# jkulhanek/tetra-nerf

Measured on AMD Instinct MI355X. Metric: ray_tet_intersections_per_s, higher is better.
Workload: dtype f32

## Files before the change

### include/tetranerf_hip.h

```cpp
#ifndef TETRANERF_HIP_H
#define TETRANERF_HIP_H

#include <stddef.h>
#include <stdint.h>

#ifdef __cplusplus
extern "C" {
#endif

typedef struct tn_tracer *tn_tracer_t;

const char *tn_last_error(void);

const char *tn_version(void);

#define TN_ABI_VERSION 6
int tn_abi_version(void);

int tn_tracer_create(int device, tn_tracer_t *out);

int tn_tracer_destroy(tn_tracer_t tracer);

int tn_load_tetrahedra(tn_tracer_t tracer, size_t num_vertices, size_t num_cells,
                       const float *xyz, const uint32_t *cells, void *stream);

int tn_update_vertices(tn_tracer_t tracer, size_t num_vertices, const float *xyz, void *stream);

size_t tn_refit_table_bytes(tn_tracer_t tracer);

#define TN_LIMIT_STEP_NO_VERIFY 1u
int tn_tet_quality(tn_tracer_t tracer, size_t num_vertices, const float *xyz, float *width, int8_t *orient, float *star_width,
                   void *stream);
int tn_limit_vertex_step(tn_tracer_t tracer, size_t num_vertices, const float *xyz_old, float *xyz_new, float fraction,
                         float *star_width, uint32_t *counters, uint32_t flags, void *stream);

int tn_delaunay_check(tn_tracer_t tracer, size_t num_vertices, const float *xyz, uint32_t *counters, int8_t *face_state,
                      uint8_t *tet_violations, void *stream);

int tn_remap_tet_values(size_t num_vertices, size_t num_old_cells, const uint32_t *old_cells, const float *old_values,
                        size_t num_new_cells, const uint32_t *new_cells, float *new_values, float *star_max, void *stream);

int tn_isosurface_count(size_t num_vertices, size_t num_cells, const uint32_t *cells, const float *values, float level,
                        const uint8_t *tet_mask, uint32_t *tri_offsets, uint32_t *ref_offsets, void *stream);
int tn_isosurface_emit(size_t num_vertices, size_t num_cells, const float *xyz, const uint32_t *cells, const float *values,
                       float level, const uint8_t *tet_mask, const uint32_t *tri_offsets, const uint32_t *ref_offsets,
                       size_t num_triangles, size_t num_refs, uint32_t *triangles, uint32_t *triangle_tets,
                       uint32_t *edge_vertices, float *edge_t, float *positions, uint32_t *num_out_vertices, void *stream);

int tn_isosurface_refine_begin(size_t num_vertices, size_t num_surface_vertices, const uint32_t *edge_vertices,
                               const float *values, float level, float *brackets, uint8_t *frozen, void *stream);
int tn_isosurface_refine_points(size_t num_vertices, size_t num_surface_vertices, uint32_t round, const uint32_t *edge_vertices,
                                const float *brackets, const uint8_t *frozen, uint32_t *vertex_indices, float *barycentric,
                                void *stream);
int tn_isosurface_refine_select(size_t num_surface_vertices, uint32_t round, float level, const float *densities,
                                float *brackets, uint8_t *frozen, void *stream);
int tn_isosurface_refine_vertices(size_t num_vertices, size_t num_surface_vertices, const float *xyz,
                                  const uint32_t *edge_vertices, const float *brackets, float level, float *edge_t,
                                  float *positions, void *stream);

int tn_split_count(size_t num_vertices, size_t num_cells, const float *xyz, const uint32_t *cells, const uint8_t *select,
                   uint32_t *offsets, uint32_t *counters, void *stream);
int tn_split_emit(size_t num_vertices, size_t num_cells, const float *xyz, const uint32_t *cells, const uint32_t *offsets,
                  size_t num_new, float *xyz_out, uint32_t *cells_out, uint32_t *cell_parent, uint32_t *vertex_parents,
                  void *stream);
int tn_split_vertex_rows(size_t rows, size_t num_vertices, size_t num_new, const float *values, const float *values_vm,
                         const uint32_t *vertex_parents, uint32_t new_mode, float *out, float *out_vm, void *stream);

int tn_prune_count(tn_tracer_t tracer, size_t num_vertices, const uint8_t *dead, const uint8_t *vertex_select, uint32_t *offsets,
                   uint32_t *counters, void *stream);
int tn_prune_count_tables(int device, size_t num_vertices, size_t num_cells, const uint32_t *cells, size_t num_faces,
                          const uint32_t *faces, const uint32_t *face_tets, const uint8_t *dead, const uint8_t *vertex_select,
                          uint32_t *offsets, uint32_t *counters, void *stream);
int tn_prune_emit(size_t num_vertices, const float *xyz, const uint32_t *offsets, size_t num_kept, uint32_t *new_id,
                  uint32_t *kept_ids, float *xyz_out, void *stream);
int tn_prune_vertex_rows(size_t rows, size_t num_vertices, size_t num_kept, const float *values, const float *values_vm,
                         const uint32_t *kept_ids, float *out, float *out_vm, void *stream);

int tn_edge_split_count_tables(int device, size_t num_vertices, size_t num_cells, const float *xyz, const uint32_t *cells,
                               const uint8_t *select, size_t num_faces, const uint32_t *faces, const uint32_t *face_tets,
                               uint32_t *tet_offsets, uint32_t *tet_edge, uint8_t *bisected, uint32_t *edge_vertices,
                               uint32_t *counters, void *stream);
int tn_edge_split_count(tn_tracer_t tracer, size_t num_vertices, const float *xyz, const uint8_t *select, uint32_t *tet_offsets,
                        uint32_t *tet_edge, uint8_t *bisected, uint32_t *edge_vertices, uint32_t *counters, void *stream);
int tn_edge_split_emit(size_t num_vertices, size_t num_cells, const float *xyz, const uint32_t *cells, const uint32_t *tet_offsets,
                       const uint32_t *tet_edge, const uint32_t *edge_vertices, size_t num_new, size_t num_rows, float *xyz_out,
                       uint32_t *cells_out, uint32_t *cell_parent, uint32_t *vertex_parents, void *stream);

size_t tn_num_faces(tn_tracer_t tracer);

int tn_get_faces(tn_tracer_t tracer, uint32_t *faces_host, uint32_t *face_tets_host);

int tn_get_build_table(tn_tracer_t tracer, int which, void *dst, size_t *bytes);

int tn_trace_rays(tn_tracer_t tracer, size_t num_rays, uint32_t max_ray_triangles,
                  const float *origins, const float *directions, uint32_t *num_visited,
                  uint32_t *visited, float *bary, float *dist, uint32_t *verts, void *stream);

#define TN_TRACE_COMPACT_ROWS 1u
#define TN_TRACE_BIN_RAYS 2u
int tn_trace_rays_ex(tn_tracer_t tracer, size_t num_rays, uint32_t max_ray_triangles,
                     const float *origins, const float *directions, uint32_t *num_visited,
                     uint32_t *visited, float *bary, float *dist, uint32_t *verts, uint32_t flags, void *stream);

int tn_trace_rays_triangles(tn_tracer_t tracer, size_t num_rays, uint32_t max_ray_triangles,
                            const float *origins, const float *directions, uint32_t *num_visited,
                            uint32_t *visited, float *bary, float *dist, uint32_t *verts, void *stream);

int tn_find_tetrahedra(tn_tracer_t tracer, size_t num_points, const float *positions, uint32_t *tetrahedra,
                       float *bary, uint32_t *verts, void *stream);

int tn_find_matched_cells(size_t num_rays, size_t num_samples, size_t max_visited_cells,
                          const uint32_t *num_visited, const uint32_t *visited,
                          const float *dist, const float *bary, const float *distances,
                          const uint32_t *verts, uint32_t *cells_out, uint32_t *verts_out,
                          uint8_t *mask_out, float *bary_out, void *stream);

int tn_find_matched_cells_indexed(size_t num_rays, size_t num_samples, size_t max_visited_cells,
                                  const uint32_t *ray_index, const uint32_t *num_visited, const uint32_t *visited,
                                  const float *dist, const float *bary, const float *distances,
                                  const uint32_t *verts, uint32_t *cells_out, uint32_t *verts_out,
                                  uint8_t *mask_out, float *bary_out, const uint32_t *count ,
                                  void *stream);

int tn_compact_hits(size_t num_rays, const uint32_t *num_visited, uint32_t *order, uint32_t *count, uint32_t *padded,
                    uint32_t *scratch, size_t scratch_len, void *stream);

int tn_interpolate_values(uint32_t interpolation_dim, uint32_t num_vertices,
                          uint32_t num_values, uint32_t field_dim,
                          const uint32_t *vertex_indices, const float *barycentric,
                          const float *field, float *result, void *stream);

int tn_interpolate_values_backward(uint32_t interpolation_dim, uint32_t num_vertices,
                                   uint32_t num_values, uint32_t field_dim,
                                   const uint32_t *vertex_indices, const float *barycentric,
                                   const float *grad_in, float *field_grad_out, void *stream);

int tn_interpolate_values_backward_rows(uint32_t interpolation_dim, uint32_t num_vertices,
                                        uint32_t num_values, uint32_t field_dim,
                                        const uint32_t *vertex_indices, const float *barycentric,
                                        const float *grad_rows, float *field_grad_out, void *stream);

int tn_transpose_f32(uint32_t rows, uint32_t cols, const float *in, float *out, void *stream);
int tn_interpolate_values_vm(uint32_t interpolation_dim, uint32_t num_values, uint32_t field_dim,
                             const uint32_t *vertex_indices, const float *barycentric, const float *field_vm,
                             float *result, void *stream);
int tn_interpolate_values_backward_vm(uint32_t interpolation_dim, uint32_t num_values, uint32_t field_dim,
                                      const uint32_t *vertex_indices, const float *barycentric,
                                      const float *grad_rows, float *field_grad_vm, void *stream);
int tn_interpolate_values_backward_vm_det(uint32_t interpolation_dim, uint32_t num_vertices, uint32_t num_values,
                                          uint32_t field_dim, const uint32_t *vertex_indices, const float *barycentric,
                                          const float *grad_rows, float *field_grad_vm, void *stream);

int tn_interpolate_values_backward_bary_vm(uint32_t interpolation_dim, uint32_t num_values, uint32_t field_dim,
                                           const uint32_t *vertex_indices, const float *grad_rows, const float *field_vm,
                                           float *grad_bary, void *stream);
int tn_sample_positions_backward(size_t num_rays, uint32_t samples_per_ray, uint32_t num_vertices,
                                 const uint32_t *vertex_indices, const float *barycentric, const float *grad_bary,
                                 const float *distances, const float *vertices,
                                 float *grad_points, float *grad_origins, float *grad_directions,
                                 float *grad_vertices, void *stream);

int tn_postprocess_hits(tn_tracer_t tracer, size_t num_rays, uint32_t max_ray_triangles,
                        const uint32_t *hit_count, const uint32_t *hit_ids, const float *hit_t,
                        const float *hit_uv, uint32_t *num_visited, uint32_t *visited,
                        float *bary, float *dist, uint32_t *verts, void *stream);

int tn_postprocess_hits_tables(int device, size_t num_rays, uint32_t max_ray_triangles, const uint32_t *faces,
                               const uint32_t *face_tets, const uint32_t *hit_count, const uint32_t *hit_ids,
                               const float *hit_t, const float *hit_uv, uint32_t *num_visited, uint32_t *visited,
                               float *bary, float *dist, uint32_t *verts, void *stream);

int tn_trace_stats(tn_tracer_t tracer, uint64_t stats[4]);

int tn_trace_flag_reasons(tn_tracer_t tracer, uint64_t reasons[16]);

int tn_trace_cross_check(tn_tracer_t tracer, uint64_t out[8]);

int tn_trace_timings(tn_tracer_t tracer, float ms[8]);

int tn_trace_ray_order(tn_tracer_t tracer, uint32_t *order_host, size_t *n);

int tn_fill_rows(size_t num_rays, uint32_t max_ray_triangles, uint32_t first_slot, uint32_t *visited, float *bary, float *dist,
                 uint32_t *verts, void *stream);

int tn_set_option(tn_tracer_t tracer, const char *name, int value);

int tn_gather_uint32(int elem_size, uint32_t num_values, uint32_t num_indices, const uint32_t *indices,
                     const void *values, void *result, void *stream);
int tn_scatter_ema_uint32(int elem_size, uint32_t num_result, uint32_t num_indices, const uint32_t *indices,
                          double decay, const void *values, void *result, void *stream);

typedef struct tn_mlp_weights {
    const float *w1, *b1;
    const float *w2, *b2;
    const float *w3, *b3;
    const float *wd, *bd;
    const float *wh, *bh;
    const float *wr, *br;
} tn_mlp_weights;

typedef struct tn_mlp *tn_mlp_t;
int tn_mlp_create(int device, tn_mlp_t *out);
int tn_mlp_destroy(tn_mlp_t mlp);
int tn_mlp_set_weights(tn_mlp_t mlp, const tn_mlp_weights *weights, void *stream);

int tn_mlp_forward(tn_mlp_t mlp, size_t n, uint32_t samples_per_ray, const float *feats, const float *dirs, int mode,
                   float *sigma, float *rgb, void *stream);

int tn_mlp_forward_gather(tn_mlp_t mlp, size_t n, uint32_t samples_per_ray, const uint32_t *vertex_indices,
                          const float *barycentric, const float *field_vm, const float *dirs, int mode, float *sigma,
                          float *rgb, const float *ray_head_bias, const uint32_t *count ,
                          void *stream);

int tn_occupancy_update(uint32_t num_cells, size_t n, const uint32_t *cells, const float *sigma, float decay, float *occupancy,
                        uint32_t samples_per_ray, const uint32_t *count, void *stream);

int tn_cull_samples(size_t n, uint32_t samples_per_ray, const uint32_t *cells, const float *occupancy, uint32_t num_cells,
                    float threshold, uint32_t *live, uint32_t *live_count, float *sigma, float *rgb, uint32_t *scratch,
                    size_t scratch_len, const uint32_t *count, void *stream);

int tn_mlp_forward_gather_indexed(tn_mlp_t mlp, size_t n_max, uint32_t samples_per_ray, const uint32_t *live,
                                  const uint32_t *live_count, const uint32_t *vertex_indices, const float *barycentric,
                                  const float *field_vm, const float *dirs, int mode, float *sigma, float *rgb,
                                  const float *ray_head_bias, const uint32_t *count, void *stream);

int tn_tet_stats_accumulate(uint32_t num_cells, size_t num_rows, uint32_t samples_per_ray, const uint32_t *cells, const float *sigma,
                            const float *edges, const float *ray_value, const uint32_t *ray_index, const uint32_t *count,
                            int64_t *stats, void *stream);

int tn_sample_live(size_t num_hit_rays, uint32_t num_samples, uint32_t max_ray_triangles, const uint32_t *ray_index,
                   const uint32_t *num_visited, const uint32_t *visited, const float *hit_distances, const float *occupancy,
                   uint32_t num_cells, float threshold, const float *linspace, const float *t_rand, float *s_edges,
                   float *near_far_live, const uint32_t *count, void *stream);
int tn_live_to_distance(size_t num_hit_rays, uint32_t num_values, uint32_t max_ray_triangles, const uint32_t *ray_index,
                        const uint32_t *num_visited, const uint32_t *visited, const float *hit_distances, const float *occupancy,
                        uint32_t num_cells, float threshold, const float *values, float *t, uint32_t *slot, const uint32_t *count,
                        void *stream);

typedef struct tn_rgb_background { float r, g, b; int clamp; } tn_rgb_background;
int tn_render_rays(tn_mlp_t mlp, uint32_t max_ray_triangles, const uint32_t *num_visited, const float *hit_distances,
                   const float *barycentric, const uint32_t *vertex_indices, const uint32_t *ray_index, const uint32_t *count,
                   size_t num_hit_rays_max, uint32_t num_samples, uint32_t num_fine, int biased, const float *linspace,
                   const float *u_table, float histogram_padding, float eps, const float *field_vm, const float *dirs,
                   const tn_rgb_background *background, float *out_rgb, float *out_acc, float *out_depth,
                   const float *ray_head_bias, void *stream);
int tn_render_rays_ex(tn_mlp_t mlp, uint32_t max_ray_triangles, const uint32_t *num_visited, const float *hit_distances,
                   const float *barycentric, const uint32_t *vertex_indices, const uint32_t *ray_index, const uint32_t *count,
                   size_t num_hit_rays_max, uint32_t num_samples, uint32_t num_fine, int biased, const float *linspace,
                   const float *u_table, float histogram_padding, float eps, const float *field_vm, const float *dirs,
                   const tn_rgb_background *background, float *out_rgb, float *out_acc, float *out_depth,
                   const float *ray_head_bias, int mode, void *stream);

int tn_sample_coarse(size_t num_hit_rays, uint32_t num_samples, uint32_t max_ray_triangles, const uint32_t *ray_index,
                     const uint32_t *num_visited, const float *hit_distances, const float *linspace, const float *t_rand,
                     int biased, float *edges, float *near_far, const uint32_t *count, void *stream);
int tn_sample_pdf(size_t num_hit_rays, uint32_t num_samples, uint32_t num_fine, const float *edges, const float *weights,
                  const float *near_far, const float *u_table, const float *u_rand, float histogram_padding, float eps,
                  float *edges_out, const uint32_t *count, void *stream);

int tn_composite(size_t num_rays, uint32_t num_samples, const float *sigma, const float *rgb, const float *edges,
                 const tn_rgb_background *background, float *out_rgb, float *out_acc, float *out_depth,
                 float *out_weights, const uint32_t *ray_index, const uint32_t *count, void *stream);

typedef struct tn_mlp_backward_buffers {
    float *x0, *h1, *h2, *h3, *h4;
    void *masks;
    float *d1, *d2, *d3, *d4, *dhead, *dx0;
} tn_mlp_backward_buffers;
int tn_mlp_forward_gather_train(tn_mlp_t mlp, size_t n, uint32_t samples_per_ray, const uint32_t *vertex_indices,
                                const float *barycentric, const float *field_vm, const float *dirs, float *sigma, float *rgb,
                                const tn_mlp_backward_buffers *buffers, const float *ray_head_bias, void *stream);
int tn_mlp_forward_gather_train_ex(tn_mlp_t mlp, size_t n, uint32_t samples_per_ray, const uint32_t *vertex_indices,
                                   const float *barycentric, const float *field_vm, const float *dirs, int mode, float *sigma,
                                   float *rgb, const tn_mlp_backward_buffers *buffers, const float *ray_head_bias, void *stream);
int tn_mlp_backward(tn_mlp_t mlp, size_t n, const float *sigma, const float *rgb, const float *d_sigma, const float *d_rgb,
                    const tn_mlp_backward_buffers *buffers, void *stream);
int tn_mlp_backward_ex(tn_mlp_t mlp, size_t n, const float *sigma, const float *rgb, const float *d_sigma, const float *d_rgb,
                       const tn_mlp_backward_buffers *buffers, int mode, void *stream);
int tn_mlp_ray_head_grad(size_t n, uint32_t samples_per_ray, const tn_mlp_backward_buffers *buffers, float *d_ray_head_bias,
                         void *stream);
typedef struct tn_mlp_grads {
    float *w1, *b1, *w2, *b2, *w3, *b3, *wd, *bd, *wh, *bh, *wr, *br;
} tn_mlp_grads;
int tn_mlp_param_grads(tn_mlp_t mlp, size_t n, uint32_t samples_per_ray, const float *dirs,
                       const tn_mlp_backward_buffers *buffers, const tn_mlp_grads *grads, void *stream);
int tn_mlp_param_grads_ex(tn_mlp_t mlp, size_t n, uint32_t samples_per_ray, const float *dirs,
                          const tn_mlp_backward_buffers *buffers, const tn_mlp_grads *grads, int mode, void *stream);

int tn_mlp_forward_gather_train_indexed(tn_mlp_t mlp, size_t n_live, size_t n_samples, uint32_t samples_per_ray, const uint32_t *live,
                                        const uint32_t *vertex_indices, const float *barycentric, const float *field_vm,
                                        const float *dirs, int mode, float *sigma, float *rgb, const tn_mlp_backward_buffers *buffers,
                                        const float *ray_head_bias, void *stream);
int tn_mlp_param_grads_indexed(tn_mlp_t mlp, size_t n_live, size_t n_samples, uint32_t samples_per_ray, const uint32_t *live,
                               const float *dirs, const tn_mlp_backward_buffers *buffers, const tn_mlp_grads *grads, int mode,
                               void *stream);
int tn_mlp_ray_head_grad_indexed(size_t n_live, size_t n_samples, uint32_t samples_per_ray, const uint32_t *live,
                                 const tn_mlp_backward_buffers *buffers, float *d_ray_head_bias, void *stream);
int tn_compact_rows(uint32_t words_per_row, size_t n_live, const uint32_t *live, const void *src, void *dst, void *stream);

int tn_composite_backward(size_t num_rays, uint32_t num_samples, const float *sigma, const float *rgb, const float *edges,
                          const tn_rgb_background *background, const float *d_out_rgb, const float *d_out_acc,
                          float *d_sigma, float *d_rgb, void *stream);

int tn_composite_aux(size_t num_rays, uint32_t num_samples, const float *sigma, const float *edges, float *out_depth_moment,
                     float *out_distortion, float *out_weights, void *stream);

int tn_composite_backward_aux(size_t num_rays, uint32_t num_samples, const float *sigma, const float *rgb, const float *edges,
                              const tn_rgb_background *background, const float *d_out_rgb, const float *d_out_acc,
                              const float *d_out_depth_moment, const float *d_out_distortion, float *d_sigma, float *d_rgb,
                              void *stream);

typedef struct tn_radam_hyper {
    float one_minus_beta1, beta2, one_minus_beta2, eps, decay;
    int decay_mode;
} tn_radam_hyper;
typedef struct tn_radam_tensor {
    float *param;
    const float *grad;
    float *exp_avg, *exp_avg_sq;
    size_t count;
    float step_size;
    int adaptive;
} tn_radam_tensor;
int tn_radam_step_field(uint32_t num_vertices, float *field, const float *grad, float *exp_avg, float *exp_avg_sq, float *shadow_vm,
                        float step_size, int adaptive, const tn_radam_hyper *hyper, void *stream);
int tn_radam_step(size_t num_tensors, const tn_radam_tensor *tensors, const tn_radam_hyper *hyper, void *stream);

#ifdef __cplusplus
}
#endif
#endif
```

### tetra-nerf_amd/_lib.py

```python
from __future__ import annotations

import ctypes as C
from pathlib import Path

import os

_HERE = Path(__file__).resolve().parent
LIB_PATH = Path(os.environ["TETRANERF_HIP_LIB"]).resolve() if os.environ.get("TETRANERF_HIP_LIB") else _HERE / "libtetranerf_hip.so"

SYMBOLS = (
    "tn_last_error", "tn_version", "tn_abi_version", "tn_tracer_create", "tn_tracer_destroy", "tn_load_tetrahedra",
    "tn_num_faces", "tn_get_faces", "tn_get_build_table", "tn_trace_rays", "tn_trace_rays_ex", "tn_trace_rays_triangles", "tn_find_tetrahedra",
    "tn_find_matched_cells", "tn_find_matched_cells_indexed",
    "tn_interpolate_values", "tn_interpolate_values_backward", "tn_interpolate_values_backward_rows",
    "tn_transpose_f32", "tn_interpolate_values_vm", "tn_interpolate_values_backward_vm", "tn_interpolate_values_backward_vm_det",
    "tn_postprocess_hits", "tn_postprocess_hits_tables",
    "tn_trace_stats", "tn_trace_flag_reasons", "tn_set_option", "tn_mlp_create", "tn_mlp_destroy", "tn_mlp_set_weights",
    "tn_mlp_forward", "tn_mlp_forward_gather", "tn_composite", "tn_gather_uint32", "tn_scatter_ema_uint32",
    "tn_mlp_forward_gather_train", "tn_mlp_forward_gather_train_ex", "tn_mlp_backward", "tn_mlp_backward_ex", "tn_mlp_ray_head_grad", "tn_mlp_param_grads", "tn_mlp_param_grads_ex", "tn_composite_backward", "tn_sample_coarse", "tn_sample_pdf",
    "tn_trace_timings", "tn_trace_cross_check", "tn_fill_rows", "tn_compact_hits", "tn_render_rays", "tn_render_rays_ex",
    "tn_trace_ray_order",
    "tn_interpolate_values_backward_bary_vm", "tn_sample_positions_backward",
    "tn_occupancy_update", "tn_cull_samples", "tn_mlp_forward_gather_indexed",
    "tn_mlp_forward_gather_train_indexed", "tn_mlp_param_grads_indexed", "tn_mlp_ray_head_grad_indexed", "tn_compact_rows",
    "tn_update_vertices", "tn_refit_table_bytes",
    "tn_sample_live", "tn_live_to_distance",
    "tn_composite_aux", "tn_composite_backward_aux",
    "tn_tet_quality", "tn_limit_vertex_step",
    "tn_delaunay_check", "tn_remap_tet_values",
    "tn_isosurface_count", "tn_isosurface_emit",
    "tn_isosurface_refine_begin", "tn_isosurface_refine_points", "tn_isosurface_refine_select", "tn_isosurface_refine_vertices",
    "tn_radam_step_field", "tn_radam_step",
    "tn_split_count", "tn_split_emit", "tn_split_vertex_rows",
    "tn_tet_stats_accumulate",
    "tn_prune_count", "tn_prune_count_tables", "tn_prune_emit", "tn_prune_vertex_rows",
    "tn_edge_split_count", "tn_edge_split_count_tables", "tn_edge_split_emit",
)

ABI_VERSION = 6

_lib = None


def load():
    global _lib
    if _lib is not None:
        return _lib
    if not LIB_PATH.exists():
        raise RuntimeError(
            f"ERROR: {LIB_PATH} is missing. Build it first: python __graft_entry__.py "
            "(or make -C tetra-nerf_amd/csrc). There is no CPU fallback.")
    lib = C.CDLL(str(LIB_PATH))
    vp, sz, u32, i32 = C.c_void_p, C.c_size_t, C.c_uint32, C.c_int
    lib.tn_last_error.restype = C.c_char_p
    lib.tn_last_error.argtypes = []
    lib.tn_version.restype = C.c_char_p
    lib.tn_version.argtypes = []
    if not hasattr(lib, "tn_abi_version") or lib.tn_abi_version() != ABI_VERSION:
        got = lib.tn_abi_version() if hasattr(lib, "tn_abi_version") else "none (a build older than ABI 6)"
        raise RuntimeError(f"ERROR: {LIB_PATH} exports ABI {got}, this binding needs ABI {ABI_VERSION} "
                           "(include/tetranerf_hip.h: TN_ABI_VERSION). Rebuild it: python __graft_entry__.py")
    lib.tn_abi_version.argtypes = []
    lib.tn_tracer_create.argtypes = [i32, C.POINTER(vp)]
    lib.tn_tracer_destroy.argtypes = [vp]
    lib.tn_load_tetrahedra.argtypes = [vp, sz, sz, vp, vp, vp]
    lib.tn_update_vertices.argtypes = [vp, sz, vp, vp]
    lib.tn_tet_quality.argtypes = [vp, sz, vp, vp, vp, vp, vp]
    lib.tn_limit_vertex_step.argtypes = [vp, sz, vp, vp, C.c_float, vp, vp, u32, vp]
    lib.tn_delaunay_check.argtypes = [vp, sz, vp, vp, vp, vp, vp]
    lib.tn_remap_tet_values.argtypes = [sz, sz, vp, vp, sz, vp, vp, vp, vp]
    lib.tn_isosurface_count.argtypes = [sz, sz, vp, vp, C.c_float, vp, vp, vp, vp]
    lib.tn_isosurface_emit.argtypes = [sz, sz, vp, vp, vp, C.c_float, vp, vp, vp, sz, sz, vp, vp, vp, vp, vp, vp, vp]
    lib.tn_isosurface_refine_begin.argtypes = [sz, sz, vp, vp, C.c_float, vp, vp, vp]
    lib.tn_isosurface_refine_points.argtypes = [sz, sz, u32, vp, vp, vp, vp, vp, vp]
    lib.tn_isosurface_refine_select.argtypes = [sz, u32, C.c_float, vp, vp, vp, vp]
    lib.tn_isosurface_refine_vertices.argtypes = [sz, sz, vp, vp, vp, C.c_float, vp, vp, vp]
    lib.tn_split_count.argtypes = [sz, sz, vp, vp, vp, vp, vp, vp]
    lib.tn_split_emit.argtypes = [sz, sz, vp, vp, vp, sz, vp, vp, vp, vp, vp]
    lib.tn_split_vertex_rows.argtypes = [sz, sz, sz, vp, vp, vp, u32, vp, vp, vp]
    lib.tn_prune_count.argtypes = [vp, sz, vp, vp, vp, vp, vp]
    lib.tn_prune_count_tables.argtypes = [i32, sz, sz, vp, sz, vp, vp, vp, vp, vp, vp, vp]
    lib.tn_prune_emit.argtypes = [sz, vp, vp, sz, vp, vp, vp, vp]
    lib.tn_prune_vertex_rows.argtypes = [sz, sz, sz, vp, vp, vp, vp, vp, vp]
    lib.tn_edge_split_count_tables.argtypes = [i32, sz, sz, vp, vp, vp, sz, vp, vp, vp, vp, vp, vp, vp, vp]
    lib.tn_edge_split_count.argtypes = [vp, sz, vp, vp, vp, vp, vp, vp, vp, vp]
    lib.tn_edge_split_emit.argtypes = [sz, sz, vp, vp, vp, vp, vp, sz, sz, vp, vp, vp, vp, vp]
    lib.tn_tet_stats_accumulate.argtypes = [u32, sz, u32, vp, vp, vp, vp, vp, vp, vp, vp]
    lib.tn_refit_table_bytes.restype = sz
    lib.tn_refit_table_bytes.argtypes = [vp]
    lib.tn_num_faces.restype = sz
    lib.tn_num_faces.argtypes = [vp]
    lib.tn_get_faces.argtypes = [vp, vp, vp]
    lib.tn_get_build_table.argtypes = [vp, i32, vp, C.POINTER(sz)]
    lib.tn_trace_rays.argtypes = [vp, sz, u32, vp, vp, vp, vp, vp, vp, vp, vp]
    lib.tn_trace_rays_ex.argtypes = [vp, sz, u32, vp, vp, vp, vp, vp, vp, vp, u32, vp]
    lib.tn_trace_rays_triangles.argtypes = [vp, sz, u32, vp, vp, vp, vp, vp, vp, vp, vp]
    lib.tn_find_tetrahedra.argtypes = [vp, sz, vp, vp, vp, vp, vp]
    lib.tn_find_matched_cells.argtypes = [sz, sz, sz] + [vp] * 11
    lib.tn_find_matched_cells_indexed.argtypes = [sz, sz, sz] + [vp] * 13
    lib.tn_interpolate_values.argtypes = [u32, u32, u32, u32, vp, vp, vp, vp, vp]
    lib.tn_interpolate_values_backward.argtypes = [u32, u32, u32, u32, vp, vp, vp, vp, vp]
    lib.tn_interpolate_values_backward_rows.argtypes = [u32, u32, u32, u32, vp, vp, vp, vp, vp]
    lib.tn_transpose_f32.argtypes = [u32, u32, vp, vp, vp]
    lib.tn_interpolate_values_vm.argtypes = [u32, u32, u32, vp, vp, vp, vp, vp]
    lib.tn_interpolate_values_backward_vm.argtypes = [u32, u32, u32, vp, vp, vp, vp, vp]
    lib.tn_interpolate_values_backward_vm_det.argtypes = [u32, u32, u32, u32, vp, vp, vp, vp, vp]
    lib.tn_interpolate_values_backward_bary_vm.argtypes = [u32, u32, u32, vp, vp, vp, vp, vp]
    lib.tn_sample_positions_backward.argtypes = [sz, u32, u32] + [vp] * 10
    lib.tn_postprocess_hits.argtypes = [vp, sz, u32] + [vp] * 10
    lib.tn_postprocess_hits_tables.argtypes = [i32, sz, u32] + [vp] * 12
    lib.tn_trace_stats.argtypes = [vp, C.POINTER(C.c_uint64 * 4)]
    lib.tn_trace_flag_reasons.argtypes = [vp, C.POINTER(C.c_uint64 * 16)]
    lib.tn_set_option.argtypes = [vp, C.c_char_p, i32]
    lib.tn_trace_timings.argtypes = [vp, C.POINTER(C.c_float * 8)]
    lib.tn_trace_cross_check.argtypes = [vp, C.POINTER(C.c_uint64 * 8)]
    lib.tn_trace_ray_order.argtypes = [vp, vp, C.POINTER(sz)]
    lib.tn_fill_rows.argtypes = [sz, u32, u32, vp, vp, vp, vp, vp]
    lib.tn_mlp_create.argtypes = [i32, C.POINTER(vp)]
    lib.tn_mlp_destroy.argtypes = [vp]
    lib.tn_mlp_set_weights.argtypes = [vp, vp, vp]
    lib.tn_mlp_forward.argtypes = [vp, sz, u32, vp, vp, i32, vp, vp, vp]
    lib.tn_mlp_forward_gather.argtypes = [vp, sz, u32, vp, vp, vp, vp, i32, vp, vp, vp, vp, vp]
    lib.tn_gather_uint32.argtypes = [i32, u32, u32, vp, vp, vp, vp]
    lib.tn_scatter_ema_uint32.argtypes = [i32, u32, u32, vp, C.c_double, vp, vp, vp]
    lib.tn_composite.argtypes = [sz, u32, vp, vp, vp, vp, vp, vp, vp, vp, vp, vp, vp]
    lib.tn_mlp_forward_gather_train.argtypes = [vp, sz, u32, vp, vp, vp, vp, vp, vp, vp, vp, vp]
    lib.tn_mlp_forward_gather_train_ex.argtypes = [vp, sz, u32, vp, vp, vp, vp, i32, vp, vp, vp, vp, vp]
    lib.tn_mlp_ray_head_grad.argtypes = [sz, u32, vp, vp, vp]
    lib.tn_mlp_backward.argtypes = [vp, sz, vp, vp, vp, vp, vp, vp]
    lib.tn_mlp_backward_ex.argtypes = [vp, sz, vp, vp, vp, vp, vp, i32, vp]
    lib.tn_mlp_param_grads.argtypes = [vp, sz, u32, vp, vp, vp, vp]
    lib.tn_mlp_param_grads_ex.argtypes = [vp, sz, u32, vp, vp, vp, i32, vp]
    lib.tn_composite_backward.argtypes = [sz, u32, vp, vp, vp, vp, vp, vp, vp, vp, vp]
    lib.tn_composite_aux.argtypes = [sz, u32, vp, vp, vp, vp, vp, vp]
    lib.tn_composite_backward_aux.argtypes = [sz, u32, vp, vp, vp, vp, vp, vp, vp, vp, vp, vp, vp]
    lib.tn_sample_coarse.argtypes = [sz, u32, u32, vp, vp, vp, vp, vp, i32, vp, vp, vp, vp]
    lib.tn_sample_pdf.argtypes = [sz, u32, u32, vp, vp, vp, vp, vp, C.c_float, C.c_float, vp, vp, vp]
    lib.tn_sample_live.argtypes = [sz, u32, u32, vp, vp, vp, vp, vp, u32, C.c_float, vp, vp, vp, vp, vp, vp]
    lib.tn_live_to_distance.argtypes = [sz, u32, u32, vp, vp, vp, vp, vp, u32, C.c_float, vp, vp, vp, vp, vp]
    lib.tn_compact_hits.argtypes = [sz, vp, vp, vp, vp, vp, sz, vp]
    lib.tn_render_rays.argtypes = [vp, u32, vp, vp, vp, vp, vp, vp, sz, u32, u32, i32, vp, vp, C.c_float, C.c_float, vp, vp, vp, vp, vp, vp, vp, vp]
    lib.tn_render_rays_ex.argtypes = [vp, u32, vp, vp, vp, vp, vp, vp, sz, u32, u32, i32, vp, vp, C.c_float, C.c_float, vp, vp, vp, vp, vp, vp, vp, i32, vp]
    lib.tn_occupancy_update.argtypes = [u32, sz, vp, vp, C.c_float, vp, u32, vp, vp]
    lib.tn_cull_samples.argtypes = [sz, u32, vp, vp, u32, C.c_float, vp, vp, vp, vp, vp, sz, vp, vp]
    lib.tn_mlp_forward_gather_indexed.argtypes = [vp, sz, u32, vp, vp, vp, vp, vp, vp, i32, vp, vp, vp, vp, vp]
    lib.tn_mlp_forward_gather_train_indexed.argtypes = [vp, sz, sz, u32, vp, vp, vp, vp, vp, i32, vp, vp, vp, vp, vp]
    lib.tn_mlp_param_grads_indexed.argtypes = [vp, sz, sz, u32, vp, vp, vp, vp, i32, vp]
    lib.tn_mlp_ray_head_grad_indexed.argtypes = [sz, sz, u32, vp, vp, vp, vp]
    lib.tn_compact_rows.argtypes = [u32, sz, vp, vp, vp, vp]
    lib.tn_radam_step_field.argtypes = [u32, vp, vp, vp, vp, vp, C.c_float, i32, vp, vp]
    lib.tn_radam_step.argtypes = [sz, vp, vp, vp]
    for name in SYMBOLS:
        fn = getattr(lib, name)
        if fn.restype is C.c_int and name not in ("tn_last_error", "tn_version", "tn_abi_version", "tn_num_faces", "tn_refit_table_bytes"):
            fn.restype = C.c_int
    _lib = lib
    return lib


def check(rc: int):
    if rc != 0:
        msg = load().tn_last_error().decode("utf-8", "replace")
        raise RuntimeError(msg or f"libtetranerf_hip call failed (rc={rc})")
```

### tetra-nerf_amd/csrc/tn_api_tracer.hip

```cpp
#include <algorithm>
#include <cmath>
#include <cstring>
#include <memory>
#include <mutex>

#include "tn_api_common.h"
#include "tn_build.h"
#include "tn_devbuf.h"
#include "tn_isosurface_core.h"
#include "tn_kernels.h"
#include "tn_split_core.h"
#include "tn_edge_split_core.h"

using tn::check_loaded;
using tn::check_pow2_M;
using tn::DeviceGuard;
using tn::guarded;

struct tn_tracer {
    int device = 0;
    std::mutex mu;

    struct Mesh {
        bool loaded = false;
        tn::DeviceMesh view;
        tn::HostMesh host;
        uint32_t bvh_max_stack = 1;
        tn::DevBuf<uint32_t> faces, face_tets;
        tn::DevWideBvh bvh;
        tn::DevBuf<tn::WalkVar> vars;
        tn::DevBuf<tn::WalkHot> hot;
        tn::DevBuf<tn::WalkCold> cold;
        tn::DevBuf<tn::WalkTet> tets;
        tn::DevBuf<tn::WalkFid> fidt;
        tn::DevBuf<float> hull_nodes, hull_tris;
        tn::RefitTables refit;
        bool device_built = false;
    } mesh;

    struct Options {
        bool gpu_build = true;
        unsigned leaf_width = 16;
        int writer_table = 0;
        bool refit_tables = false;
        int use_walk = 1;
        size_t walk_min_rays = 12288;
        bool walk_min_auto = true;
        bool dense_tails = true;
        bool literal = true;
        size_t log_cap_bytes = 0;
        int spec_fill = 0;
        unsigned spec_k0 = 0;
        tn::FillRange spec{true, 0, true, tn::FillKind::Spans, 512};
        unsigned walk_lds_kb = 26;
        tn::FillRange tail{false, 0, false, tn::FillKind::RowPerBlock, 0};
        unsigned writer_blocks = 0;
        bool hull_flat = true;
        bool small_lds = true;
        unsigned lds_cap = 0;
        unsigned verify_stride = 256;
        bool verify_risk = true;
        unsigned risk_band = 2;
        bool verify_inject = false;
        unsigned literal_sort_passes = 8;
        int cert_ends = 2;
        bool bin_rays = false;
        bool timing = false;
    } opt;

    struct Scratch {
        tn::DevBuf<uint32_t> fallback_list;
        tn::DevBuf<uint32_t> walk_n;
        tn::DevBuf<uint4> hull_entry;
        tn::DevBuf<uint2> literal_list;
        tn::DevBuf<uint4> hit_log;
        tn::DevBuf<uint32_t> verify_list;
        tn::DevBuf<uint32_t> risk_list;
        tn::DevBuf<uint32_t> ray_keys, ray_iota, ray_keys_sorted, order, walk_n_item;
        tn::DevBuf<char> sort_temp;
        static constexpr int N_CTR = 2;
        tn::DevBuf<unsigned long long> stats;
        uint32_t *fallback_count() { return reinterpret_cast<uint32_t *>(stats.p + tn::N_STATS); }
        uint32_t *literal_count() { return fallback_count() + 1; }
        uint32_t *verify_count() { return fallback_count() + 2; }
        uint32_t *risk_count() { return fallback_count() + 3; }
        static constexpr size_t stats_bytes() { return (tn::N_STATS + N_CTR) * sizeof(unsigned long long); }
        size_t last_num_rays = 0;
        bool last_walk = false;
        bool last_binned = false;
        hipStream_t last_stream = nullptr;

        template <typename T>
        static void grow(tn::DevBuf<T> &b, size_t n) { if (b.n < n) b.alloc(n); }
        void reserve(size_t R, size_t log_entries, bool verify, bool risk, size_t sort_temp_bytes = 0) {
            grow(fallback_list, R);
            if (!log_entries) return;
            grow(walk_n, R); grow(literal_list, R); grow(hull_entry, R); grow(hit_log, log_entries);
            if (verify) grow(verify_list, R);
            if (risk) grow(risk_list, R);
            if (sort_temp_bytes) {
                grow(ray_keys, R); grow(ray_iota, R); grow(ray_keys_sorted, R); grow(order, R); grow(walk_n_item, R);
                grow(sort_temp, sort_temp_bytes);
            }
        }
    } scratch;

    struct Schedule {
        hipStream_t side = nullptr;
        hipStream_t aux = nullptr;
        hipStream_t pre = nullptr;
        hipEvent_t ev_fork = nullptr, ev_join = nullptr, ev_start = nullptr, ev_pre = nullptr, ev_seg = nullptr, ev_aux = nullptr;
        static constexpr int N_TEV = 9;
        hipEvent_t tev[N_TEV] = {};
        bool tev_valid = false;
    } sched;
};

namespace {

tn_tracer *checked(tn_tracer_t t) {
    if (!t) throw tn::Error("tracer handle is null");
    return t;
}

void check_bvh_depth(uint32_t max_stack) {
    if (max_stack + (uint32_t)tn::WIDE > (uint32_t)tn::STACK_CAP)
        throw tn::Error("face BVH too deep for the traversal stack (" + std::to_string(max_stack) + " > " +
                        std::to_string(tn::STACK_CAP) + " entries)");
}

struct BuildCounts { size_t F = 0, n_hull = 0, n_hull_nodes = 0; };

BuildCounts build_on_host(tn_tracer::Mesh &m, unsigned leaf_width, size_t V, size_t T, const float *xyz, const uint32_t *cells,
                          hipStream_t stream) {
    std::vector<float> hxyz(3 * V);
    std::vector<uint32_t> hcells(4 * T);
    TN_HIP(hipStreamSynchronize(stream));
    if (V) TN_HIP(hipMemcpy(hxyz.data(), xyz, hxyz.size() * sizeof(float), hipMemcpyDeviceToHost));
    if (T) TN_HIP(hipMemcpy(hcells.data(), cells, hcells.size() * sizeof(uint32_t), hipMemcpyDeviceToHost));
    for (size_t i = 0; i < hcells.size(); ++i)
        if (hcells[i] >= V) throw tn::Error("cells contains a vertex index that is out of bounds");

    tn::build_face_table(T, hcells.data(), m.host);
    const size_t F = m.host.face_tets.size() / 2;
    float smax = 0.f;
    for (size_t i = 0; i < hcells.size(); ++i)
        for (int k = 0; k < 3; ++k) smax = std::max(smax, std::fabs(hxyz[3 * (size_t)hcells[i] + k]));
    m.host.scene_max = smax;

    std::vector<uint32_t> all(F), hull_ids;
    for (size_t f = 0; f < F; ++f) {
        all[f] = (uint32_t)f;
        if (m.host.face_tets[2 * f + 1] == TN_EMPTY) hull_ids.push_back((uint32_t)f);
    }
    tn::HostWideBvh hb;
    tn::build_wide_bvh(hxyz.data(), m.host.faces.data(), all, hb, leaf_width);
    check_bvh_depth(hb.max_stack);
    m.bvh_max_stack = hb.max_stack;
    std::vector<tn::TetRec> recs;
    std::vector<uint32_t> rec_of_tet;
    tn::build_tet_records(T, hcells.data(), hxyz.data(), m.host, recs, rec_of_tet);
    tn::HostHullBvh hth;
    tn::build_hull_threaded(hxyz.data(), m.host.faces.data(), m.host.face_tets.data(), hull_ids, recs, rec_of_tet, hth);

    m.faces.upload(m.host.faces);
    m.face_tets.upload(m.host.face_tets);
    m.bvh.upload(hb, smax);
    {
        std::vector<tn::WalkVar> vars;
        tn::build_walk_variants(recs, vars);
        m.vars.upload(vars);
    }
    m.hull_nodes.upload(hth.nodes_and_flat());
    m.hull_tris.upload(hth.tris);
    return BuildCounts{F, hull_ids.size(), hth.nodes.size() / 8};
}

tn::TraceParams mesh_params(const tn_tracer *t, size_t num_items, const tn::Rows &r, const float *o, const float *d) {
    tn::TraceParams p{};
    p.origins = o; p.dirs = d;
    p.faces = t->mesh.view.faces; p.face_tets = t->mesh.view.face_tets;
    p.bvh = t->mesh.view.bvh;
    p.out_num = r.num; p.out_cells = r.cells; p.out_bary = r.bary; p.out_dist = r.dist; p.out_verts = r.verts;
    p.M = r.M; p.num_items = num_items; p.ray_list = nullptr;
    return p;
}

struct TraceCall {
    tn_tracer *t;
    size_t R;
    const float *origins, *dirs;
    tn::Rows rows;
    bool dense_tails;
    hipStream_t stream;
    bool binned = false;

    const tn_tracer::Options &o() const { return t->opt; }
    tn_tracer::Scratch &s() const { return t->scratch; }
    const tn::DeviceMesh &mesh() const { return t->mesh.view; }
    bool verify_risk() const { return o().verify_risk && o().verify_stride; }

    size_t walk_min_rays() const {
        if (!o().walk_min_auto) return o().walk_min_rays;
        return mesh().T >= 4000000u ? (size_t)6144 : mesh().T >= 2000000u ? (size_t)8192 : o().walk_min_rays;
    }
    bool use_walk() const {
        return o().use_walk && (R >= walk_min_rays() || o().use_walk == 2) && rows.M >= 4 && mesh().n_hull > 0 &&
               mesh().n_hull < (1u << 24);
    }
    size_t log_chunk() const {
        size_t cap_bytes = o().log_cap_bytes;
        if (!cap_bytes) {
            size_t free_b = 0, total_b = 0;
            TN_HIP(hipMemGetInfo(&free_b, &total_b));
            cap_bytes = std::min<size_t>((free_b + s().hit_log.n * sizeof(uint4)) / 4, (size_t)24 << 30);
        }
        const size_t chunk = std::max<size_t>(cap_bytes / ((size_t)rows.M * sizeof(uint4)) / 4096 * 4096, 4096);
        return std::min(chunk, R);
    }

    tn::TraceParams trace_params(size_t base, size_t n) const {
        tn::TraceParams q = mesh_params(t, n, rows.at(base), origins + 3 * base, dirs + 3 * base);
        q.stats = s().stats.p;
        q.compact_rows = dense_tails ? 0u : 1u;
        q.sort_passes = o().literal_sort_passes;
        return q;
    }
    tn::WalkParams walk_params(size_t base, size_t n) const {
        const tn::DeviceMesh &m = mesh();
        tn::WalkParams w{};
        w.t = trace_params(base, n);
        w.vars = m.hot;
        w.scene_max = m.bvh.scene_max;
        w.hull_nodes = m.hull_nodes; w.hull_tris = m.hull_tris; w.n_hull_nodes = m.n_hull_nodes; w.n_hull = m.n_hull;
        w.hull_flat = m.hull_nodes + 2 * (size_t)m.n_hull_nodes;
        w.n_hull_leaves = o().hull_flat ? tn::hull_flat_leaves(m.n_hull) : 0u;
        w.n_hull_groups = o().hull_flat ? tn::hull_flat_groups(m.n_hull) : 0u;
        w.ray_base = base;
        w.hull_entry = s().hull_entry.p + base; w.walk_n = s().walk_n.p + base; w.hit_log = s().hit_log.p;
        w.fallback_list = s().fallback_list.p; w.fallback_count = s().fallback_count();
        w.literal_list = o().literal ? s().literal_list.p : nullptr; w.literal_count = s().literal_count();
        w.risk_list = verify_risk() ? s().risk_list.p : nullptr; w.risk_count = s().risk_count();
        w.risk_band = (float)o().risk_band;
        if (binned) { w.order = s().order.p; w.walk_n_item = s().walk_n_item.p; }
        w.cert_ends = o().cert_ends == 2 ? (m.T >= tn::WALK_TET_MIN_TETS ? 1u : 3u) : (uint32_t)o().cert_ends;
        return w;
    }
    tn::WriteParams write_params(size_t base, size_t n) const {
        const tn::Rows r = rows.at(base);
        tn::WriteParams q{};
        q.num_rays = n; q.M = r.M; q.dense_tails = dense_tails ? 1u : 0u;
        q.walk_n = s().walk_n.p + base;
        q.hit_log = s().hit_log.p;
        q.cold = mesh().cold; q.tets = mesh().tets;
        q.out_cells = r.cells; q.out_bary = r.bary; q.out_dist = r.dist; q.out_verts = r.verts;
        if (binned) { q.walk_n = s().walk_n_item.p; q.order = s().order.p; }
        return q;
    }

    void fill_tails(size_t base, size_t n, uint32_t k_hi) const {
        if (!dense_tails) return;
        tn::FillRange f = o().tail;
        f.k_split = k_hi;
        tn::launch_fill(rows.at(base), n, s().walk_n.p + base, f, stream);
    }
    void pair_literal(size_t base, size_t n, hipStream_t st) const {
        if (!o().literal) return;
        tn::launch_postprocess_log(trace_params(base, n), mesh().fidt, s().hit_log.p, s().literal_list.p, s().literal_count(), n, st,
                                   binned ? s().order.p : nullptr);
    }
    void trace_listed(const uint32_t *list, const uint32_t *count, size_t max_items, hipStream_t st) const {
        tn::TraceParams q = trace_params(0, max_items);
        q.ray_list = list; q.item_count = count;
        tn::launch_trace_general(q, st);
    }

    uint32_t spec_fill_first_slot() const {
        if (!o().spec_fill || !dense_tails) return 0;
        const uint32_t M = rows.M;
        uint32_t K0 = (((uint32_t)(3.6 * std::cbrt((double)std::max<uint32_t>(mesh().T, 1u))) + 31u) & ~31u) + 32u;
        const uint32_t quarter = (3u * M / 4u) & ~31u, half = (M / 2u) & ~31u;
        if (mesh().T >= tn::WALK_TET_MIN_TETS) K0 = K0 > quarter + 32u ? 0u : quarter;
        else K0 = K0 > quarter ? 0u : (K0 + 32u > half ? half : quarter);
        if (o().spec_k0) K0 = o().spec_k0 & ~31u;
        return K0 + 32u > M ? 0u : K0;
    }

    void run_overlapped() const {
        tn_tracer::Schedule &c = t->sched;
        const bool timing = o().timing;
        const hipStream_t s_pre = timing ? stream : c.pre, s_aux = timing ? stream : c.aux, s_side = timing ? stream : c.side;
        if (timing && !c.tev[0])
            for (hipEvent_t &e : c.tev) TN_HIP(hipEventCreate(&e));
        int mark_i = 0;
        auto mark = [&] { if (timing) TN_HIP(hipEventRecord(c.tev[mark_i++], stream)); };
        const uint32_t K0 = spec_fill_first_slot();
        mark();
        if (K0) {
            TN_HIP(hipEventRecord(c.ev_start, stream));
            TN_HIP(hipStreamWaitEvent(s_pre, c.ev_start, 0));
            tn::FillRange f = o().spec;
            f.k_split = K0;
            tn::launch_fill(rows, R, s().walk_n.p, f, s_pre);
            TN_HIP(hipEventRecord(c.ev_pre, s_pre));
        }
        mark();
        if (binned)
            tn::launch_ray_order(R, origins, dirs, tn::ray_key_box(mesh().box_lo, mesh().box_hi), s().ray_keys.p, s().ray_iota.p,
                                 s().ray_keys_sorted.p, s().order.p, s().sort_temp.p, s().sort_temp.n, stream);
        tn::launch_trace_walk(walk_params(0, R), stream, K0 && !timing ? (size_t)o().walk_lds_kb * 1024 : 0);
        mark();
        TN_HIP(hipEventRecord(c.ev_fork, stream));
        TN_HIP(hipStreamWaitEvent(s_aux, c.ev_fork, 0));
        if (K0) {
            TN_HIP(hipStreamWaitEvent(s_aux, c.ev_pre, 0));
            TN_HIP(hipStreamWaitEvent(stream, c.ev_pre, 0));
        }
        trace_listed(s().fallback_list.p, s().fallback_count(), R, s_aux);
        mark();
        if (o().verify_stride) {
            tn::launch_verify_counts(trace_params(0, R), o().verify_stride, s().walk_n.p, s().verify_list.p, s().verify_count(), 0,
                                     s_aux, true, o().verify_inject);
            if (verify_risk())
                tn::launch_verify_counts(trace_params(0, R), o().verify_stride, s().walk_n.p, s().verify_list.p, s().verify_count(), 0,
                                         s_aux, true, false, s().risk_list.p, s().risk_count(), R);
        }
        mark();
        TN_HIP(hipEventRecord(c.ev_aux, s_aux));
        tn::launch_write_segments(write_params(0, R), stream, o().writer_blocks);
        mark();
        TN_HIP(hipEventRecord(c.ev_seg, stream));
        TN_HIP(hipStreamWaitEvent(s_side, c.ev_seg, 0));
        pair_literal(0, R, s_side);
        mark();
        fill_tails(0, R, K0 ? K0 : rows.M);
        mark();
        TN_HIP(hipEventRecord(c.ev_join, s_side));
        TN_HIP(hipStreamWaitEvent(stream, c.ev_join, 0));
        TN_HIP(hipStreamWaitEvent(stream, c.ev_aux, 0));
        if (o().verify_stride) trace_listed(s().verify_list.p, s().verify_count(), 64, stream);
        mark();
        c.tev_valid = timing;
    }

    void run_chunked(size_t chunk) const {
        for (size_t base = 0; base < R; base += chunk) {
            const size_t n = std::min(R - base, chunk);
            TN_HIP(hipMemsetAsync(s().literal_count(), 0, sizeof(uint32_t), stream));
            TN_HIP(hipMemsetAsync(s().risk_count(), 0, sizeof(uint32_t), stream));
            const tn::WalkParams w = walk_params(base, n);
            tn::launch_trace_walk(w, stream, 0);
            if (o().verify_stride) {
                tn::launch_verify_counts(w.t, o().verify_stride, w.walk_n, w.fallback_list, w.fallback_count, base, stream, false,
                                         o().verify_inject);
                if (verify_risk())
                    tn::launch_verify_counts(w.t, o().verify_stride, w.walk_n, w.fallback_list, w.fallback_count, base, stream, false,
                                             false, s().risk_list.p, s().risk_count(), n);
            }
            tn::launch_write_segments(write_params(base, n), stream, o().writer_blocks);
            fill_tails(base, n, rows.M);
            pair_literal(base, n, stream);
        }
        trace_listed(s().fallback_list.p, s().fallback_count(), R, stream);
    }

    void run_small_batch() const {
        uint32_t C = 64;
        const double expect = 3.6 * std::cbrt((double)std::max<uint32_t>(mesh().T, 1u));
        while (C < expect && C < rows.M) C <<= 1;
        if (o().lds_cap) C = o().lds_cap;
        tn::TraceParams p = trace_params(0, R);
        if (o().small_lds && C < rows.M) {
            s().reserve(R, 0, false, false);
            tn::TraceParams p1 = p;
            p1.lds_cap = C; p1.overflow_list = s().fallback_list.p; p1.overflow_count = s().fallback_count();
            tn::launch_trace_general(p1, stream);
            p.ray_list = s().fallback_list.p;
            p.item_count = s().fallback_count();
        }
        tn::launch_trace_general(p, stream);
    }
};

}

extern "C" {

int tn_tracer_create(int device, tn_tracer_t *out) {
    return guarded([&] {
        if (!out) throw tn::Error("out is null");
        int count = 0;
        TN_HIP(hipGetDeviceCount(&count));
        if (device < 0 || device >= count) throw tn::Error("The device argument must be a CUDA device.");
        DeviceGuard g(device);
        auto t = std::make_unique<tn_tracer>();
        t->device = device;
        t->opt.use_walk = tn::env_flag("TETRANERF_HIP_WALK", true) ? 1 : 0;
        t->opt.gpu_build = tn::env_flag("TETRANERF_HIP_GPU_BUILD", true);
        t->opt.bin_rays = tn::env_flag("TETRANERF_HIP_BIN_RAYS", false);
        t->scratch.stats.alloc(tn::N_STATS + tn_tracer::Scratch::N_CTR);
        TN_HIP(hipMemset(t->scratch.stats.p, 0, tn_tracer::Scratch::stats_bytes()));
        tn_tracer::Schedule &c = t->sched;
        int least = 0, greatest = 0;
        TN_HIP(hipDeviceGetStreamPriorityRange(&least, &greatest));
        TN_HIP(hipStreamCreateWithPriority(&c.side, hipStreamNonBlocking, least));
        TN_HIP(hipStreamCreateWithPriority(&c.aux, hipStreamNonBlocking, least));
        TN_HIP(hipStreamCreateWithFlags(&c.pre, hipStreamNonBlocking));
        for (hipEvent_t *e : {&c.ev_fork, &c.ev_join, &c.ev_start, &c.ev_pre, &c.ev_seg, &c.ev_aux})
            TN_HIP(hipEventCreateWithFlags(e, hipEventDisableTiming));
        *out = t.release();
    });
}

int tn_tracer_destroy(tn_tracer_t tracer) {
    return guarded([&] {
        if (!tracer) return;
        DeviceGuard g(tracer->device);
        (void)hipDeviceSynchronize();
        const tn_tracer::Schedule &c = tracer->sched;
        for (hipStream_t st : {c.side, c.aux, c.pre})
            if (st) (void)hipStreamDestroy(st);
        for (hipEvent_t e : {c.ev_fork, c.ev_join, c.ev_start, c.ev_pre, c.ev_seg, c.ev_aux})
            if (e) (void)hipEventDestroy(e);
        for (hipEvent_t e : c.tev)
            if (e) (void)hipEventDestroy(e);
        delete tracer;
    });
}

int tn_load_tetrahedra(tn_tracer_t tracer, size_t V, size_t T, const float *xyz, const uint32_t *cells,
                       void *stream_) {
    return guarded([&] {
        tn_tracer *t = checked(tracer);
        std::lock_guard<std::mutex> lock(t->mu);
        DeviceGuard g(t->device);
        hipStream_t stream = (hipStream_t)stream_;
        if ((V && !xyz) || (T && !cells)) throw tn::Error("xyz / cells must not be null");
        if (V >= 0xFFFFFFFFull || T >= 0x0FFFFFFFull) throw tn::Error("mesh too large (uint32 ids)");
        if (T == 0) throw tn::Error("load_tetrahedra needs at least one tetrahedron");
        tn_tracer::Mesh &b = t->mesh;
        b.loaded = false;
        b.host.faces.clear(); b.host.face_tets.clear();
        b.refit.release();
        b.device_built = t->opt.gpu_build;
        BuildCounts n;
        if (b.device_built) {
            tn::BuildInfo bi;
            tn::device_build(V, T, xyz, cells, stream,
                             tn::BuildTargets{b.faces, b.face_tets, b.vars, b.hull_nodes, b.hull_tris, b.bvh}, bi, t->opt.leaf_width,
                             t->opt.refit_tables ? &b.refit : nullptr);
            check_bvh_depth(bi.max_stack);
            b.host.scene_max = bi.scene_max;
            b.bvh_max_stack = bi.max_stack;
            n = BuildCounts{bi.F, bi.n_hull, bi.n_hull_nodes};
        } else {
            n = build_on_host(b, t->opt.leaf_width, V, T, xyz, cells, stream);
        }

        tn::DeviceMesh &m = b.view;
        m.xyz = xyz; m.cells = cells;
        m.V = (uint32_t)V; m.T = (uint32_t)T; m.F = (uint32_t)n.F;
        m.faces = b.faces.p; m.face_tets = b.face_tets.p;
        m.bvh = b.bvh.view;
        {
            const size_t n4 = b.vars.n;
            const bool per_tet = t->opt.writer_table ? t->opt.writer_table == 2 : n4 / 4 >= tn::WALK_TET_MIN_TETS;
            b.hot.alloc(n4); b.fidt.alloc(n4);
            b.cold.release(); b.tets.release();
            if (per_tet) b.tets.alloc(n4 / 4); else b.cold.alloc(n4);
            tn::launch_split_walk_records(n4, b.vars.p, b.hot.p, per_tet ? nullptr : b.cold.p, per_tet ? b.tets.p : nullptr,
                                          b.fidt.p, stream);
            TN_HIP(hipStreamSynchronize(stream));
            b.vars.release();
        }
        m.hot = b.hot.p; m.cold = b.cold.n ? b.cold.p : nullptr; m.tets = b.tets.n ? b.tets.p : nullptr; m.fidt = b.fidt.p;
        m.n_hull = (uint32_t)n.n_hull;
        m.hull_nodes = reinterpret_cast<const float4 *>(b.hull_nodes.p);
        m.hull_tris = reinterpret_cast<const float4 *>(b.hull_tris.p);
        m.n_hull_nodes = (uint32_t)n.n_hull_nodes;
        tn::mesh_box(V, T, xyz, cells, m.box_lo, m.box_hi, stream);
        b.loaded = true;
    });
}

int tn_update_vertices(tn_tracer_t tracer, size_t V, const float *xyz, void *stream_) {
    return guarded([&] {
        tn_tracer *t = checked(tracer);
        std::lock_guard<std::mutex> lock(t->mu);
        tn_tracer::Mesh &b = t->mesh;
        if (!b.loaded) throw tn::Error("tn_update_vertices: no mesh is loaded; call load_tetrahedra first");
        if (!b.device_built)
            throw tn::Error("tn_update_vertices: the mesh was built on the host (option \"gpu_build\" = 0); the refit is part of the "
                            "device build: set \"gpu_build\" = 1 and load again, or reload after every move");
        if (!b.refit.valid)
            throw tn::Error("tn_update_vertices: the mesh was loaded without the refit tables; set option \"refit_tables\" = 1 "
                            "(Python: load_tetrahedra(..., refittable=True)) and load again");
        if (V != b.view.V)
            throw tn::Error("tn_update_vertices: " + std::to_string(V) + " vertices given, the loaded mesh has " +
                            std::to_string(b.view.V) + "; a mesh with other vertices or cells needs load_tetrahedra");
        if (!xyz) throw tn::Error("tn_update_vertices: xyz must not be null");
        DeviceGuard g(t->device);
        hipStream_t stream = (hipStream_t)stream_;
        tn::DeviceMesh &m = b.view;
        float smax = 0.f;
        tn::device_refit(V, m.T, xyz, m.cells, stream, tn::RefitTargets{b.hot.p, b.faces.p, b.hull_nodes, b.hull_tris, b.bvh}, b.refit,
                         smax, m.box_lo, m.box_hi);
        b.host.scene_max = smax;
        m.bvh = b.bvh.view;
        m.xyz = xyz;
    });
}

size_t tn_refit_table_bytes(tn_tracer_t tracer) {
    return tracer && tracer->mesh.loaded && tracer->mesh.refit.valid ? tracer->mesh.refit.bytes() : 0;
}

namespace {
void check_guard_mesh(tn_tracer *t, const char *who, size_t V) {
    tn_tracer::Mesh &b = t->mesh;
    if (!b.loaded) throw tn::Error(std::string(who) + ": no mesh is loaded; call load_tetrahedra first");
    if (V != b.view.V)
        throw tn::Error(std::string(who) + ": " + std::to_string(V) + " vertices given, the loaded mesh has " + std::to_string(b.view.V));
}
}

int tn_tet_quality(tn_tracer_t tracer, size_t V, const float *xyz, float *width, int8_t *orient, float *star_width, void *stream_) {
    return guarded([&] {
        tn_tracer *t = checked(tracer);
        std::lock_guard<std::mutex> lock(t->mu);
        check_guard_mesh(t, "tn_tet_quality", V);
        const tn::DeviceMesh &m = t->mesh.view;
        if (!xyz) throw tn::Error("tn_tet_quality: xyz must not be null");
        DeviceGuard g(t->device);
        tn::launch_tet_quality(V, m.T, m.cells, xyz, width, orient, star_width, (hipStream_t)stream_);
    });
}

int tn_limit_vertex_step(tn_tracer_t tracer, size_t V, const float *xyz_old, float *xyz_new, float fraction, float *star_width,
                         uint32_t *counters, uint32_t flags, void *stream_) {
    return guarded([&] {
        tn_tracer *t = checked(tracer);
        std::lock_guard<std::mutex> lock(t->mu);
        check_guard_mesh(t, "tn_limit_vertex_step", V);
        const tn::DeviceMesh &m = t->mesh.view;
        if (!xyz_old || !xyz_new || !star_width || !counters)
            throw tn::Error("tn_limit_vertex_step: xyz_old, xyz_new, star_width and counters must not be null");
        if (!(fraction > 0.f && fraction <= 0.45f))
            throw tn::Error("tn_limit_vertex_step: fraction must be in (0, 0.45]: the bound is proved for moves below half a width, "
                            "and 0.45 leaves room for the rounding of the new coordinates");
        if (flags & ~(uint32_t)TN_LIMIT_STEP_NO_VERIFY) throw tn::Error("tn_limit_vertex_step: unknown flags");
        DeviceGuard g(t->device);
        tn::launch_limit_vertex_step(V, m.T, m.cells, xyz_old, xyz_new, fraction, star_width, counters,
                                     !(flags & TN_LIMIT_STEP_NO_VERIFY), (hipStream_t)stream_);
    });
}

int tn_delaunay_check(tn_tracer_t tracer, size_t V, const float *xyz, uint32_t *counters, int8_t *face_state, uint8_t *tet_violations,
                      void *stream_) {
    return guarded([&] {
        tn_tracer *t = checked(tracer);
        std::lock_guard<std::mutex> lock(t->mu);
        check_guard_mesh(t, "tn_delaunay_check", V);
        const tn::DeviceMesh &m = t->mesh.view;
        if (!xyz || !counters) throw tn::Error("tn_delaunay_check: xyz and counters must not be null");
        if ((uintptr_t)tet_violations & 3u)
            throw tn::Error("tn_delaunay_check: tet_violations must be 4-byte aligned (its bytes are counted through 32-bit atomics)");
        DeviceGuard g(t->device);
        tn::launch_delaunay_check(m.T, m.F, m.cells, m.face_tets, xyz, counters, face_state, tet_violations, (hipStream_t)stream_);
    });
}

int tn_remap_tet_values(size_t V, size_t num_old_cells, const uint32_t *old_cells, const float *old_values, size_t num_new_cells,
// ... 215 lines not shown
        if (num_kept && (!kept_ids || !out || (!values && !values_vm)))
            throw tn::Error("tn_prune_vertex_rows: a null pointer beside a non-zero count");
        tn::launch_prune_vertex_rows(rows, V, num_kept, values, values_vm, kept_ids, out, out_vm, (hipStream_t)stream_);
    });
}

namespace {
void check_edge_split_count(const char *who, size_t V, size_t T, size_t F, const void *xyz, const void *cells, const void *select,
                            const void *faces, const void *face_tets, const void *tet_offsets, const void *tet_edge,
                            const void *bisected, const void *edge_vertices, const void *counters) {
    const std::string w(who);
    if (V >= 0xFFFFFFFFull) throw tn::Error(w + ": too many vertices (uint32 ids)");
    if (T >= tn::esplit::MAX_CELLS) throw tn::Error(w + ": num_cells must be below 2^30");
    if (F >= 0xFFFFFFFFull) throw tn::Error(w + ": too many faces");
    if (!tet_offsets || !counters || (T && (!cells || !select || !tet_edge || !bisected || !edge_vertices)) || (T && V && !xyz) ||
        (F && (!faces || !face_tets)))
        throw tn::Error(w + ": a null pointer beside a non-zero count");
}
}

int tn_edge_split_count_tables(int device, size_t V, size_t T, const float *xyz, const uint32_t *cells, const uint8_t *select,
                               size_t F, const uint32_t *faces, const uint32_t *face_tets, uint32_t *tet_offsets, uint32_t *tet_edge,
                               uint8_t *bisected, uint32_t *edge_vertices, uint32_t *counters, void *stream_) {
    return guarded([&] {
        check_edge_split_count("tn_edge_split_count_tables", V, T, F, xyz, cells, select, faces, face_tets, tet_offsets, tet_edge,
                               bisected, edge_vertices, counters);
        DeviceGuard g(device);
        tn::launch_edge_split_count(V, T, xyz, cells, select, F, faces, face_tets, tet_offsets, tet_edge, bisected, edge_vertices,
                                    counters, (hipStream_t)stream_);
    });
}

int tn_edge_split_count(tn_tracer_t tracer, size_t V, const float *xyz, const uint8_t *select, uint32_t *tet_offsets,
                        uint32_t *tet_edge, uint8_t *bisected, uint32_t *edge_vertices, uint32_t *counters, void *stream_) {
    return guarded([&] {
        tn_tracer *t = checked(tracer);
        std::lock_guard<std::mutex> lock(t->mu);
        check_guard_mesh(t, "tn_edge_split_count", V);
        const tn::DeviceMesh &m = t->mesh.view;
        check_edge_split_count("tn_edge_split_count", V, m.T, m.F, xyz, m.cells, select, m.faces, m.face_tets, tet_offsets, tet_edge,
                               bisected, edge_vertices, counters);
        DeviceGuard g(t->device);
        tn::launch_edge_split_count(V, m.T, xyz, m.cells, select, m.F, m.faces, m.face_tets, tet_offsets, tet_edge, bisected,
                                    edge_vertices, counters, (hipStream_t)stream_);
    });
}

int tn_edge_split_emit(size_t V, size_t T, const float *xyz, const uint32_t *cells, const uint32_t *tet_offsets,
                       const uint32_t *tet_edge, const uint32_t *edge_vertices, size_t num_new, size_t num_rows, float *xyz_out,
                       uint32_t *cells_out, uint32_t *cell_parent, uint32_t *vertex_parents, void *stream_) {
    return guarded([&] {
        const std::string w("tn_edge_split_emit");
        if (num_new > T || num_rows > T) throw tn::Error(w + ": num_new or num_rows exceeds num_cells (a tetrahedron is bisected at most once)");
        if (V >= 0xFFFFFFFFull || V + num_new >= 0xFFFFFFFFull) throw tn::Error(w + ": too many vertices (uint32 ids)");
        if (T >= tn::esplit::MAX_CELLS || T + num_rows >= tn::esplit::MAX_CELLS) throw tn::Error(w + ": num_cells + num_rows must be below 2^30");
        if ((T && (!cells || !tet_offsets || !tet_edge || !cells_out || !cell_parent)) || (V && (!xyz || !xyz_out)) ||
            (num_new && (!edge_vertices || !xyz_out || !vertex_parents)) || (num_rows && !edge_vertices))
            throw tn::Error(w + ": a null pointer beside a non-zero count");
        tn::launch_edge_split_emit(V, T, xyz, cells, tet_offsets, tet_edge, edge_vertices, num_new, num_rows, xyz_out, cells_out,
                                   cell_parent, vertex_parents, (hipStream_t)stream_);
    });
}

size_t tn_num_faces(tn_tracer_t tracer) { return tracer && tracer->mesh.loaded ? tracer->mesh.view.F : 0; }

int tn_get_faces(tn_tracer_t tracer, uint32_t *faces_host, uint32_t *face_tets_host) {
    return guarded([&] {
        tn_tracer *t = checked(tracer);
        check_loaded(t->mesh.loaded);
        tn_tracer::Mesh &b = t->mesh;
        const size_t F = b.view.F;
        if (b.host.face_tets.size() != 2 * F) {
            DeviceGuard g(t->device);
            b.host.faces.resize(3 * F);
            b.host.face_tets.resize(2 * F);
            if (F) {
                TN_HIP(hipMemcpy(b.host.faces.data(), b.faces.p, b.host.faces.size() * sizeof(uint32_t), hipMemcpyDeviceToHost));
                TN_HIP(hipMemcpy(b.host.face_tets.data(), b.face_tets.p, b.host.face_tets.size() * sizeof(uint32_t), hipMemcpyDeviceToHost));
            }
        }
        if (faces_host) std::memcpy(faces_host, b.host.faces.data(), b.host.faces.size() * sizeof(uint32_t));
        if (face_tets_host) std::memcpy(face_tets_host, b.host.face_tets.data(), b.host.face_tets.size() * sizeof(uint32_t));
    });
}

int tn_get_build_table(tn_tracer_t tracer, int which, void *dst, size_t *bytes) {
    return guarded([&] {
        tn_tracer *t = checked(tracer);
        check_loaded(t->mesh.loaded);
        DeviceGuard g(t->device);
        const tn_tracer::Mesh &b = t->mesh;
        const void *src = nullptr;
        size_t n = 0;
        switch (which) {
            case 0: src = b.faces.p; n = b.faces.n * 4; break;
            case 1: src = b.face_tets.p; n = b.face_tets.n * 4; break;
            case 2: {
                const size_t n4 = b.hot.n;
                n = n4 * sizeof(tn::WalkVar);
                if (bytes) *bytes = n;
                if (dst && n4) {
                    std::vector<tn::WalkHot> h(n4); std::vector<tn::WalkTet> c(b.tets.n); std::vector<tn::WalkCold> cc(b.cold.n);
                    std::vector<tn::WalkFid> f(n4);
                    TN_HIP(hipMemcpy(h.data(), b.hot.p, n4 * sizeof(tn::WalkHot), hipMemcpyDeviceToHost));
                    if (!c.empty()) TN_HIP(hipMemcpy(c.data(), b.tets.p, c.size() * sizeof(tn::WalkTet), hipMemcpyDeviceToHost));
                    if (!cc.empty()) TN_HIP(hipMemcpy(cc.data(), b.cold.p, cc.size() * sizeof(tn::WalkCold), hipMemcpyDeviceToHost));
                    TN_HIP(hipMemcpy(f.data(), b.fidt.p, n4 * sizeof(tn::WalkFid), hipMemcpyDeviceToHost));
                    tn::WalkVar *o = static_cast<tn::WalkVar *>(dst);
                    for (size_t i = 0; i < n4; ++i) {
                        tn::WalkVar v{};
                        for (int k = 0; k < 3; ++k) v.pn[k] = h[i].pn[k];
                        v.nb[0] = h[i].nb0; v.nb[1] = h[i].nb1; v.nb[2] = h[i].nb2; v.code_lo = h[i].code_lo; v.code_hi = h[i].code_hi;
                        if (!c.empty()) { v.orig = c[i >> 2].orig; for (uint32_t k = 0; k < 4; ++k) v.vid[k] = c[i >> 2].vid((uint32_t)(i & 3), k); }
                        else { v.orig = cc[i].orig; for (int k = 0; k < 4; ++k) v.vid[k] = cc[i].vid[k]; }
                        v.fid0 = f[i].fid[0]; v.fid1 = f[i].fid[1]; v.fid2 = f[i].fid[2];
                        o[i] = v;
                    }
                }
                return;
            }
            case 3: src = b.hull_nodes.p; n = b.hull_nodes.n * 4; break;
            case 4: src = b.hull_tris.p; n = b.hull_tris.n * 4; break;
            case 5: src = b.bvh.child.p; n = b.bvh.child.n * 4; break;
            case 6: src = b.bvh.boxes.p; n = b.bvh.boxes.n * 4; break;
            case 7: src = b.bvh.leaf_id.p; n = b.bvh.leaf_id.n * 4; break;
            case 8: src = b.bvh.leaf_tri.p; n = b.bvh.leaf_tri.n * 4; break;
            default: throw tn::Error("unknown table");
        }
        if (bytes) *bytes = n;
        if (dst && n) TN_HIP(hipMemcpy(dst, src, n, hipMemcpyDeviceToHost));
    });
}

int tn_trace_rays_ex(tn_tracer_t tracer, size_t R, uint32_t M, const float *origins, const float *directions,
                     uint32_t *num_visited, uint32_t *visited, float *bary, float *dist, uint32_t *verts,
                     uint32_t flags, void *stream_) {
    return guarded([&] {
        tn_tracer *t = checked(tracer);
        std::lock_guard<std::mutex> lock(t->mu);
        if (flags & ~(uint32_t)(TN_TRACE_COMPACT_ROWS | TN_TRACE_BIN_RAYS)) throw tn::Error("unknown trace flag");
        check_pow2_M(M);
        check_loaded(t->mesh.loaded);
        if (M > 4096) throw tn::Error("max_ray_triangles larger than 4096 is not supported");
        if (R >= 0xFFFFFFFFull) throw tn::Error("too many rays for one call");
        if (R == 0) return;
        if (!origins || !directions || !num_visited || !visited || !bary || !dist)
            throw tn::Error("null ray / output pointer");
        DeviceGuard g(t->device);
        TraceCall call{t, R, origins, directions, tn::Rows{num_visited, visited, bary, dist, verts, M},
                             t->opt.dense_tails && !(flags & TN_TRACE_COMPACT_ROWS), (hipStream_t)stream_};
        tn_tracer::Scratch &s = t->scratch;
        TN_HIP(hipMemsetAsync(s.stats.p, 0, tn_tracer::Scratch::stats_bytes(), call.stream));
        s.last_stream = call.stream;
        s.last_num_rays = R;
        s.last_walk = call.use_walk();
        s.last_binned = false;
        if (s.last_walk) {
            const size_t chunk = call.log_chunk();
            call.binned = s.last_binned = ((flags & TN_TRACE_BIN_RAYS) || t->opt.bin_rays) && chunk >= R;
            s.reserve(R, (chunk + 255) / 256 * 256 * (size_t)M, t->opt.verify_stride != 0, call.verify_risk(),
                      call.binned ? tn::ray_order_temp_bytes(R) : 0);
            if (chunk >= R) call.run_overlapped();
            else call.run_chunked(chunk);
        } else {
            call.run_small_batch();
        }
        TN_HIP(hipGetLastError());
    });
}

int tn_trace_rays(tn_tracer_t tracer, size_t R, uint32_t M, const float *origins, const float *directions,
                  uint32_t *num_visited, uint32_t *visited, float *bary, float *dist, uint32_t *verts,
                  void *stream_) {
    return tn_trace_rays_ex(tracer, R, M, origins, directions, num_visited, visited, bary, dist, verts, 0u, stream_);
}

int tn_postprocess_hits(tn_tracer_t tracer, size_t R, uint32_t M, const uint32_t *hit_count,
                        const uint32_t *hit_ids, const float *hit_t, const float *hit_uv,
                        uint32_t *num_visited, uint32_t *visited, float *bary, float *dist, uint32_t *verts,
                        void *stream_) {
    return guarded([&] {
        tn_tracer *t = checked(tracer);
        check_pow2_M(M);
        check_loaded(t->mesh.loaded);
        if (R == 0) return;
        DeviceGuard g(t->device);
        const tn::TraceParams p = mesh_params(t, R, tn::Rows{num_visited, visited, bary, dist, verts, M}, nullptr, nullptr);
        tn::launch_postprocess_hits(p, hit_count, hit_ids, hit_t, hit_uv, (hipStream_t)stream_);
        TN_HIP(hipGetLastError());
    });
}

int tn_postprocess_hits_tables(int device, size_t R, uint32_t M, const uint32_t *faces, const uint32_t *face_tets,
                               const uint32_t *hit_count, const uint32_t *hit_ids, const float *hit_t,
                               const float *hit_uv, uint32_t *num_visited, uint32_t *visited, float *bary, float *dist,
                               uint32_t *verts, void *stream_) {
    return guarded([&] {
        check_pow2_M(M);
        if (!faces || !face_tets) throw tn::Error("null face table");
        if (R == 0) return;
        DeviceGuard g(device);
        tn::TraceParams p{};
        p.M = M; p.num_items = R;
        p.faces = faces; p.face_tets = face_tets;
        p.out_num = num_visited; p.out_cells = visited; p.out_bary = bary; p.out_dist = dist; p.out_verts = verts;
        tn::launch_postprocess_hits(p, hit_count, hit_ids, hit_t, hit_uv, (hipStream_t)stream_);
        TN_HIP(hipGetLastError());
    });
}

int tn_trace_rays_triangles(tn_tracer_t tracer, size_t R, uint32_t M, const float *origins, const float *directions,
                            uint32_t *num_visited, uint32_t *visited, float *bary, float *dist, uint32_t *verts,
                            void *stream_) {
    return guarded([&] {
        tn_tracer *t = checked(tracer);
        check_pow2_M(M);
        check_loaded(t->mesh.loaded);
        if (M > 4096) throw tn::Error("max_ray_triangles larger than 4096 is not supported");
        if (R == 0) return;
        DeviceGuard g(t->device);
        const tn::TraceParams p = mesh_params(t, R, tn::Rows{num_visited, nullptr, nullptr, nullptr, nullptr, M}, origins, directions);
        tn::launch_trace_triangles(p, visited, dist, bary, verts, (hipStream_t)stream_);
        TN_HIP(hipGetLastError());
    });
}

int tn_find_tetrahedra(tn_tracer_t tracer, size_t N, const float *positions, uint32_t *tetrahedra, float *bary,
                       uint32_t *verts, void *stream_) {
    return guarded([&] {
        tn_tracer *t = checked(tracer);
        check_loaded(t->mesh.loaded);
        if (N == 0) return;
        DeviceGuard g(t->device);
        const tn::TraceParams p = mesh_params(t, N, tn::Rows{nullptr, nullptr, nullptr, nullptr, nullptr, 512}, nullptr, nullptr);
        tn::launch_find_tetrahedra(p, positions, tetrahedra, bary, verts, (hipStream_t)stream_);
        TN_HIP(hipGetLastError());
    });
}

int tn_trace_stats(tn_tracer_t tracer, uint64_t stats[4]) {
    return guarded([&] {
        tn_tracer *t = checked(tracer);
        std::lock_guard<std::mutex> lock(t->mu);
        DeviceGuard g(t->device);
        TN_HIP(hipStreamSynchronize(t->scratch.last_stream));
        unsigned long long h[tn::N_STATS];
        TN_HIP(hipMemcpy(h, t->scratch.stats.p, sizeof h, hipMemcpyDeviceToHost));
        const size_t R = t->scratch.last_num_rays;
        size_t other = R;
        if (t->scratch.last_walk) {
            uint32_t fb = 0;
            TN_HIP(hipMemcpy(&fb, t->scratch.fallback_count(), sizeof fb, hipMemcpyDeviceToHost));
            other = (uint32_t)(fb + (uint32_t)h[tn::STAT_REASON + tn::REASON_LITERAL_PAIRED]);
        }
        stats[tn::STAT_WALK] = R - other;
        stats[tn::STAT_OTHER] = other;
        stats[tn::STAT_LITERAL_BRANCH] = h[tn::STAT_LITERAL_BRANCH];
        stats[tn::STAT_OVERFLOW] = h[tn::STAT_OVERFLOW];
    });
}

int tn_trace_flag_reasons(tn_tracer_t tracer, uint64_t reasons[16]) {
    return guarded([&] {
        tn_tracer *t = checked(tracer);
        std::lock_guard<std::mutex> lock(t->mu);
        DeviceGuard g(t->device);
        TN_HIP(hipStreamSynchronize(t->scratch.last_stream));
        unsigned long long h[tn::N_STATS];
        TN_HIP(hipMemcpy(h, t->scratch.stats.p, sizeof h, hipMemcpyDeviceToHost));
        for (int i = 0; i < tn::N_REASONS; ++i) reasons[i] = h[tn::STAT_REASON + i];
    });
}

int tn_trace_cross_check(tn_tracer_t tracer, uint64_t out[8]) {
    return guarded([&] {
        tn_tracer *t = checked(tracer);
        std::lock_guard<std::mutex> lock(t->mu);
        if (!out) throw tn::Error("out is null");
        DeviceGuard g(t->device);
        TN_HIP(hipStreamSynchronize(t->scratch.last_stream));
        unsigned long long h[tn::N_STATS];
        TN_HIP(hipMemcpy(h, t->scratch.stats.p, sizeof h, hipMemcpyDeviceToHost));
        out[0] = t->opt.verify_stride;
        out[1] = h[tn::STAT_REASON + tn::REASON_VERIFY_CHECKED]; out[2] = h[tn::STAT_REASON + tn::REASON_VERIFY_BAD];
        out[3] = h[tn::STAT_RISK_HULL]; out[4] = h[tn::STAT_RISK_THIN];
        out[5] = h[tn::STAT_RISK_CHECKED]; out[6] = h[tn::STAT_RISK_BAD]; out[7] = 0;
    });
}

int tn_trace_ray_order(tn_tracer_t tracer, uint32_t *order_host, size_t *n) {
    return guarded([&] {
        tn_tracer *t = checked(tracer);
        std::lock_guard<std::mutex> lock(t->mu);
        if (!n) throw tn::Error("n is null");
        const tn_tracer::Scratch &s = t->scratch;
        *n = s.last_binned ? s.last_num_rays : 0;
        if (!order_host || !*n) return;
        DeviceGuard g(t->device);
        TN_HIP(hipStreamSynchronize(s.last_stream));
        TN_HIP(hipMemcpy(order_host, s.order.p, *n * sizeof(uint32_t), hipMemcpyDeviceToHost));
    });
}

int tn_trace_timings(tn_tracer_t tracer, float ms[8]) {
    return guarded([&] {
        tn_tracer *t = checked(tracer);
        std::lock_guard<std::mutex> lock(t->mu);
        if (!ms) throw tn::Error("ms is null");
        const tn_tracer::Schedule &c = t->sched;
        if (!c.tev_valid) throw tn::Error("no timed call: set option \"timing\" = 1 and trace a one-chunk walk call first");
        DeviceGuard g(t->device);
        TN_HIP(hipEventSynchronize(c.tev[c.N_TEV - 1]));
        for (int i = 0; i + 1 < c.N_TEV; ++i) TN_HIP(hipEventElapsedTime(&ms[i], c.tev[i], c.tev[i + 1]));
    });
}

int tn_fill_rows(size_t R, uint32_t M, uint32_t first_slot, uint32_t *visited, float *bary, float *dist, uint32_t *verts,
                 void *stream_) {
    return guarded([&] {
        if (R == 0) return;
        if (!visited || !bary || !dist) throw tn::Error("null output pointer");
        if (M < 4 || (M & (M - 1)) != 0) throw tn::Error("max_ray_triangles must be a power of 2.");
        if (first_slot >= M) return;
        if (first_slot & 31u) throw tn::Error("tn_fill_rows: first_slot must be a multiple of 32");
        tn::launch_fill(tn::Rows{nullptr, visited, bary, dist, verts, M}, R, nullptr,
                        tn::FillRange{true, first_slot, false, tn::FillKind::Linear, 0}, (hipStream_t)stream_);
        TN_HIP(hipGetLastError());
    });
}

int tn_set_option(tn_tracer_t tracer, const char *name, int value) {
    return guarded([&] {
        tn_tracer *t = checked(tracer);
        std::lock_guard<std::mutex> lock(t->mu);
        tn_tracer::Options &o = t->opt;
        auto set_grid = [](tn::FillRange &f, int v) {
            f.kind = v == -2 ? tn::FillKind::Linear : v < 0 ? tn::FillKind::RowPerBlock : tn::FillKind::Spans;
            f.blocks = v > 0 ? (unsigned)v : 0u;
        };
        const std::string k = name ? name : "";
        if (k == "gpu_build") o.gpu_build = value != 0;
        else if (k == "bin_rays") o.bin_rays = value != 0;
        else if (k == "timing") { o.timing = value != 0; t->sched.tev_valid = false; }
        else if (k == "leaf_width") {
            if (value != 16 && value != 32 && value != 64) throw tn::Error("leaf_width must be 16, 32 or 64");
            o.leaf_width = (unsigned)value;
        }
        else if (k == "walk") o.use_walk = value < 0 ? 0 : (value > 2 ? 2 : value);
        else if (k == "walk_min_rays") { o.walk_min_rays = value < 0 ? 0 : (size_t)value; o.walk_min_auto = false; }
        else if (k == "dense_tails") o.dense_tails = value != 0;
        else if (k == "literal") o.literal = value != 0;
        else if (k == "spec_fill") o.spec_fill = value != 0;
        else if (k == "spec_k0") o.spec_k0 = (unsigned)value;
        else if (k == "spec_blocks") set_grid(o.spec, value);
        else if (k == "hull_flat") o.hull_flat = value != 0;
        else if (k == "writer_blocks") o.writer_blocks = (unsigned)value;
        else if (k == "fill_blocks") set_grid(o.tail, value);
        else if (k == "walk_lds_kb") o.walk_lds_kb = (unsigned)value;
        else if (k == "small_lds") o.small_lds = value != 0;
        else if (k == "lds_cap") {
            if (value < 0 || (value & (value - 1)) != 0 || (value && value < 8)) throw tn::Error("lds_cap must be 0 or a power of two >= 8");
            o.lds_cap = (unsigned)value;
        }
        else if (k == "writer_table") o.writer_table = value;
        else if (k == "refit_tables") o.refit_tables = value != 0;
        else if (k == "cert_ends") { if (value < 0 || value > 3) throw tn::Error("cert_ends must be 0 .. 3"); o.cert_ends = value; }
        else if (k == "verify_inject") o.verify_inject = value != 0;
        else if (k == "literal_sort_passes") o.literal_sort_passes = value < 0 ? 0u : (unsigned)value;
        else if (k == "verify_stride") o.verify_stride = value < 0 ? 0u : (unsigned)value;
        else if (k == "verify_risk") o.verify_risk = value != 0;
        else if (k == "risk_band") o.risk_band = value < 1 ? 1u : (unsigned)value;
        else if (k == "log_cap_mb") o.log_cap_bytes = value <= 0 ? 0 : (size_t)value << 20;
        else throw tn::Error("unknown option " + (name ? k : std::string("(null)")));
    });
}

}
```

### tetra-nerf_amd/csrc/tn_kernels.h

```cpp
#pragma once
#include "tn_common.h"
#include "tn_ray_key.h"

namespace tn {

struct Rows {
    uint32_t *num;
    uint32_t *cells;
    float *bary;
    float *dist;
    uint32_t *verts;
    uint32_t M;
    Rows at(size_t base) const {
        return Rows{num ? num + base : nullptr, cells + base * M, bary + base * M * 6, dist + base * M * 2,
                    verts ? verts + base * M * 4 : nullptr, M};
    }
};

struct TraceParams {
    const float *origins;
    const float *dirs;
    const uint32_t *faces;
    const uint32_t *face_tets;
    WideBvh bvh;
    uint32_t *out_num;
    uint32_t *out_cells;
    float *out_bary;
    float *out_dist;
    uint32_t *out_verts;
    uint32_t M;
    size_t num_items;
    const uint32_t *ray_list;
    const uint32_t *item_count;
    uint32_t lds_cap;
    uint32_t *overflow_list;
    uint32_t *overflow_count;
    unsigned long long *stats;
    uint32_t compact_rows;
    uint32_t sort_passes;
};

void launch_trace_general(const TraceParams &p, hipStream_t stream);
void launch_postprocess_hits(const TraceParams &p, const uint32_t *hit_count, const uint32_t *hit_ids,
                             const float *hit_t, const float *hit_uv, hipStream_t stream);
size_t trace_general_smem_bytes(uint32_t M);
void launch_trace_triangles(const TraceParams &p, uint32_t *out_ids, float *out_t, float *out_uv, uint32_t *out_v3,
                            hipStream_t stream);
void launch_find_tetrahedra(const TraceParams &p, const float *points, uint32_t *out_tet, float *out_bary,
                            uint32_t *out_verts, hipStream_t stream);

void launch_split_walk_records(size_t n4, const WalkVar *vars, WalkHot *hot, WalkCold *cold, WalkTet *tets, WalkFid *fidt, hipStream_t stream);

struct WalkParams {
    TraceParams t;
    const WalkHot *vars;
    float scene_max;
    const float4 *hull_nodes;
    const float4 *hull_tris;
    uint32_t n_hull_nodes;
    const float4 *hull_flat;
    uint32_t n_hull_groups, n_hull_leaves;
    uint32_t n_hull;
    uint4 *hull_entry;
    uint32_t *fallback_list;
    uint32_t *fallback_count;
    uint2 *literal_list;
    uint32_t *literal_count;
    uint32_t *walk_n;
    uint4 *hit_log;
    size_t ray_base;
    uint32_t *risk_list;
    uint32_t *risk_count;
    float risk_band;
    uint32_t cert_ends;
    const uint32_t *order;
    uint32_t *walk_n_item;
};
void launch_trace_walk(const WalkParams &p, hipStream_t stream, size_t lds_reserve = 0);
void launch_postprocess_log(const TraceParams &p, const WalkFid *fidt, const uint4 *hit_log, const uint2 *literal_list,
                            const uint32_t *literal_count, size_t max_items, hipStream_t stream, const uint32_t *order = nullptr);

void launch_verify_counts(const TraceParams &p, uint32_t stride, uint32_t *walk_n, uint32_t *fallback_list, uint32_t *fallback_count,
                          size_t ray_base, hipStream_t stream, bool late = false, bool inject = false, const uint32_t *ray_list = nullptr,
                          const uint32_t *list_count = nullptr, size_t max_list = 0);

struct WriteParams {
    size_t num_rays;
    uint32_t M;
    uint32_t dense_tails;
    const uint32_t *walk_n;
    const uint4 *hit_log;
    const WalkCold *cold;
    const WalkTet *tets;
    uint32_t *out_cells;
    float *out_bary;
    float *out_dist;
    uint32_t *out_verts;
    const uint32_t *order;
};
void launch_write_segments(const WriteParams &q, hipStream_t stream, unsigned max_blocks = 0);
enum class FillKind {
    Spans,
    RowPerBlock,
    Linear,
};
struct FillRange { bool all_rows; uint32_t k_split; bool nontemporal; FillKind kind; unsigned blocks; };
void launch_fill(const Rows &rows, size_t num_rays, const uint32_t *walk_n, const FillRange &f, hipStream_t stream);

void mesh_box(size_t V, size_t T, const float *xyz, const uint32_t *cells, float lo[3], float hi[3], hipStream_t stream);
size_t ray_order_temp_bytes(size_t R);
void launch_ray_order(size_t R, const float *origins, const float *dirs, const RayKeyBox &box, uint32_t *keys, uint32_t *iota,
                      uint32_t *keys_sorted, uint32_t *order, void *temp, size_t temp_bytes, hipStream_t stream);

void launch_find_matched_cells(size_t R, size_t S, size_t M, const uint32_t *num_visited,
                               const uint32_t *visited, const float *dist, const float *bary,
                               const float *distances, const uint32_t *verts, uint32_t *cells_out,
                               uint32_t *verts_out, uint8_t *mask_out, float *bary_out, hipStream_t stream,
                               const uint32_t *ray_index = nullptr, const uint32_t *count = nullptr);

void launch_interpolate_values(uint32_t D, uint32_t V, uint32_t n, uint32_t Fd, const uint32_t *vi,
                               const float *bc, const float *field, float *result, hipStream_t stream);
void launch_interpolate_values_backward(uint32_t D, uint32_t V, uint32_t n, uint32_t Fd, const uint32_t *vi,
                                        const float *bc, const float *grad_in, bool rows_major, float *field_grad,
                                        hipStream_t stream);

void launch_interpolate_values_vm(uint32_t D, uint32_t n, uint32_t Fd, const uint32_t *vi, const float *bc,
                                  const float *fieldT, float *result, hipStream_t stream);
void launch_interpolate_values_backward_vm_det(uint32_t D, uint32_t V, uint32_t n, uint32_t Fd, const uint32_t *vi, const float *bc,
                                               const float *grad_rows, float *gradT, hipStream_t stream);
void launch_interpolate_values_backward_vm(uint32_t D, uint32_t n, uint32_t Fd, const uint32_t *vi, const float *bc,
                                           const float *grad_rows, float *gradT, hipStream_t stream);

void launch_interpolate_values_backward_bary_vm(uint32_t D, uint32_t n, uint32_t Fd, const uint32_t *vi, const float *grad_rows,
                                                const float *fieldT, float *grad_bary, hipStream_t stream);
void launch_sample_positions_backward(size_t R, uint32_t S, uint32_t V, const uint32_t *vi, const float *bc, const float *grad_bary,
                                      const float *dist, const float *verts, float *grad_points, float *grad_o, float *grad_d,
                                      float *grad_v, hipStream_t stream);

struct MlpWeights {
    const float *w1, *b1;
    const float *w2, *b2;
    const float *w3, *b3;
    const float *wd, *bd;
    const float *wh, *bh;
    const float *wr, *br;
};
struct MlpPacks {
    const float *pk_plain;
    const float *pk_gather;
    const float *pt;
    const uint4 *blob;
    const float *wenc;
    float *hterm;
    float *enc;
    const float *ray_bias;
    float *grad_scratch;
    const uint4 *blob_bf16;
    const uint4 *blob_t;
};
size_t mlp_pack_floats();
size_t mlp_backward_pack_floats();
size_t mlp_x3_blob_u4();
size_t mlp_x3_t_blob_u4();
size_t mlp_enc_floats_per_ray();
void launch_mlp_pack(const MlpWeights &w, float *pk, bool gather_l1, hipStream_t stream);
void launch_pack_wenc(const MlpWeights &w, float *wenc, hipStream_t stream);
void launch_mlp_pack_t(const MlpWeights &w, float *pt, hipStream_t stream);
void launch_mlp_pack_x3(const MlpWeights &w, uint4 *blob, hipStream_t stream);
void launch_mlp_pack_x3_t(const MlpWeights &w, uint4 *blob_t, hipStream_t stream);
void launch_mlp_forward(size_t n, uint32_t samples_per_ray, size_t num_rays, const float *feats, const uint32_t *vi,
                        const float *bc, const float *fieldT, const float *dirs, const MlpPacks &w, float *sigma, float *rgb,
                        hipStream_t stream, const uint32_t *count = nullptr);
void launch_mlp_forward_x3(size_t n, uint32_t samples_per_ray, size_t num_rays, const float *feats, const uint32_t *vi,
                           const float *bc, const float *fieldT, const float *dirs, const MlpPacks &w, float *sigma, float *rgb,
                           hipStream_t stream, const uint32_t *count = nullptr);
size_t mlp_bf16_blob_u4();
void launch_mlp_pack_bf16(const uint4 *x3blob, uint4 *blob, hipStream_t stream);
void launch_mlp_forward_bf16(size_t n, uint32_t samples_per_ray, size_t num_rays, const float *feats, const uint32_t *vi,
                             const float *bc, const float *fieldT, const float *dirs, const MlpPacks &w, float *sigma, float *rgb,
                             hipStream_t stream, const uint32_t *count = nullptr);
struct MlpFwdSave {
    float *x0;
    float *h1, *h2, *h3, *h4;
    unsigned long long *masks;
};
struct MlpBackwardBuffers : MlpFwdSave {
    float *d1, *d2, *d3, *d4;
    float *dhead;
    float *dx0;
};
void launch_mlp_forward_train(size_t n, uint32_t samples_per_ray, size_t num_rays, const uint32_t *vi, const float *bc,
                              const float *fieldT, const float *dirs, const MlpPacks &w, float *sigma, float *rgb,
                              const MlpBackwardBuffers &save, hipStream_t stream);
void launch_mlp_forward_x3_train(size_t n, uint32_t samples_per_ray, size_t num_rays, const uint32_t *vi, const float *bc,
                                 const float *fieldT, const float *dirs, const MlpPacks &w, float *sigma, float *rgb,
                                 const MlpBackwardBuffers &save, hipStream_t stream);
void launch_mlp_backward(size_t n, const float *sigma, const float *rgb, const MlpPacks &w, const float *d_sigma, const float *d_rgb,
                         const MlpBackwardBuffers &b, hipStream_t stream);
void launch_mlp_backward_x3(size_t n, const float *sigma, const float *rgb, const MlpPacks &w, const float *d_sigma, const float *d_rgb,
                            const MlpBackwardBuffers &b, hipStream_t stream);
void launch_ray_head_grad(size_t n, uint32_t samples_per_ray, const float *d4, float *out, hipStream_t stream);
struct MlpParamGrads { float *w1, *b1, *w2, *b2, *w3, *b3, *wd, *bd, *wh, *bh, *wr, *br; };
size_t mlp_param_grad_scratch_floats();
void launch_mlp_param_grads(size_t n, uint32_t samples_per_ray, const float *dirs, const MlpPacks &w, const MlpBackwardBuffers &b,
                            const MlpParamGrads &g, hipStream_t stream);
void launch_mlp_param_grads_x3(size_t n, uint32_t samples_per_ray, const float *dirs, const MlpPacks &w, const MlpBackwardBuffers &b,
                               const MlpParamGrads &g, hipStream_t stream);
struct DwGemmArgs {
    const float *A;
    const float *B;
    const float *enc;
    const float *dh;
    uint32_t spr;
    float *part;
};
void launch_dw_gemm_x3(int nbm, bool extra, unsigned grid, const DwGemmArgs &g, size_t n, uint32_t slice, hipStream_t stream);
struct Background { float r, g, b; int clamp; };
__host__ __device__ __forceinline__ float nan_to_num(float x) {
    return x != x ? 0.f : (x > 3.4028234663852886e38f ? 3.4028234663852886e38f : (x < -3.4028234663852886e38f ? -3.4028234663852886e38f : x));
}
void launch_composite_backward(size_t R, uint32_t S, const float *sigma, const float *rgb, const float *edges, Background background,
                               const float *d_out_rgb, const float *d_out_acc, float *d_sigma, float *d_rgb, hipStream_t stream);
void launch_composite_aux(size_t R, uint32_t S, const float *sigma, const float *edges, float *out_moment, float *out_dist,
                          float *out_weights, hipStream_t stream);
void launch_composite_backward_aux(size_t R, uint32_t S, const float *sigma, const float *rgb, const float *edges, Background background,
                                   const float *d_out_rgb, const float *d_out_acc, const float *d_out_moment, const float *d_out_dist,
                                   float *d_sigma, float *d_rgb, hipStream_t stream);
void launch_transpose(const float *in, float *out, uint32_t rows, uint32_t cols, hipStream_t stream);
struct RadamHyper { float one_minus_beta1, beta2, one_minus_beta2, eps, decay; int decay_mode; };
struct RadamTensor { float *p; const float *g; float *m; float *v; uint64_t n; float a; int adaptive; uint32_t first_block; };
constexpr uint32_t RADAM_TABLE = 32;
struct RadamTable { RadamTensor t[RADAM_TABLE]; uint32_t count; };
void launch_radam_field(uint32_t V, float *p, const float *g, float *m, float *v, float *shadow, const RadamHyper &h, float a,
                        bool adaptive, hipStream_t stream);
void launch_radam_flat(size_t count, const RadamTensor *tensors, const RadamHyper &h, hipStream_t stream);
struct RenderRaysLayout { uint32_t T; size_t per_block, o_edges_f, o_hterm, o_vi, o_bc, o_sigma, o_rgb, o_enc; };
size_t render_rays_scratch_floats(size_t r_max, uint32_t S, uint32_t S_fine, bool has_bias, unsigned grid, RenderRaysLayout &L);
void launch_render_rays(const uint32_t *num_visited, const float *dist, const float *bary, const uint32_t *verts, uint32_t M,
                        const uint32_t *ray_index, const uint32_t *count, size_t r_max, uint32_t S, uint32_t S_fine, bool biased,
                        const float *lin, const float *u_table, float hist_pad, float eps, const float *fieldT, const float *dirs,
                        const float *ray_bias, const MlpPacks &w, Background background, float *out_rgb, float *out_acc, float *out_depth,
                        float *scratch, const RenderRaysLayout &L, unsigned grid, hipStream_t stream,
                        unsigned long long *prof = nullptr ,
                        int mode = 0 );
void launch_sample_coarse(size_t r, uint32_t S, uint32_t M, const uint32_t *ray_index, const uint32_t *num_visited, const float *hit_dist,
                          const float *lin, const float *t_rand, bool biased, float *edges, float *near_far, hipStream_t stream,
                          const uint32_t *count = nullptr);
void launch_sample_pdf(size_t r, uint32_t S, uint32_t num_fine, const float *edges, const float *weights, const float *near_far,
                       const float *u_table, const float *u_rand, float histogram_padding, float eps, float *out, hipStream_t stream,
                       const uint32_t *count = nullptr);
void launch_sample_live(size_t r, uint32_t S, uint32_t M, const uint32_t *ray_index, const uint32_t *num_visited, const uint32_t *visited,
                        const float *hit_dist, const float *occupancy, uint32_t T, float threshold, const float *lin, const float *t_rand,
                        float *edges, float *near_far, hipStream_t stream, const uint32_t *count = nullptr);
void launch_live_to_distance(size_t r, uint32_t n, uint32_t M, const uint32_t *ray_index, const uint32_t *num_visited,
                             const uint32_t *visited, const float *hit_dist, const float *occupancy, uint32_t T, float threshold,
                             const float *values, float *t, uint32_t *slot, hipStream_t stream, const uint32_t *count = nullptr);
void launch_composite(size_t R, uint32_t S, const float *sigma, const float *rgb, const float *edges, Background background,
                      float *out_rgb, float *out_acc, float *out_depth, float *out_weights, hipStream_t stream,
                      const uint32_t *ray_index = nullptr, const uint32_t *count = nullptr);
size_t compact_scratch_u32(size_t R);
void launch_compact_hits(size_t R, const uint32_t *num_visited, uint32_t *order, uint32_t *count, uint32_t *padded, uint32_t *scratch,
                         hipStream_t stream);

void launch_head_ray_term(size_t num_rays, const float *dirs, const MlpPacks &w, hipStream_t stream);

void launch_occupancy_update(uint32_t T, size_t n, const uint32_t *cells, const float *sigma, float decay, float *occupancy,
                             uint32_t samples_per_ray, const uint32_t *count, hipStream_t stream);
size_t cull_scratch_u32(size_t n);
void launch_cull_samples(size_t n, uint32_t samples_per_ray, const uint32_t *cells, const float *occupancy, uint32_t T, float threshold,
                         uint32_t *live, uint32_t *live_count, float *sigma, float *rgb, uint32_t *scratch, const uint32_t *count,
                         hipStream_t stream);
void launch_mlp_forward_indexed(size_t n_max, uint32_t samples_per_ray, size_t num_rays, const uint32_t *live, const uint32_t *live_count,
                                const uint32_t *vi, const float *bc, const float *fieldT, const float *dirs, const MlpPacks &w, int mode,
                                float *sigma, float *rgb, hipStream_t stream, const uint32_t *count);
void launch_mlp_forward_train_indexed(size_t n_live, size_t n_samples, uint32_t samples_per_ray, const uint32_t *live, const uint32_t *vi,
                                      const float *bc, const float *fieldT, const float *dirs, const MlpPacks &w, int mode, float *sigma,
                                      float *rgb, const MlpBackwardBuffers &save, hipStream_t stream);
void launch_mlp_param_grads_indexed(size_t n_live, size_t n_samples, uint32_t samples_per_ray, const uint32_t *live, const float *dirs,
                                    const MlpPacks &w, const MlpBackwardBuffers &b, const MlpParamGrads &g, int mode, hipStream_t stream);
void launch_dw_gemm_head_indexed(bool x3, unsigned grid, const DwGemmArgs &g, size_t n, uint32_t slice, const uint32_t *live,
                                 uint32_t num_rays, hipStream_t stream);
void launch_ray_head_grad_indexed(size_t n_live, size_t n_samples, uint32_t samples_per_ray, const uint32_t *live, const float *d4,
                                  float *out, hipStream_t stream);
void launch_compact_rows(int words_per_row, size_t n_live, const uint32_t *live, const void *src, void *dst, hipStream_t stream);

void launch_gather_uint32(int elem_size, uint32_t num_values, uint32_t num_indices, const uint32_t *indices,
                          const void *values, void *result, hipStream_t stream);
void launch_scatter_ema_uint32(int elem_size, uint32_t num_result, uint32_t num_indices, const uint32_t *indices,
                               double decay, const void *values, void *result, hipStream_t stream);

}
```

### tetra-nerf_amd/csrc/tn_trace_general.hip

```cpp
#include "tn_device.h"
#include "tn_kernels.h"

namespace tn {

namespace {

struct WaveSmem {
    uint64_t *key;
    float *hu;
    float *hv;
    uint2 *hft;
    uint32_t *stack;
    uint8_t *mark;
    uint8_t *emitf;
};

__device__ __forceinline__ WaveSmem carve(char *smem, uint32_t M) {
    WaveSmem s;
    s.key = reinterpret_cast<uint64_t *>(smem);
    s.hft = reinterpret_cast<uint2 *>(s.key + M);
    s.hu = reinterpret_cast<float *>(s.hft + (M < 32 ? 32 : M));
    s.hv = s.hu + M;
    s.stack = reinterpret_cast<uint32_t *>(s.hv + M);
    s.mark = reinterpret_cast<uint8_t *>(s.stack + STACK_CAP);
    s.emitf = s.mark + M;
    return s;
}

__device__ __forceinline__ void wave_sync() { __syncthreads(); }

__device__ void insert_overflow(WaveSmem &s, uint32_t cap, uint64_t k, float u, float v, int lane) {
    uint64_t best = 0;
    uint32_t bidx = 0;
    for (uint32_t i = lane; i < cap; i += 64) {
        const uint64_t x = s.key[i];
        if (x >= best) { best = x; bidx = i; }
    }
#pragma unroll
    for (int off = 32; off > 0; off >>= 1) {
        const uint64_t ob = __shfl_xor(best, off);
        const uint32_t oi = __shfl_xor(bidx, off);
        if (ob > best || (ob == best && oi > bidx)) { best = ob; bidx = oi; }
    }
    if (k < best && lane == 0) { s.key[bidx] = k; s.hu[bidx] = u; s.hv[bidx] = v; }
    wave_sync();
}

__device__ void postprocess_and_write(const WaveSmem &s, uint32_t nh, uint32_t M, const uint32_t *__restrict__ faces,
                                      const uint32_t *__restrict__ face_tets, uint32_t *__restrict__ out_num,
                                      uint32_t *__restrict__ out_cells, float *__restrict__ out_bary,
                                      float *__restrict__ out_dist, uint32_t *__restrict__ out_verts,
                                      unsigned long long *stats, int lane, bool compact = false) {
    for (uint32_t base = 0; base < nh; base += 512) {
        uint2 ft[8];
#pragma unroll
        for (int q = 0; q < 8; ++q) {
            const uint32_t j = base + 64 * q + lane;
            if (j < nh) ft[q] = *reinterpret_cast<const uint2 *>(face_tets + 2 * (size_t)(uint32_t)s.key[j]);
        }
#pragma unroll
        for (int q = 0; q < 8; ++q) {
            const uint32_t j = base + 64 * q + lane;
            if (j < nh) { s.hft[j] = ft[q]; s.mark[j] = 0; }
        }
    }
    wave_sync();

    bool bad = false;
    for (uint32_t j = lane; j + 1 < nh; j += 64) {
        uint32_t c;
        const float t0 = __uint_as_float((uint32_t)(s.key[j] >> 32));
        const float t1 = __uint_as_float((uint32_t)(s.key[j + 1] >> 32));
        if (!common_tet(s.hft[j], s.hft[j + 1], c)) bad = true;
        if (j + 2 < nh) {
            const float t2 = __uint_as_float((uint32_t)(s.key[j + 2] >> 32));
            if (fabsf(t1 - t0) < TN_EPS && fabsf(t2 - t1) < TN_EPS) bad = true;
        }
    }
    const bool clean = (__ballot(bad) == 0ull);

    if (clean) {
        for (uint32_t j = lane; j < nh; j += 64) {
            bool em = false;
            if (j + 1 < nh) {
                const float t0 = __uint_as_float((uint32_t)(s.key[j] >> 32));
                const float t1 = __uint_as_float((uint32_t)(s.key[j + 1] >> 32));
                em = fabsf(t0 - t1) >= TN_EPS;
            }
            s.emitf[j] = em ? 1 : 0;
        }
    } else {
        if (stats && lane == 0) atomicAdd(&stats[STAT_LITERAL_BRANCH], 1ull);
        auto Tk = [](uint64_t k) { return __uint_as_float((uint32_t)(k >> 32)); };
        auto T = [&](uint32_t j) { return Tk(s.key[j]); };
        auto ID = [&](uint32_t j) { return (uint32_t)s.key[j]; };
        uint32_t nruns = 0;
        for (uint32_t base = 0; base < nh; base += 64) {
            const uint32_t j = base + lane;
            bool start = false;
            if (j + 1 < nh) {
                const bool sj = fabsf(T(j + 1) - T(j)) < TN_EPS;
                const bool sp = j > 0 && fabsf(T(j) - T(j - 1)) < TN_EPS;
                start = sj && !sp;
            }
            const uint64_t m = __ballot(start);
            if (start) {
                const uint32_t slot = nruns + __popcll(m & lanemask_lt());
                if (slot < (uint32_t)STACK_CAP) s.stack[slot] = j;
            }
            nruns += __popcll(m);
        }
        wave_sync();
        const bool runs_fit = nruns <= (uint32_t)STACK_CAP;
        auto phase1_at = [&](uint32_t j) {
            if (ID(j) == TN_EMPTY) return;
            const float dn = T(j);
            bool clear_self = false;
            for (uint32_t off = 1; j + off < nh && (ID(j + off) == TN_EMPTY || fabsf(T(j + off) - dn) < TN_EPS); ++off) {
                uint32_t c;
                if (ID(j + off) != TN_EMPTY && common_tet(s.hft[j], s.hft[j + off], c)) {
                    if (ID(j) != ID(j + off)) clear_self = true;
                    if (s.mark[j + off]) s.key[j + off] = (s.key[j + off] & 0xFFFFFFFF00000000ull) | TN_EMPTY;
                    else s.mark[j + off] = 1;
                }
            }
            if (clear_self && s.mark[j]) s.key[j] = (s.key[j] & 0xFFFFFFFF00000000ull) | TN_EMPTY;
            s.mark[j] = 0;
        };
        if (runs_fit) {
            for (uint32_t ci = lane; ci < nruns; ci += 64) {
                for (uint32_t j = s.stack[ci];; ++j) {
                    phase1_at(j);
                    if (!(j + 1 < nh && fabsf(T(j + 1) - T(j)) < TN_EPS)) break;
                }
            }
        } else if (lane == 0) {
            for (uint32_t j = 0; j + 1 < nh; ++j) phase1_at(j);
        }
        wave_sync();
        unsigned long long *amask = reinterpret_cast<unsigned long long *>(s.stack);
        for (uint32_t base = 0; base < nh; base += 64) {
            const uint32_t j = base + lane;
            bool anomalous = false;
            uint8_t em = 0;
            if (j + 1 < nh && ID(j) != TN_EMPTY) {
                uint32_t c;
                const bool plain = ID(j + 1) != TN_EMPTY && common_tet(s.hft[j], s.hft[j + 1], c);
                anomalous = !plain;
                em = (plain && fabsf(T(j) - T(j + 1)) >= TN_EPS) ? 1 : 0;
            }
            if (j < nh) s.emitf[j] = em;
            const uint64_t m = __ballot(anomalous);
            if (lane == 0) amask[base >> 6] = m;
        }
        wave_sync();
        if (lane == 0) {
            const uint32_t nwords = (nh + 63) >> 6;
            auto next_anomaly = [&](uint32_t from) -> uint32_t {
                for (uint32_t w = from >> 6; w < nwords; ++w) {
                    unsigned long long m = amask[w];
                    if (w == (from >> 6)) m &= ~0ull << (from & 63);
                    if (m) return (w << 6) + (uint32_t)__ffsll(m) - 1;
                }
                return nh;
            };
            uint32_t touched = 0;
            uint32_t j = next_anomaly(0);
            while (j < nh) {
                s.emitf[j] = 0;
                if (ID(j) != TN_EMPTY) {
                    uint32_t cell;
                    if (j + 1 < nh && ID(j + 1) != TN_EMPTY && common_tet(s.hft[j], s.hft[j + 1], cell)) {
                        if (fabsf(T(j) - T(j + 1)) >= TN_EPS) s.emitf[j] = 1;
                    } else {
                        const uint2 orig = s.hft[j];
                        float dn = T(j);
                        uint32_t real_off = 1;
                        for (uint32_t off = 1; j + off < nh && (real_off < 3 || ID(j + off) == TN_EMPTY || fabsf(T(j + off) - dn) < TN_EPS); ++off) {
                            if (ID(j + off) == TN_EMPTY) continue;
                            if (common_tet(orig, s.hft[j + off], cell)) {
                                if (fabsf(T(j) - T(j + off)) >= TN_EPS) s.emitf[j] = 1;
                                if (off > 1) {
                                    const uint64_t k0 = s.key[j + off]; s.key[j + off] = s.key[j + 1]; s.key[j + 1] = k0;
                                    const float u0 = s.hu[j + off]; s.hu[j + off] = s.hu[j + 1]; s.hu[j + 1] = u0;
                                    const float v0 = s.hv[j + off]; s.hv[j + off] = s.hv[j + 1]; s.hv[j + 1] = v0;
                                    const uint2 f0 = s.hft[j + off]; s.hft[j + off] = s.hft[j + 1]; s.hft[j + 1] = f0;
                                    const uint8_t m0 = s.mark[j + off]; s.mark[j + off] = s.mark[j + 1]; s.mark[j + 1] = m0;
                                    touched = j + off > touched ? j + off : touched;
                                }
                                break;
                            }
                            dn = T(j + off);
                            real_off++;
                        }
                    }
                }
                ++j;
                if (j > touched) j = next_anomaly(j);
            }
        }
    }
    wave_sync();

    uint32_t nseg = 0;
    struct FaceIds { uint32_t a[3], b[3]; bool emit; };
    auto face_ids = [&](uint32_t base) {
        FaceIds r;
        const uint32_t j = base + lane;
        r.emit = j + 1 < nh && s.emitf[j] != 0;
#pragma unroll
        for (int k = 0; k < 3; ++k) r.a[k] = r.b[k] = 0u;
        if (r.emit) {
            const uint32_t f0 = (uint32_t)s.key[j], f1 = (uint32_t)s.key[j + 1];
#pragma unroll
            for (int k = 0; k < 3; ++k) { r.a[k] = faces[3 * (size_t)f0 + k]; r.b[k] = faces[3 * (size_t)f1 + k]; }
        }
        return r;
    };
    FaceIds nxt = face_ids(0);
    for (uint32_t base = 0; base + 1 < nh; base += 64) {
        const uint32_t j = base + lane;
        const FaceIds cur = nxt;
        if (base + 65 < nh) nxt = face_ids(base + 64);
        const bool emit = cur.emit;
        const uint64_t m = __ballot(emit);
        if (emit) {
            const uint32_t slot = nseg + __popcll(m & lanemask_lt());
            const float t0 = __uint_as_float((uint32_t)(s.key[j] >> 32));
            const float t1 = __uint_as_float((uint32_t)(s.key[j + 1] >> 32));
            uint32_t cell = TN_EMPTY;
            common_tet(s.hft[j], s.hft[j + 1], cell);
            const uint32_t id1[3] = {cur.a[0], cur.a[1], cur.a[2]};
            const uint32_t id2[3] = {cur.b[0], cur.b[1], cur.b[2]};
            uint32_t vi[4];
            float b1[3], b2[3];
            combine_indices(id1, id2, s.hu[j], s.hv[j], s.hu[j + 1], s.hv[j + 1], vi, b1, b2);
            out_cells[slot] = cell;
            *reinterpret_cast<float2 *>(out_dist + 2 * (size_t)slot) = make_float2(t0, t1);
            float2 *bp = reinterpret_cast<float2 *>(out_bary + 6 * (size_t)slot);
            bp[0] = make_float2(b1[0], b1[1]);
            bp[1] = make_float2(b1[2], b2[0]);
            bp[2] = make_float2(b2[1], b2[2]);
            if (out_verts) *reinterpret_cast<uint4 *>(out_verts + 4 * (size_t)slot) = make_uint4(vi[0], vi[1], vi[2], vi[3]);
        }
        nseg += __popcll(m);
    }

    for (uint32_t j = nseg + lane; j < (compact ? nseg : M); j += 64) {
        out_cells[j] = TN_EMPTY;
        *reinterpret_cast<float2 *>(out_dist + 2 * (size_t)j) = make_float2(0.f, 0.f);
        float2 *bp = reinterpret_cast<float2 *>(out_bary + 6 * (size_t)j);
        bp[0] = make_float2(0.f, 0.f); bp[1] = make_float2(0.f, 0.f); bp[2] = make_float2(0.f, 0.f);
        if (out_verts) *reinterpret_cast<uint4 *>(out_verts + 4 * (size_t)j) = make_uint4(TN_EMPTY, TN_EMPTY, TN_EMPTY, TN_EMPTY);
    }
    if (lane == 0) *out_num = nseg;
}

__device__ void sort_hits(const WaveSmem &s, uint32_t nh, int lane) {
    uint32_t Np = 1;
    while (Np < nh) Np <<= 1;
    for (uint32_t i = nh + lane; i < Np; i += 64) s.key[i] = ~0ull;
    wave_sync();
    for (uint32_t k = 2; k <= Np; k <<= 1) {
        for (uint32_t j = k >> 1; j > 0; j >>= 1) {
            for (uint32_t tix = lane; tix < (Np >> 1); tix += 64) {
                const uint32_t i = ((tix & ~(j - 1)) << 1) | (tix & (j - 1));
                const uint32_t ij = i | j;
                const uint64_t a = s.key[i], b = s.key[ij];
                const bool up = (i & k) == 0;
                if ((a > b) == up && a != b) {
                    s.key[i] = b; s.key[ij] = a;
                    const float ua = s.hu[i], ub = s.hu[ij]; s.hu[i] = ub; s.hu[ij] = ua;
                    const float va = s.hv[i], vb = s.hv[ij]; s.hv[i] = vb; s.hv[ij] = va;
                }
            }
            wave_sync();
        }
    }
}

__device__ void sort_logged_hits(const WaveSmem &s, uint32_t nh, int lane, uint32_t max_passes) {
    for (uint32_t pass = 0; pass < max_passes; ++pass) {
        bool swapped = false;
#pragma unroll
        for (uint32_t par = 0; par < 2; ++par) {
            for (uint32_t i = 2 * (uint32_t)lane + par; i + 1 < nh; i += 128) {
                const uint64_t a = s.key[i], b = s.key[i + 1];
                if (a > b) {
                    s.key[i] = b; s.key[i + 1] = a;
                    const float ua = s.hu[i], ub = s.hu[i + 1]; s.hu[i] = ub; s.hu[i + 1] = ua;
                    const float va = s.hv[i], vb = s.hv[i + 1]; s.hv[i] = vb; s.hv[i + 1] = va;
                    swapped = true;
                }
            }
            wave_sync();
        }
        if (__ballot(swapped) == 0ull) return;
    }
    sort_hits(s, nh, lane);
}

}

__device__ uint32_t collect_hits(const WideBvh &bvh, WaveSmem &s, uint32_t M, uint32_t cap, float ox, float oy, float oz,
                                 float dx, float dy, float dz, unsigned long long *stats, int lane, bool &overflow,
                                 bool defer = false) {
    const RayPre rp = ray_pre(ox, oy, oz, dx, dy, dz);
    const float ix = safe_inv(dx), iy = safe_inv(dy), iz = safe_inv(dz);
    const float pad = 16.0f * 1.1920929e-7f * (fmaxf(fabsf(ox), fmaxf(fabsf(oy), fabsf(oz))) + bvh.scene_max);
        uint32_t nh = 0;
        overflow = false;
        bool aborted = false;

        auto test_leaf = [&](float a0, float a1, float a2, float b0, float b1, float b2, float c0, float c1, float c2,
                             uint32_t fid) {
            const SV A = shear(rp, a0, a1, a2), B = shear(rp, b0, b1, b2), C = shear(rp, c0, c1, c2);
            float t = 0.f, u = 0.f, v = 0.f;
            const bool hit = (fid != TN_EMPTY) && tri_hit_sv(A, B, C, t, u, v);
            const uint64_t m = __ballot(hit);
            const uint32_t c = __popcll(m);
            if (c) {
                const uint64_t k = ((uint64_t)__float_as_uint(t) << 32) | fid;
                if (nh + c <= cap) {
                    if (hit) {
                        const uint32_t slot = nh + __popcll(m & lanemask_lt());
                        s.key[slot] = k; s.hu[slot] = u; s.hv[slot] = v;
                    }
                    nh += c;
                } else if (defer) {
                    overflow = true;
                    aborted = true;
                } else {
                    overflow = true;
                    wave_sync();
                    uint64_t mm = m;
                    while (mm) {
                        const int src = __ffsll((unsigned long long)mm) - 1;
                        mm &= mm - 1;
                        const uint64_t ks = __shfl(k, src);
                        const float us = __shfl(u, src), vs = __shfl(v, src);
                        if (nh < cap) {
                            if (lane == 0) { s.key[nh] = ks; s.hu[nh] = us; s.hv[nh] = vs; }
                            nh++;
                            wave_sync();
                        } else {
                            insert_overflow(s, cap, ks, us, vs, lane);
                        }
                    }
                }
            }
        };
        uint32_t *leaf_list = reinterpret_cast<uint32_t *>(s.hft);
        const uint32_t leaf_cap = 2 * (M < 32 ? 32 : M);
        uint32_t nleaf = 0;
        auto run_leaves = [&]() {
            wave_sync();
            if (nleaf == 0) return;
            if (lane == 0 && stats) atomicAdd(&stats[STAT_DIAG_LEAVES], (unsigned long long)nleaf);
            const uint32_t LW = bvh.leaf_w, LS = bvh.leaf_shift, G = 64u >> LS;
            const uint32_t sub = (uint32_t)lane >> LS, in = (uint32_t)lane & (LW - 1);
            const uint32_t ngroups = (nleaf + G - 1) / G;
            auto fetch = [&](uint32_t gi, float (&d)[9], uint32_t &fid) {
                const uint32_t e = gi * G + sub;
                fid = TN_EMPTY;
#pragma unroll
                for (int k = 0; k < 9; ++k) d[k] = 0.f;
                if (e < nleaf) {
                    const size_t li = leaf_list[e];
                    const float *tr = bvh.leaf_tri + li * (9 * (size_t)LW) + in;
#pragma unroll
                    for (int k = 0; k < 9; ++k) d[k] = tr[k * LW];
                    fid = bvh.leaf_id[li * LW + in];
                }
            };
            float cur[9], nx1[9], nx2[9];
            uint32_t cfid, f1 = TN_EMPTY, f2 = TN_EMPTY;
            fetch(0, cur, cfid);
            if (ngroups > 1) fetch(1, nx1, f1);
            for (uint32_t i = 0; i < ngroups && !aborted; ++i) {
                if (i + 2 < ngroups) fetch(i + 2, nx2, f2);
                test_leaf(cur[0], cur[1], cur[2], cur[3], cur[4], cur[5], cur[6], cur[7], cur[8], cfid);
#pragma unroll
                for (int k = 0; k < 9; ++k) { cur[k] = nx1[k]; nx1[k] = nx2[k]; }
                cfid = f1; f1 = f2;
            }
            nleaf = 0;
            wave_sync();
        };

        auto load_node = [&](uint32_t idx, float (&bx)[6], uint32_t &ch) {
            const float *b = bvh.boxes + (size_t)idx * (6 * WIDE) + lane;
#pragma unroll
            for (int k = 0; k < 6; ++k) bx[k] = b[k * WIDE];
            ch = bvh.child[(size_t)idx * WIDE + lane];
        };
        uint32_t sp = 0;
        float cbx[6], nbx[6];
        uint32_t cch, nch = TN_EMPTY;
        load_node(0u, cbx, cch);
        bool have_cur = true;
        while (have_cur && !aborted) {
            bool have_nxt = sp > 0;
            if (have_nxt) {
                const uint32_t nidx = s.stack[sp - 1];
                sp--;
                wave_sync();
                load_node(nidx, nbx, nch);
            }
            if (lane == 0 && stats) atomicAdd(&stats[STAT_DIAG_NODES], 1ull);
            const bool hit = cch != TN_EMPTY && line_box(ox, oy, oz, ix, iy, iz, cbx[0], cbx[1], cbx[2], cbx[3], cbx[4], cbx[5], pad);
            const bool to_leaf = hit && (cch >> 31) != 0, to_node = hit && (cch >> 31) == 0;
            const uint64_t ml = __ballot(to_leaf), mn = __ballot(to_node);
            if (nleaf + __popcll(ml) > leaf_cap) run_leaves();
            if (to_leaf) leaf_list[nleaf + __popcll(ml & lanemask_lt())] = cch & 0x7FFFFFFFu;
            nleaf += __popcll(ml);
            if (to_node) s.stack[sp + __popcll(mn & lanemask_lt())] = cch;
            sp += __popcll(mn);
            wave_sync();
            if (!have_nxt && sp > 0) {
                const uint32_t nidx = s.stack[sp - 1];
                sp--;
                wave_sync();
                load_node(nidx, nbx, nch);
                have_nxt = true;
            }
#pragma unroll
            for (int k = 0; k < 6; ++k) cbx[k] = nbx[k];
            cch = nch;
            have_cur = have_nxt;
        }
        if (!aborted) run_leaves();
        wave_sync();
        return nh;
}

#if TN_WALK_DIAG
__device__ unsigned long long g_gen_time[8];
extern "C" int tn_debug_general_time(unsigned long long out[8], int reset) {
    if (hipMemcpyFromSymbol(out, HIP_SYMBOL(g_gen_time), sizeof(unsigned long long) * 8) != hipSuccess) return 1;
    if (reset) { unsigned long long z[8] = {}; if (hipMemcpyToSymbol(HIP_SYMBOL(g_gen_time), z, sizeof z) != hipSuccess) return 1; }
    return 0;
}
#endif
__global__ __launch_bounds__(64) void k_trace_general(TraceParams p) {
    extern __shared__ __attribute__((aligned(16))) char smem[];
    const int lane = threadIdx.x;
    const uint32_t M = p.M;
    const uint32_t C = p.lds_cap && p.lds_cap < M ? p.lds_cap : M;
    const bool defer = C < M;
    WaveSmem s = carve(smem, C);
    const uint32_t cap = C - 1;

    const size_t n_items = p.item_count ? (size_t)*p.item_count : p.num_items;
    for (size_t it = blockIdx.x; it < n_items; it += gridDim.x) {
        const size_t ray = p.ray_list ? (size_t)p.ray_list[it] : it;
        bool overflow = false;
#if TN_WALK_DIAG
        const unsigned long long tk0 = wall_clock64();
#endif
        uint32_t nh = collect_hits(p.bvh, s, C, cap, p.origins[3 * ray], p.origins[3 * ray + 1], p.origins[3 * ray + 2],
                                   p.dirs[3 * ray], p.dirs[3 * ray + 1], p.dirs[3 * ray + 2],
                                   nullptr,
                                   lane, overflow, defer);
#if TN_WALK_DIAG
        const unsigned long long tk1 = wall_clock64();
#endif
        if (overflow && defer) {
            if (lane == 0) p.overflow_list[atomicAdd(p.overflow_count, 1u)] = (uint32_t)ray;
            continue;
        }
        if (overflow && lane == 0 && p.stats) atomicAdd(&p.stats[STAT_OVERFLOW], 1ull);

        sort_hits(s, nh, lane);
#if TN_WALK_DIAG
        const unsigned long long tk2 = wall_clock64();
#endif
        postprocess_and_write(s, nh, M, p.faces, p.face_tets, p.out_num + ray, p.out_cells + ray * M,
                              p.out_bary + ray * M * 6, p.out_dist + ray * M * 2,
                              p.out_verts ? p.out_verts + ray * M * 4 : nullptr, p.stats, lane, p.compact_rows != 0);
        wave_sync();
#if TN_WALK_DIAG
        if (lane == 0) {
            const unsigned long long tk3 = wall_clock64();
            atomicAdd(&g_gen_time[0], 1ull); atomicAdd(&g_gen_time[1], tk1 - tk0); atomicAdd(&g_gen_time[2], tk2 - tk1);
            atomicAdd(&g_gen_time[3], tk3 - tk2); atomicAdd(&g_gen_time[6], (unsigned long long)nh);
        }
#endif
    }
}

__global__ __launch_bounds__(64) void k_postprocess_hits(TraceParams p, const uint32_t *hit_count,
                                                         const uint32_t *hit_ids, const float *hit_t,
                                                         const float *hit_uv) {
    extern __shared__ __attribute__((aligned(16))) char smem[];
    WaveSmem s = carve(smem, p.M);
    const int lane = threadIdx.x;
    const uint32_t M = p.M;
    for (size_t ray = blockIdx.x; ray < p.num_items; ray += gridDim.x) {
        const uint32_t nh = hit_count[ray] < M ? hit_count[ray] : M;
        for (uint32_t j = lane; j < nh; j += 64) {
            s.key[j] = ((uint64_t)__float_as_uint(hit_t[ray * M + j]) << 32) | hit_ids[ray * M + j];
            s.hu[j] = hit_uv[2 * (ray * M + j)];
            s.hv[j] = hit_uv[2 * (ray * M + j) + 1];
        }
        wave_sync();
        postprocess_and_write(s, nh, M, p.faces, p.face_tets, p.out_num + ray, p.out_cells + ray * M,
                              p.out_bary + ray * M * 6, p.out_dist + ray * M * 2,
                              p.out_verts ? p.out_verts + ray * M * 4 : nullptr, p.stats, lane);
        wave_sync();
    }
}

template <bool BINNED>
__global__ __launch_bounds__(64) void k_postprocess_log(TraceParams p, const WalkFid *__restrict__ fidt,
                                                        const uint4 *__restrict__ hit_log,
                                                        const uint2 *__restrict__ literal_list,
                                                        const uint32_t *__restrict__ literal_count,
                                                        const uint32_t *__restrict__ order) {
    extern __shared__ __attribute__((aligned(16))) char smem[];
    WaveSmem s = carve(smem, p.M);
    const int lane = threadIdx.x;
    const uint32_t M = p.M;
    const size_t n_items = *literal_count;
    for (size_t it = blockIdx.x; it < n_items; it += gridDim.x) {
        const uint2 ent = literal_list[it];
        const size_t item = ent.x;
        const size_t ray = BINNED ? (size_t)order[item] : item;
        const uint32_t nh = ent.y < M ? ent.y : M - 1;
        const uint4 *lg = hit_log + (item >> 6) * (size_t)M * 64 + (item & 63);
        for (uint32_t base = 0; base < nh; base += 512) {
            uint4 e[8];
            uint32_t fid[8];
#pragma unroll
            for (int q = 0; q < 8; ++q) {
                const uint32_t j = base + 64 * q + lane;
                if (j < nh) e[q] = lg[(size_t)j * 64];
            }
#pragma unroll
            for (int q = 0; q < 8; ++q) {
                const uint32_t j = base + 64 * q + lane;
                if (j < nh) {
                    const uint32_t x = e[q].w >> 30, lo = e[q].w & 0x3FFFFFFFu;
                    fid[q] = x == 3u ? lo : fidt[lo].fid[x];
                }
            }
#pragma unroll
            for (int q = 0; q < 8; ++q) {
                const uint32_t j = base + 64 * q + lane;
                if (j < nh) {
                    s.key[j] = ((uint64_t)e[q].x << 32) | fid[q];
                    s.hu[j] = __uint_as_float(e[q].y);
                    s.hv[j] = __uint_as_float(e[q].z);
                }
            }
        }
        wave_sync();
        sort_logged_hits(s, nh, lane, p.sort_passes);
        postprocess_and_write(s, nh, M, p.faces, p.face_tets, p.out_num + ray, p.out_cells + ray * M,
                              p.out_bary + ray * M * 6, p.out_dist + ray * M * 2,
                              p.out_verts ? p.out_verts + ray * M * 4 : nullptr, p.stats, lane, p.compact_rows != 0);
        if (lane == 0 && p.stats) atomicAdd(&p.stats[STAT_REASON + REASON_LITERAL_PAIRED], 1ull);
        wave_sync();
    }
}

__global__ __launch_bounds__(64) void k_verify_counts(TraceParams p, uint32_t stride, uint32_t *__restrict__ walk_n,
                                                      uint32_t *__restrict__ fallback_list, uint32_t *__restrict__ fallback_count,
                                                      size_t ray_base, uint32_t late, uint32_t inject,
                                                      const uint32_t *__restrict__ ray_list, const uint32_t *__restrict__ list_count) {
    extern __shared__ __attribute__((aligned(16))) char smem[];
    WaveSmem s = carve(smem, p.M);
    const int lane = threadIdx.x;
    const size_t n_checks = ray_list ? (size_t)*list_count : (p.num_items + stride - 1) / stride;
    const int c_checked = ray_list ? STAT_RISK_CHECKED : STAT_REASON + REASON_VERIFY_CHECKED,
              c_bad = ray_list ? STAT_RISK_BAD : STAT_REASON + REASON_VERIFY_BAD;
    for (size_t it = blockIdx.x; it < n_checks; it += gridDim.x) {
        const size_t ray = ray_list ? (size_t)ray_list[it] : it * stride;
        if (ray_list && stride && ray % stride == 0) continue;
        const uint32_t wn_raw = walk_n[ray];
        if (wn_raw == TN_EMPTY) continue;
        const uint32_t wn = wn_raw & 0x3FFFFFFFu;
        bool overflow = false;
        const uint32_t nh = collect_hits(p.bvh, s, p.M, p.M - 1, p.origins[3 * ray], p.origins[3 * ray + 1], p.origins[3 * ray + 2],
                                         p.dirs[3 * ray], p.dirs[3 * ray + 1], p.dirs[3 * ray + 2], nullptr, lane, overflow);
        if (lane == 0) {
            if (p.stats) atomicAdd(&p.stats[c_checked], 1ull);
            if (nh != wn || overflow || inject) {
                if (!late) walk_n[ray] = TN_EMPTY;
                fallback_list[atomicAdd(fallback_count, 1u)] = (uint32_t)(ray_base + ray);
                if (p.stats) atomicAdd(&p.stats[c_bad], 1ull);
            }
        }
        wave_sync();
    }
}

size_t trace_general_smem_bytes(uint32_t M) {
    return (size_t)M * (8 + 4 + 4) + (size_t)(M < 32 ? 32 : M) * 8 + STACK_CAP * 4 + 2 * (size_t)M;
}

template <typename K>
static size_t wave_smem(K kernel, uint32_t M) {
    const size_t bytes = trace_general_smem_bytes(M);
    if (bytes > 64 * 1024) allow_dynamic_lds(reinterpret_cast<const void *>(kernel), bytes);
    return bytes;
}


__global__ __launch_bounds__(64) void k_trace_triangles(TraceParams p, uint32_t *out_ids, float *out_t, float *out_uv,
                                                        uint32_t *out_v3) {
    extern __shared__ __attribute__((aligned(16))) char smem[];
    WaveSmem s = carve(smem, p.M);
    const int lane = threadIdx.x;
    const uint32_t M = p.M;
    for (size_t ray = blockIdx.x; ray < p.num_items; ray += gridDim.x) {
        bool overflow = false;
        const uint32_t nh = collect_hits(p.bvh, s, M, M - 1, p.origins[3 * ray], p.origins[3 * ray + 1], p.origins[3 * ray + 2],
                                         p.dirs[3 * ray], p.dirs[3 * ray + 1], p.dirs[3 * ray + 2], nullptr, lane, overflow);
        sort_hits(s, nh, lane);
        for (uint32_t j = lane; j < M; j += 64) {
            const bool ok = j < nh;
            const uint32_t id = ok ? (uint32_t)s.key[j] : 0u;
            const size_t q = ray * M + j;
            out_ids[q] = id;
            out_t[q] = ok ? __uint_as_float((uint32_t)(s.key[j] >> 32)) : 0.f;
            out_uv[2 * q] = ok ? s.hu[j] : 0.f;
            out_uv[2 * q + 1] = ok ? s.hv[j] : 0.f;
            for (int k = 0; k < 3; ++k) out_v3[3 * q + k] = ok ? p.faces[3 * (size_t)id + k] : 0u;
        }
        if (lane == 0) p.out_num[ray] = nh;
        wave_sync();
    }
}

__global__ __launch_bounds__(64) void k_find_tetrahedra(TraceParams p, const float *__restrict__ points, uint32_t *out_tet,
                                                        float *out_bary, uint32_t *out_verts) {
    extern __shared__ __attribute__((aligned(16))) char smem[];
    WaveSmem s = carve(smem, p.M);
    const int lane = threadIdx.x;
    const uint32_t M = p.M;
    for (size_t pt = blockIdx.x; pt < p.num_items; pt += gridDim.x) {
        const float ox = points[3 * pt], oy = points[3 * pt + 1], oz = points[3 * pt + 2];
        uint32_t fid[2] = {TN_EMPTY, TN_EMPTY};
        float ht[2] = {0.f, 0.f}, hu[2] = {0.f, 0.f}, hv[2] = {0.f, 0.f};
        for (int side = 0; side < 2; ++side) {
            bool overflow = false;
            const uint32_t nh = collect_hits(p.bvh, s, M, M - 1, ox, oy, oz, side == 0 ? 1.0f : -1.0f, 0.0f, 0.0f, nullptr, lane, overflow);
            wave_sync();
            uint64_t best = ~0ull;
            uint32_t bidx = 0;
            for (uint32_t j = lane; j < nh; j += 64) if (s.key[j] < best) { best = s.key[j]; bidx = j; }
#pragma unroll
            for (int off = 32; off > 0; off >>= 1) {
                const uint64_t ob = __shfl_xor(best, off);
                const uint32_t oi = __shfl_xor(bidx, off);
                if (ob < best) { best = ob; bidx = oi; }
            }
            if (nh) {
                fid[side] = (uint32_t)best; ht[side] = __uint_as_float((uint32_t)(best >> 32));
                hu[side] = s.hu[bidx]; hv[side] = s.hv[bidx];
            }
            wave_sync();
        }
        if (lane == 0) {
            uint32_t cell = TN_EMPTY;
            uint32_t vi[4] = {0, 0, 0, 0};
            float c[3] = {0.f, 0.f, 0.f};
            if (fid[0] != TN_EMPTY && fid[1] != TN_EMPTY) {
                const uint2 t0 = *reinterpret_cast<const uint2 *>(p.face_tets + 2 * (size_t)fid[0]);
                const uint2 t1 = *reinterpret_cast<const uint2 *>(p.face_tets + 2 * (size_t)fid[1]);
                if (common_tet(t0, t1, cell)) {
                    const uint32_t id1[3] = {p.faces[3 * (size_t)fid[0]], p.faces[3 * (size_t)fid[0] + 1], p.faces[3 * (size_t)fid[0] + 2]};
                    const uint32_t id2[3] = {p.faces[3 * (size_t)fid[1]], p.faces[3 * (size_t)fid[1] + 1], p.faces[3 * (size_t)fid[1] + 2]};
                    float c0[3], c1[3];
                    combine_indices(id1, id2, hu[0], hv[0], hu[1], hv[1], vi, c0, c1);
                    const float m = ht[1] / (ht[0] + ht[1]);
                    for (int k = 0; k < 3; ++k) c[k] = c0[k] * m + c1[k] * (1 - m);
                } else {
                    cell = TN_EMPTY;
                }
            }
            out_tet[pt] = cell;
            for (int k = 0; k < 3; ++k) out_bary[3 * pt + k] = c[k];
            for (int k = 0; k < 4; ++k) out_verts[4 * pt + k] = vi[k];
        }
        wave_sync();
    }
}

void launch_trace_triangles(const TraceParams &p, uint32_t *out_ids, float *out_t, float *out_uv, uint32_t *out_v3,
                            hipStream_t stream) {
    if (p.num_items == 0) return;
    const size_t max_blocks = 256 * 16;
    const unsigned grid = (unsigned)(p.num_items < max_blocks ? p.num_items : max_blocks);
    hipLaunchKernelGGL(k_trace_triangles, dim3(grid), dim3(64), wave_smem(k_trace_triangles, p.M), stream, p, out_ids, out_t, out_uv, out_v3);
}

void launch_find_tetrahedra(const TraceParams &p, const float *points, uint32_t *out_tet, float *out_bary,
                            uint32_t *out_verts, hipStream_t stream) {
    if (p.num_items == 0) return;
    const size_t max_blocks = 256 * 16;
    const unsigned grid = (unsigned)(p.num_items < max_blocks ? p.num_items : max_blocks);
    hipLaunchKernelGGL(k_find_tetrahedra, dim3(grid), dim3(64), wave_smem(k_find_tetrahedra, p.M), stream, p, points, out_tet, out_bary, out_verts);
}

void launch_trace_general(const TraceParams &p, hipStream_t stream) {
    if (p.num_items == 0) return;
    const size_t smem = wave_smem(k_trace_general, p.lds_cap && p.lds_cap < p.M ? p.lds_cap : p.M);
    const size_t max_blocks = 256 * 16;
    const unsigned grid = (unsigned)(p.num_items < max_blocks ? p.num_items : max_blocks);
    hipLaunchKernelGGL(k_trace_general, dim3(grid), dim3(64), smem, stream, p);
}

void launch_verify_counts(const TraceParams &p, uint32_t stride, uint32_t *walk_n, uint32_t *fallback_list, uint32_t *fallback_count,
                          size_t ray_base, hipStream_t stream, bool late, bool inject, const uint32_t *ray_list,
                          const uint32_t *list_count, size_t max_list) {
    if (p.num_items == 0 || (stride == 0 && !ray_list)) return;
    const size_t smem = wave_smem(k_verify_counts, p.M);
    const size_t n_checks = ray_list ? std::min<size_t>(max_list, 256 * 16) : (p.num_items + stride - 1) / stride, max_blocks = 256 * 16;
    if (n_checks == 0) return;
    hipLaunchKernelGGL(k_verify_counts, dim3((unsigned)(n_checks < max_blocks ? n_checks : max_blocks)), dim3(64), smem, stream, p, stride,
                       walk_n, fallback_list, fallback_count, ray_base, late ? 1u : 0u, inject ? 1u : 0u, ray_list, list_count);
}

void launch_postprocess_log(const TraceParams &p, const WalkFid *fidt, const uint4 *hit_log, const uint2 *literal_list,
                            const uint32_t *literal_count, size_t max_items, hipStream_t stream, const uint32_t *order) {
    if (max_items == 0) return;
    const size_t max_blocks = 256 * 16;
    const unsigned grid = (unsigned)(max_items < max_blocks ? max_items : max_blocks);
    if (order)
        hipLaunchKernelGGL(k_postprocess_log<true>, dim3(grid), dim3(64), wave_smem(k_postprocess_log<true>, p.M), stream, p, fidt,
                           hit_log, literal_list, literal_count, order);
    else
        hipLaunchKernelGGL(k_postprocess_log<false>, dim3(grid), dim3(64), wave_smem(k_postprocess_log<false>, p.M), stream, p, fidt,
                           hit_log, literal_list, literal_count, order);
}

void launch_postprocess_hits(const TraceParams &p, const uint32_t *hit_count, const uint32_t *hit_ids,
                             const float *hit_t, const float *hit_uv, hipStream_t stream) {
    if (p.num_items == 0) return;
    const size_t smem = wave_smem(k_postprocess_hits, p.M);
    const size_t max_blocks = 256 * 16;
    const unsigned grid = (unsigned)(p.num_items < max_blocks ? p.num_items : max_blocks);
    hipLaunchKernelGGL(k_postprocess_hits, dim3(grid), dim3(64), smem, stream, p, hit_count, hit_ids, hit_t, hit_uv);
}

}
```

### tetra-nerf_amd/tetranerf_cpp_extension.py

```python
from __future__ import annotations

import ctypes as C
import math
import os

import torch

from . import _lib


_POISON = os.environ.get("TETRANERF_HIP_POISON", "") not in ("", "0")


def _empty(*shape, dtype=torch.float32, device=None):
    t = torch.empty(*shape, dtype=dtype, device=device)
    if _POISON and t.numel():
        if t.dtype.is_floating_point:
            t.fill_(float("nan"))
        elif t.dtype == torch.bool:
            t.fill_(True)
        else:
            t.fill_(0x7F7F7F7F if t.dtype in (torch.int32, torch.int64) else 0x7F)
    return t

# ... 140 lines not shown
        return tet_values

    def _check_rays(self, ray_origins, ray_directions, max_ray_triangles):
        M = int(max_ray_triangles)
        if M <= 0 or (M & (M - 1)) != 0:
            raise RuntimeError("max_ray_triangles must be a power of 2.")
        self._check_float_dim3(ray_origins, "ray_origins")
        self._check_float_dim3(ray_directions, "ray_directions")
        R = ray_origins.numel() // 3
        _check(ray_directions.numel() // 3 == R, "ray_origins and ray_directions must have the same number of rays")
        return R, M

    def tet_quality(self, xyz=None):
        with torch.no_grad():
            xyz = self._xyz_or_loaded(xyz)
            V, T, dev = xyz.size(0), self.tetrahedra_cells.numel() // 4, self._device
            width = _empty((T,), dtype=torch.float32, device=dev)
            orient = _empty((T,), dtype=torch.int8, device=dev)
            star = _empty((V,), dtype=torch.float32, device=dev)
            with _on(dev):
                _lib.check(self._lib.tn_tet_quality(self._h, V, _ptr(xyz), _ptr(width), _ptr(orient), _ptr(star), _stream(dev)))
            return {"width": width, "orient": orient, "star_width": star}

    def limit_vertex_step(self, xyz_old, xyz_new, fraction: float = 0.25, verify: bool = True):
        with torch.no_grad():
            self._check_loaded_vertices(xyz_old, "xyz_old")
            self._check_loaded_vertices(xyz_new, "xyz_new")
            V, dev = xyz_old.size(0), self._device
            star = _empty((V,), dtype=torch.float32, device=dev)
            counters = _empty((4,), dtype=torch.int32, device=dev)
            with _on(dev):
                _lib.check(self._lib.tn_limit_vertex_step(self._h, V, _ptr(xyz_old), _ptr(xyz_new), float(fraction), _ptr(star),
                                                          _ptr(counters), 0 if verify else 1, _stream(dev)))
            return counters, star

    supports_delaunay_check = True
    DELAUNAY_GRID_LANES = 1024 * 256

    def delaunay_check(self, xyz=None, face_state: bool = False, tet_violations: bool = False):
        with torch.no_grad():
            xyz = self._xyz_or_loaded(xyz)
            V, T, dev = xyz.size(0), self.tetrahedra_cells.numel() // 4, self._device
            counters = _empty((4,), dtype=torch.int32, device=dev)
            state = _empty((int(self._lib.tn_num_faces(self._h)),), dtype=torch.int8, device=dev) if face_state else None
            per_tet = _empty((4 * ((T + 3) // 4),), dtype=torch.uint8, device=dev) if tet_violations else None
            with _on(dev):
                _lib.check(self._lib.tn_delaunay_check(self._h, V, _ptr(xyz), _ptr(counters), _ptr(state), _ptr(per_tet), _stream(dev)))
            return {"counters": counters, "face_state": state, "tet_violations": None if per_tet is None else per_tet[:T]}

    def retriangulate(self, xyz, tet_values=()):
        with torch.no_grad():
            self._check_loaded_vertices(xyz, "xyz")
            old_cells, V = self.tetrahedra_cells, xyz.size(0)
            tet_values = self._check_tet_values(tet_values, flat=True)
            cells = triangulate(xyz).to(torch.int32).contiguous()
            carried = [remap_tet_values(old_cells, cells, t, V) for t in tet_values]
            self.load_tetrahedra(xyz, cells, refittable=self._refittable)
            return {"cells": cells, "tet_values": carried, "num_tetrahedra": cells.size(0)}

    supports_isosurface = True
    ISOSURFACE_GRID_LANES = 1024 * 256

    def isosurface(self, values, level, tet_mask=None, xyz=None, refine=None):
        xyz = self._xyz_or_loaded(xyz)
        surface = isosurface(xyz.detach(), self.tetrahedra_cells.reshape(-1, 4), values, level, tet_mask)
        if refine is None:
            return surface
        _check(isinstance(refine, dict) and "rounds" in refine and (("density_fn" in refine) != ("field" in refine and "weights" in refine)),
               'refine must be a dict with "rounds" and either "density_fn" or "field" and "weights"')
        if "density_fn" in refine:
            return isosurface_refine_with(surface, xyz.detach(), values, level, refine["density_fn"], refine["rounds"])
        return isosurface_refine(surface, xyz.detach(), values, level, refine["field"], refine["weights"], refine["rounds"],
                                 mode=refine.get("mode", "fp32"))

    supports_split = True
    SPLIT_GRID_LANES = 1024 * 256

    def split_tetrahedra(self, select, vertex_rows=(), tet_values=()):
        with torch.no_grad():
            xyz, cells = self.tetrahedra_vertices, self.tetrahedra_cells
            _check(xyz is not None, "no mesh is loaded; call load_tetrahedra first")
            xyz, cells = xyz.detach().reshape(-1, 3), cells.reshape(-1, 4)
            V, T = xyz.size(0), cells.size(0)
            vertex_rows = tuple(vertex_rows)
            for v in vertex_rows:
                _check_input(v, "vertex_rows")
                _check(v.dtype == torch.float32 and v.dim() == 2 and v.size(1) == V and v.device == self._device,
                       "vertex_rows must be float32 [rows, V] arrays over the loaded vertices, on the tracer's device")
            tet_values = self._check_tet_values(tet_values, flat=False)
            out = split_tetrahedra(xyz, cells, select)
            if out["num_new"] == 0:
                out.update(vertices=self.tetrahedra_vertices, cells=self.tetrahedra_cells, vertex_rows=list(vertex_rows),
                           tet_values=list(tet_values))
                return out
            out["vertex_rows"] = [split_vertex_rows(v.detach(), out["vertex_parents"]) for v in vertex_rows]
            parent = out["cell_parent"].long()
            out["tet_values"] = [t.detach()[parent] for t in tet_values]
            self.load_tetrahedra(out["vertices"], out["cells"], refittable=self._refittable)
            return out

    supports_edge_split = True
    EDGE_SPLIT_GRID_LANES = 1024 * 256

    def edge_split_count(self, select, xyz=None):
        with torch.no_grad():
            xyz = self._xyz_or_loaded(xyz)
            V, T, dev = xyz.size(0), self.tetrahedra_cells.numel() // 4, self._device
            _check_input(select, "select")
            _check(select.dtype in (torch.uint8, torch.bool) and select.numel() == T and select.device == dev,
                   "select must be uint8 or bool [num_cells] on the tracer's device")
            with _on(dev):
                out = _edge_split_buffers(T, dev)
                _lib.check(self._lib.tn_edge_split_count(self._h, V, _ptr(xyz), _ptr(select), _ptr(out["tet_offsets"]), _ptr(out["tet_edge"]),
                                                         _ptr(out["bisected"]), _ptr(out["edge_vertices"]), _ptr(out["counters"]),
                                                         _stream(dev)))
            return out

    def split_edges(self, select, vertex_rows=(), tet_values=()):
        with torch.no_grad():
            xyz, cells = self.tetrahedra_vertices, self.tetrahedra_cells
            _check(xyz is not None, "no mesh is loaded; call load_tetrahedra first")
            xyz, cells = xyz.detach().reshape(-1, 3), cells.reshape(-1, 4)
            V = xyz.size(0)
            vertex_rows = tuple(vertex_rows)
            for v in vertex_rows:
                _check_input(v, "vertex_rows")
                _check(v.dtype == torch.float32 and v.dim() == 2 and v.size(1) == V and v.device == self._device,
                       "vertex_rows must be float32 [rows, V] arrays over the loaded vertices, on the tracer's device")
            tet_values = self._check_tet_values(tet_values, flat=False)
            with _on(self._device):
                out = _edge_split_emit(xyz, cells, self.edge_split_count(select, xyz))
            if out["num_new"] == 0:
                out.update(vertices=self.tetrahedra_vertices, cells=self.tetrahedra_cells, vertex_rows=list(vertex_rows),
                           tet_values=list(tet_values))
                return out
            out["vertex_rows"] = [split_vertex_rows(v.detach(), out["vertex_parents"]) for v in vertex_rows]
            parent = out["cell_parent"].long()
            out["tet_values"] = [t.detach()[parent] for t in tet_values]
            self.load_tetrahedra(out["vertices"], out["cells"], refittable=self._refittable)
            return out

    supports_prune = True
    PRUNE_GRID_LANES = 1024 * 256

    def prune_count(self, dead, vertex_select=None):
        with torch.no_grad():
            xyz = self.tetrahedra_vertices
            _check(xyz is not None, "no mesh is loaded; call load_tetrahedra first")
            V, T, dev = xyz.numel() // 3, self.tetrahedra_cells.numel() // 4, self._device
            _check_prune_masks(dead, vertex_select, T, V, dev)
            with _on(dev):
                offsets = _empty((V + 1,), dtype=torch.int32, device=dev)
                counters = _empty((5,), dtype=torch.int32, device=dev)
                _lib.check(self._lib.tn_prune_count(self._h, V, _ptr(dead), _ptr(vertex_select), _ptr(offsets), _ptr(counters),
                                                    _stream(dev)))
            return offsets, counters

    def remove_vertices(self, dead, vertex_select=None, vertex_rows=(), tet_values=()):
        with torch.no_grad():
            xyz, cells = self.tetrahedra_vertices, self.tetrahedra_cells
            _check(xyz is not None, "no mesh is loaded; call load_tetrahedra first")
            xyz, old_cells = xyz.detach().reshape(-1, 3), cells.reshape(-1, 4)
            V, T, dev = xyz.size(0), old_cells.size(0), self._device
            vertex_rows = tuple(vertex_rows)
            for v in vertex_rows:
                _check_input(v, "vertex_rows")
                _check(v.dtype == torch.float32 and v.dim() == 2 and v.size(1) == V and v.device == dev,
                       "vertex_rows must be float32 [rows, V] arrays over the loaded vertices, on the tracer's device")
            tet_values = self._check_tet_values(tet_values, flat=True)
            offsets, counters = self.prune_count(dead, vertex_select)
            with _on(dev):
                out = _prune_emit(xyz, offsets, counters)
            if out["num_removed"] == 0:
                out.update(vertices=self.tetrahedra_vertices, cells=self.tetrahedra_cells, vertex_rows=list(vertex_rows),
                           tet_values=list(tet_values), num_tetrahedra=T)
                return out
            new_cells = triangulate(out["vertices"]).to(torch.int32).contiguous()
            in_old_ids = out["kept_ids"][new_cells.long()].contiguous()
            out["vertex_rows"] = [prune_vertex_rows(v.detach(), out["kept_ids"]) for v in vertex_rows]
            out["tet_values"] = [remap_tet_values(old_cells, in_old_ids, t.detach(), V) for t in tet_values]
            self.load_tetrahedra(out["vertices"], new_cells, refittable=self._refittable)
            out.update(cells=new_cells, num_tetrahedra=new_cells.size(0))
            return out

    supports_compact_rows = True
    supports_bin_rays = True

    def trace_rays(self, ray_origins, ray_directions, max_ray_triangles, compact_rows: bool = False, bin_rays: bool = False):
        with torch.no_grad():
            R, M = self._check_rays(ray_origins, ray_directions, max_ray_triangles)
            out = _trace_rows(R, M, self._device)
            _lib.check(self._lib.tn_trace_rays_ex(
                self._h, R, M, _ptr(ray_origins), _ptr(ray_directions), *map(_ptr, out.values()),
                (1 if compact_rows else 0) | (2 if bin_rays else 0), _stream(self._device)))
        return out

    def trace_rays_triangles(self, ray_origins, ray_directions, max_ray_triangles):
        with torch.no_grad():
            R, M = self._check_rays(ray_origins, ray_directions, max_ray_triangles)
            dev = self._device
            num = _empty((R,), dtype=torch.int32, device=dev)
            vis = _empty((R, M), dtype=torch.int32, device=dev)
            bary = _empty((R, M, 2), dtype=torch.float32, device=dev)
            dist = _empty((R, M), dtype=torch.float32, device=dev)
            verts = _empty((R, M, 3), dtype=torch.int32, device=dev)
            _lib.check(self._lib.tn_trace_rays_triangles(self._h, R, M, _ptr(ray_origins), _ptr(ray_directions), _ptr(num),
                                                         _ptr(vis), _ptr(bary), _ptr(dist), _ptr(verts), _stream(dev)))
        return {"num_visited_triangles": num, "visited_triangles": vis, "barycentric_coordinates": bary,
                "vertex_indices": verts, "hit_distances": dist}

    def find_tetrahedra(self, positions):
        with torch.no_grad():
            self._check_float_dim3(positions, "positions")
            shape = tuple(positions.shape[:-1])
            N = positions.numel() // 3
            dev = self._device
            bary = _empty(shape + (3,), dtype=torch.float32, device=dev)
            verts = _empty(shape + (4,), dtype=torch.int32, device=dev)
            tets = _empty(shape, dtype=torch.int32, device=dev)
            _lib.check(self._lib.tn_find_tetrahedra(self._h, N, _ptr(positions), _ptr(tets), _ptr(bary), _ptr(verts),
                                                    _stream(dev)))
        return {"tetrahedra": tets, "barycentric_coordinates": bary, "vertex_indices": verts, "valid_mask": tets != -1}

    def find_visited_cells(self, num_visited_cells, visited_cells, barycentric_coordinates,
                           hit_distances, vertex_indices, distances, ray_index=None, count=None):
        sdev = self._device
        for x, name in ((num_visited_cells, "num_visited_cells"), (visited_cells, "visited_cells"),
                        (barycentric_coordinates, "barycentric_coordinates"),
                        (hit_distances, "hit_distances"), (distances, "distances"),
                        (vertex_indices, "vertex_indices")):
            if not (isinstance(x, torch.Tensor) and x.is_cuda and x.is_contiguous() and x.device == sdev):
                _check_input(x, name)
                _check(x.device == sdev, f"{name} must be on the same device")
        _check(distances.dtype == torch.float32, "distances must have float32 type")
        R = num_visited_cells.size(0)
        _check(count is None or ray_index is not None, "find_visited_cells: `count` needs `ray_index` (it counts rows of that list)")
        if ray_index is not None:
            _check_input(ray_index, "ray_index")
            _check(ray_index.dtype == torch.int32 and ray_index.dim() == 1, "ray_index must be int32 [r]")
            _check(ray_index.device == self._device, "ray_index must be on the same device")
            R = ray_index.size(0)
        _check(distances.dim() == 2 and distances.size(0) == R,
               "distances must be of [num_rays, num_samples_per_ray] shape")
        _check(vertex_indices.size(-1) == 4, "vertex_indices must have last dimension with size 4")
        _check(self.tetrahedra_vertices is not None, "load_tetrahedra must be called first")
        _check(num_visited_cells.dtype == torch.int32 and visited_cells.dtype == torch.int32
               and vertex_indices.dtype == torch.int32, "index tensors must have int32 type")
        _check(hit_distances.dtype == torch.float32 and barycentric_coordinates.dtype == torch.float32,
               "hit_distances / barycentric_coordinates must have float32 type")
        S = distances.size(-1)
        M = visited_cells.size(1)
        dev = self._device
        mask = _empty((R, S), dtype=torch.bool, device=dev)
        matched_cells = _empty((R, S), dtype=torch.int32, device=dev)
        barycentric_coordinates_out = _empty((R, S, 3), dtype=torch.float32, device=dev)
        vertex_indices_out = _empty((R, S, 4), dtype=torch.int32, device=dev)
        with _on(dev):
            if ray_index is None:
                _lib.check(self._lib.tn_find_matched_cells(
                    R, S, M, _ptr(num_visited_cells), _ptr(visited_cells), _ptr(hit_distances),
                    _ptr(barycentric_coordinates), _ptr(distances), _ptr(vertex_indices), _ptr(matched_cells),
                    _ptr(vertex_indices_out), _ptr(mask), _ptr(barycentric_coordinates_out), _stream(dev)))
            else:
                _lib.check(self._lib.tn_find_matched_cells_indexed(
                    R, S, M, _ptr(ray_index), _ptr(num_visited_cells), _ptr(visited_cells), _ptr(hit_distances),
                    _ptr(barycentric_coordinates), _ptr(distances), _ptr(vertex_indices), _ptr(matched_cells),
                    _ptr(vertex_indices_out), _ptr(mask), _ptr(barycentric_coordinates_out), _ptr(count), _stream(dev)))
        return {
            "cell_indices": matched_cells,
            "vertex_indices": vertex_indices_out,
            "mask": mask,
            "barycentric_coordinates": barycentric_coordinates_out,
        }

    def trace_stats(self):
        arr = (C.c_uint64 * 4)()
        _lib.check(self._lib.tn_trace_stats(self._h, C.byref(arr)))
        return {"walk": arr[0], "general": arr[1], "serial": arr[2], "overflow": arr[3]}

    def flag_reasons(self):
        arr = (C.c_uint64 * 16)()
        _lib.check(self._lib.tn_trace_flag_reasons(self._h, C.byref(arr)))
        return {k: int(arr[k]) for k in range(1, 16) if arr[k]}

    def set_option(self, name: str, value: int):
        _lib.check(self._lib.tn_set_option(self._h, name.encode(), int(value)))

    def cross_check(self):
        arr = (C.c_uint64 * 8)()
        _lib.check(self._lib.tn_trace_cross_check(self._h, C.byref(arr)))
        return {"stride": int(arr[0]), "checked": int(arr[1]), "mismatches": int(arr[2]),
                "risk": {"hull_near_miss_rays": int(arr[3]), "thin_neighbourhood_rays": int(arr[4]), "checked": int(arr[5]),
                         "mismatches": int(arr[6])}}

    def ray_order(self):
        import numpy as np

        n = C.c_size_t(0)
        _lib.check(self._lib.tn_trace_ray_order(self._h, None, C.byref(n)))
        out = np.empty(n.value, np.uint32)
        if n.value:
            _lib.check(self._lib.tn_trace_ray_order(self._h, out.ctypes.data_as(C.c_void_p), C.byref(n)))
        return out.astype(np.int64)

    TIMING_KEYS = ("speculative_fill", "walk", "bvh_fallback", "cross_check", "segment_writer", "literal_pairing", "tail_fill",
                   "cross_check_retrace")

    def trace_timings(self):
        arr = (C.c_float * 8)()
        _lib.check(self._lib.tn_trace_timings(self._h, C.byref(arr)))
        return {k: float(arr[i]) for i, k in enumerate(self.TIMING_KEYS)}

    def face_tables(self):
        F = self._lib.tn_num_faces(self._h)
        faces = _empty((F, 3), dtype=torch.int32)
        ft = _empty((F, 2), dtype=torch.int32)
        _lib.check(self._lib.tn_get_faces(self._h, _ptr(faces), _ptr(ft)))
        return faces, ft

    def build_table(self, which: int):
        n = C.c_size_t(0)
        _lib.check(self._lib.tn_get_build_table(self._h, int(which), None, C.byref(n)))
        out = _empty((n.value,), dtype=torch.uint8)
        if n.value:
            _lib.check(self._lib.tn_get_build_table(self._h, int(which), _ptr(out), C.byref(n)))
        return out

    def postprocess_hits(self, hit_count, hit_ids, hit_t, hit_uv, faces=None, face_tets=None):
        R, M = hit_ids.shape
        dev = self._device
        out = _trace_rows(R, M, dev)
        hits = (_ptr(hit_count), _ptr(hit_ids), _ptr(hit_t), _ptr(hit_uv))
        if faces is not None:
            _check(face_tets is not None and faces.dtype == torch.int32 and face_tets.dtype == torch.int32
                   and faces.is_contiguous() and face_tets.is_contiguous(), "faces / face_tets must be contiguous int32")
            _lib.check(self._lib.tn_postprocess_hits_tables(dev.index or 0, R, M, _ptr(faces), _ptr(face_tets), *hits,
                                                            *map(_ptr, out.values()), _stream(dev)))
            return out
        _lib.check(self._lib.tn_postprocess_hits(self._h, R, M, *hits, *map(_ptr, out.values()), _stream(dev)))
        return out


def fill_rows(visited_cells, barycentric_coordinates, hit_distances, vertex_indices=None, first_slot=0):
    for x, name in ((visited_cells, "visited_cells"), (barycentric_coordinates, "barycentric_coordinates"),
                    (hit_distances, "hit_distances")) + (() if vertex_indices is None else ((vertex_indices, "vertex_indices"),)):
        _check_input(x, name)
    R, M = visited_cells.shape
    dev = visited_cells.device
    with _on(dev):
        _lib.check(_lib.load().tn_fill_rows(R, M, int(first_slot), _ptr(visited_cells), _ptr(barycentric_coordinates),
                                            _ptr(hit_distances), _ptr(vertex_indices), _stream(dev)))


_FIELD_VM = {}
_CHECK_CACHES = os.environ.get("TETRANERF_HIP_CHECK_CACHES", "0") == "1"


def register_field(field):
    import weakref

    hit = _FIELD_VM.get(id(field))
    if hit is None or hit[0]() is not field:
        key = id(field)

        def _drop(ref, key=key):
            cur = _FIELD_VM.get(key)
            if cur is not None and cur[0] is ref:
                del _FIELD_VM[key]

        _FIELD_VM[key] = (weakref.ref(field, _drop), None, None, None, None)
    return field


def field_is_registered(field) -> bool:
    hit = _FIELD_VM.get(id(field))
    return hit is not None and hit[0]() is field


def install_field_shadow(field, shadow, event=None):
    hit = _FIELD_VM.get(id(field))
    _check(hit is not None and hit[0]() is field, "install_field_shadow: the field is not registered (cpp.register_field)")
    _check(shadow.dtype == torch.float32 and shadow.is_contiguous() and shadow.device == field.device
           and tuple(shadow.shape) == (field.shape[1], field.shape[0]), "install_field_shadow: shadow must be f32 [V, F] on the field's device")
    ev = torch.cuda.Event() if event is None else event
    ev.record(torch.cuda.current_stream(field.device))
    _FIELD_VM[id(field)] = (hit[0], field._version, field.data_ptr(), shadow, ev)
    return ev


def unregister_field(field):
    _FIELD_VM.pop(id(field), None)


def invalidate_field_cache(field=None):
    for k, v in list(_FIELD_VM.items()):
        if v[0]() is None:
            del _FIELD_VM[k]
        elif field is None or v[0]() is field:
            _FIELD_VM[k] = (v[0], None, None, None, None)


def _transpose_field(field):
    Fd, V = field.shape
    ft = _empty((V, Fd), dtype=torch.float32, device=field.device)
    with _on(field.device):
        _lib.check(_lib.load().tn_transpose_f32(Fd, V, _ptr(field), _ptr(ft), _stream(field.device)))
    return ft


def field_vertex_major(field):
    hit = _FIELD_VM.get(id(field))
    if hit is None or hit[0]() is not field:
        hit = next((v for v in _FIELD_VM.values() if v[0]() is not None and v[2] == field.data_ptr()
                    and v[0]().shape == field.shape and v[0]()._version == field._version), None)
        if hit is None:
            return _transpose_field(field)
        field = hit[0]()
    if hit[1] == field._version and hit[2] == field.data_ptr() and hit[3] is not None:
        cur = torch.cuda.current_stream(field.device)
        cur.wait_event(hit[4])
        if _CHECK_CACHES and not torch.equal(hit[3], field.detach().t()):
            raise RuntimeError("the cached vertex-major shadow of a registered field is STALE: the field was written through "
                               ".data or a raw pointer without cpp.invalidate_field_cache(field)")
        return hit[3]
    ft = _transpose_field(field)
    ev = torch.cuda.Event()
    ev.record(torch.cuda.current_stream(field.device))
    _FIELD_VM[id(field)] = (hit[0], field._version, field.data_ptr(), ft, ev)
    return ft


def interpolate_values(vertex_indices, barycentric_coordinates, field):
    for x, name in ((vertex_indices, "vertex_indices"), (barycentric_coordinates, "barycentric_coordinates"),
                    (field, "field")):
        _check_input(x, name)
    _check(vertex_indices.dtype == torch.int32, "vertex_indices must be a tensor of type int32")
    _check(barycentric_coordinates.dtype == torch.float32, "barycentric_coordinates must be a tensor of type float32")
    _check(barycentric_coordinates.size(-1) + 1 == vertex_indices.size(-1),
           "barycentric_coordinates must have the same last dimension as vertex_indices - 1")
    _check(field.dtype == torch.float32, "field must be a tensor of type float32")
    D = vertex_indices.size(-1)
    _check(D in (2, 3, 4, 6), f"Unsupported interpolation dimension with value {D}")
    n = vertex_indices.numel() // D
    Fd = field.size(0)
    result = _empty((Fd,) + tuple(vertex_indices.shape[:-1]), dtype=field.dtype, device=field.device)
    ft = field_vertex_major(field)
    with _on(field.device):
        _lib.check(_lib.load().tn_interpolate_values_vm(
            D, n, Fd, _ptr(vertex_indices), _ptr(barycentric_coordinates), _ptr(ft), _ptr(result), _stream(field.device)))
    return result.moveaxis(0, -1)


def deterministic_gradients() -> bool:
    return bool(DETERMINISTIC_FIELD_GRADIENT) or torch.are_deterministic_algorithms_enabled()


DETERMINISTIC_FIELD_GRADIENT = False


def _gather_adjoint_vm(lib, D, V, n, Fd, vi, bc, rows, grad_vm, stream):
    if deterministic_gradients():
        _lib.check(lib.tn_interpolate_values_backward_vm_det(D, V, n, Fd, _ptr(vi), _ptr(bc), _ptr(rows), _ptr(grad_vm), stream))
    else:
        _lib.check(lib.tn_interpolate_values_backward_vm(D, n, Fd, _ptr(vi), _ptr(bc), _ptr(rows), _ptr(grad_vm), stream))


def interpolate_values_backward(vertex_indices, barycentric_coordinates, field, grad_in):
    for x, name in ((vertex_indices, "vertex_indices"), (barycentric_coordinates, "barycentric_coordinates"),
                    (field, "field"), (grad_in, "grad_in")):
        _check_input(x, name)
    _check(vertex_indices.dtype == torch.int32, "vertex_indices must be a tensor of type int32")
    _check(barycentric_coordinates.dtype == torch.float32, "barycentric_coordinates must be a tensor of type float32")
    _check(field.dtype == torch.float32, "field must be a tensor of type float32")
    _check(grad_in.dtype == torch.float32, "grad_in must be a tensor of type float32")
    _check(barycentric_coordinates.size(-1) + 1 == vertex_indices.size(-1),
           "barycentric_coordinates must have the same last dimension as vertex_indices - 1")
    D = vertex_indices.size(-1)
    _check(D in (2, 3, 4, 6), f"Unsupported interpolation dimension with value {D}")
    n = vertex_indices.numel() // D
    Fd, V = field.size(0), field.size(-1)
    _check(grad_in.size(-1) == Fd, "grad_in must have shape [..., field_dim]")
    grad_field_out = _empty((Fd, V), dtype=grad_in.dtype, device=grad_in.device)
    lib = _lib.load()
    if grad_in.moveaxis(-1, 0).is_contiguous() and Fd > 1 and not deterministic_gradients():
        with _on(field.device):
            _lib.check(lib.tn_interpolate_values_backward(D, V, n, Fd, _ptr(vertex_indices), _ptr(barycentric_coordinates),
                                                          _ptr(grad_in.moveaxis(-1, 0)), _ptr(grad_field_out),
                                                          _stream(field.device)))
        return grad_field_out
    g = grad_in.contiguous()
    grad_vm = torch.zeros((V, Fd), dtype=torch.float32, device=grad_in.device)
    with _on(field.device):
        _gather_adjoint_vm(lib, D, V, n, Fd, vertex_indices, barycentric_coordinates, g, grad_vm, _stream(field.device))
        _lib.check(lib.tn_transpose_f32(V, Fd, _ptr(grad_vm), _ptr(grad_field_out), _stream(field.device)))
    return grad_field_out


def _bary_adjoint_vm(lib, D, n, Fd, vi, rows, field_vm, stream):
    grad_bary = _empty((n, D - 1), dtype=torch.float32, device=rows.device)
    _lib.check(lib.tn_interpolate_values_backward_bary_vm(D, n, Fd, _ptr(vi), _ptr(rows), _ptr(field_vm), _ptr(grad_bary), stream))
    return grad_bary


def interpolate_values_backward_barycentrics(vertex_indices, field, grad_in):
    for x, name in ((vertex_indices, "vertex_indices"), (field, "field"), (grad_in, "grad_in")):
        _check_input(x, name)
    _check(vertex_indices.dtype == torch.int32, "vertex_indices must be a tensor of type int32")
    _check(field.dtype == torch.float32, "field must be a tensor of type float32")
    _check(grad_in.dtype == torch.float32, "grad_in must be a tensor of type float32")
    D = vertex_indices.size(-1)
    _check(D in (2, 3, 4, 6), f"Unsupported interpolation dimension with value {D}")
    n = vertex_indices.numel() // D
    Fd = field.size(0)
    _check(grad_in.size(-1) == Fd and grad_in.numel() == n * Fd, "grad_in must have shape [..., field_dim]")
    ft = field_vertex_major(field)
    with _on(field.device):
        grad_bary = _bary_adjoint_vm(_lib.load(), D, n, Fd, vertex_indices, grad_in, ft, _stream(field.device))
    return grad_bary.view(tuple(vertex_indices.shape[:-1]) + (D - 1,))


def sample_positions_backward(vertex_indices, barycentric_coordinates, grad_bary, vertices, distances=None, want_points=False,
                              want_origins=False, want_directions=False, want_vertices=False):
    for x, name in ((vertex_indices, "vertex_indices"), (barycentric_coordinates, "barycentric_coordinates"),
                    (grad_bary, "grad_bary"), (vertices, "vertices")) + (() if distances is None else ((distances, "distances"),)):
        _check_input(x, name)
    _check(vertex_indices.dtype == torch.int32 and vertex_indices.dim() == 3 and vertex_indices.size(-1) == 4,
           "vertex_indices must be i32 [R,S,4]")
    R, S = vertex_indices.size(0), vertex_indices.size(1)
    for x, name in ((barycentric_coordinates, "barycentric_coordinates"), (grad_bary, "grad_bary")):
        _check(x.dtype == torch.float32 and tuple(x.shape) == (R, S, 3), f"{name} must be f32 [R,S,3]")
    _check(vertices.dtype == torch.float32 and vertices.dim() == 2 and vertices.size(1) == 3, "vertices must be f32 [V,3]")
    _check(distances is None or (distances.dtype == torch.float32 and tuple(distances.shape) == (R, S)), "distances must be f32 [R,S]")
    _check(distances is not None or not want_directions, "want_directions needs the sample distances")
    dev, V = vertices.device, vertices.size(0)
    det = want_vertices and deterministic_gradients()
    points = _empty((R, S, 3), dtype=torch.float32, device=dev) if (want_points or det) else None
    origins = _empty((R, 3), dtype=torch.float32, device=dev) if want_origins else None
    directions = _empty((R, 3), dtype=torch.float32, device=dev) if want_directions else None
    grad_v = torch.zeros((V, 3), dtype=torch.float32, device=dev) if want_vertices else None
    lib = _lib.load()
    with _on(dev):
        stream = _stream(dev)
        _lib.check(lib.tn_sample_positions_backward(R, S, V, _ptr(vertex_indices), _ptr(barycentric_coordinates), _ptr(grad_bary),
                                                    _ptr(distances), _ptr(vertices), _ptr(points), _ptr(origins), _ptr(directions),
                                                    None if det else _ptr(grad_v), stream))
        if det and R * S:
            absent = ((vertex_indices < 0) | (vertex_indices >= V)).any(-1, keepdim=True)
            ids = torch.where(absent, torch.full_like(vertex_indices, -1), vertex_indices)
            _lib.check(lib.tn_interpolate_values_backward_vm_det(4, V, R * S, 3, _ptr(ids), _ptr(barycentric_coordinates),
                                                                 _ptr(points.neg()), _ptr(grad_v), stream))
    return (points if want_points else None), origins, directions, grad_v


class _MlpWeightsStruct(C.Structure):
    _fields_ = [(k, C.c_void_p) for k in ("w1", "b1", "w2", "b2", "w3", "b3", "wd", "bd", "wh", "bh", "wr", "br")]


_WEIGHT_SHAPES = [(128, 64), (128,), (128, 128), (128,), (128, 128), (128,), (1, 128), (1,), (128, 155), (128,), (3, 128), (3,)]
_MODES = {"fp32": 0, "bf16x3": 1, "bf16": 2, 0: 0, 1: 1, 2: 2}


def _mode(mode, inference=True):
    m = _MODES.get(mode)
    _check(m is not None, 'mlp mode must be "fp32", "bf16x3" or (evaluation forwards only) "bf16"')
    _check(inference or m != 2, 'mlp mode must be "fp32" or "bf16x3" here: "bf16" is an arithmetic of the evaluation forwards '
                                '(mlp_forward, mlp_forward_gather, TetraRenderer.render) only')
    return m


class FusedMLP:

    def __init__(self, device):
        device = torch.device(device)
        _check(device.type == "cuda", "The device argument must be a CUDA device.")
        if device.index is None:
            device = torch.device("cuda", torch.cuda.current_device())
        self.device = device
        self._lib = _lib.load()
        h = C.c_void_p()
        _lib.check(self._lib.tn_mlp_create(int(device.index), C.byref(h)))
        self._h = h
        self._key = None

    def close(self):
        h, self._h = getattr(self, "_h", None), None
        if h:
            self._lib.tn_mlp_destroy(h)

    def __del__(self):
        try:
            self.close()
        except Exception:
            pass

    def invalidate(self):
        self._key = None

    def sync(self, weights, force=False):
        _check(len(weights) == 12, "weights must hold 12 tensors")
        import weakref

        key = tuple((w._version, w.data_ptr()) for w in weights)
        if (not force and self._key is not None and key == self._key[0]
                and all(r() is w for r, w in zip(self._key[1], weights))):
            torch.cuda.current_stream(self.device).wait_event(self._packed)
            return self
# ... 1007 lines not shown
```

Baseline: 7.600 billion.

## Split literal pairing into small-LDS and full-LDS launches with prefetched hit logs

The literal-pairing postprocess kernel now runs twice by default. The first launch uses an LDS carve sized from the mesh's expected hit count, about 3.6·cbrt(T) rounded and capped at 512, and handles only rays with fewer hits than that. The second launch handles the remaining rays with the full M-sized carve. Inside the kernel, the next ray's hit log is prefetched while the current ray is being sorted. The first 64·FQ face_tets/faces gathers are hoisted into registers, and stats atomics are batched per block. The aim is higher occupancy through smaller LDS and hiding global load latency. The cost is an extra kernel launch, more register pressure, and each launch scanning the full list to filter its rays.

```diff
diff --git a/include/tetranerf_hip.h b/include/tetranerf_hip.h
--- a/include/tetranerf_hip.h
+++ b/include/tetranerf_hip.h
@@ -179,6 +179,8 @@
 int tn_trace_timings(tn_tracer_t tracer, float ms[8]);
 
 int tn_trace_ray_order(tn_tracer_t tracer, uint32_t *order_host, size_t *n);
+
+int tn_trace_literal_hits(tn_tracer_t tracer, uint32_t *hits_host, size_t *n);
 
 int tn_fill_rows(size_t num_rays, uint32_t max_ray_triangles, uint32_t first_slot, uint32_t *visited, float *bary, float *dist,
                  uint32_t *verts, void *stream);
diff --git a/profiles/literal_pairing_bench.py b/profiles/literal_pairing_bench.py
--- /dev/null
+++ b/profiles/literal_pairing_bench.py
@@ -0,0 +1,124 @@
+import argparse
+import importlib
+import json
+import os
+import sys
+from pathlib import Path
+
+
+def cached_mesh(scenes, n_points, seed):
+    import numpy as np
+
+    pts = np.random.default_rng(seed).random((n_points, 3)).astype(np.float32)
+    f = Path(os.environ.get("TETRANERF_TEST_CACHE", str(Path.home() / ".cache" / "tetranerf_tests"))) / f"delaunay_{n_points}_seed{seed}.npy"
+    if f.exists():
+        return pts, np.load(f)
+    cells = scenes.delaunay_cells(pts)
+    try:
+        f.parent.mkdir(parents=True, exist_ok=True)
+        np.save(f, cells)
+    except OSError:
+        pass
+    return pts, cells
+
+
+def sample(tree, legs, reps_scale):
+    sys.path.insert(0, str(tree))
+    import torch
+    bench = importlib.import_module("bench")
+    assert Path(bench.__file__).resolve().parent == tree, bench.__file__
+    tn = importlib.import_module("tetra-nerf_amd")
+    scenes = importlib.import_module("tetra-nerf_amd.scenes")
+    lib = importlib.import_module("tetra-nerf_amd._lib")
+    dev = torch.device("cuda:0")
+    out = {"library": str(lib.LIB_PATH), "version": lib.load().tn_version().decode()}
+
+    def leg(tr, name, rays, M, reps):
+        o, d = rays
+        o, d = torch.from_numpy(o).to(dev), torch.from_numpy(d).to(dev)
+        r = bench.trace_leg(tr, o, d, M, max(1, reps * reps_scale))
+        bd = r.get("breakdown_ms_serialised") or (bench.trace_breakdown(tr, o, d, M) if r["paths"].get("walk", 0) else None)
+        out[name] = {"ms": r["ms"], "rays": r["rays"], "paths": r["paths"], "timing": bd}
+        print(f"{name}: {r['ms']:.4f} ms" + (f", literal_pairing {bd['literal_pairing']:.4f} ms serialised" if bd else ""), flush=True)
+
+    def tracer(pts, cells):
+        tr = tn.TetrahedraTracer(dev)
+        tr.load_tetrahedra(torch.from_numpy(pts).to(dev), torch.from_numpy(cells).to(dev))
+        return tr
+
+    if "c6" in legs:
+        tr = tracer(*cached_mesh(scenes, 1_000_000, 7))
+        leg(tr, "C6_frame_512x400", bench.frame_rays(scenes, 0, 512, 400), 1024, 10)
+        leg(tr, "C6_batch_4096_outside_in", scenes.outside_in_rays(4096, 31), 1024, 20)
+        del tr
+        torch.cuda.empty_cache()
+    if "c5" in legs:
+        tr = tracer(*cached_mesh(scenes, 150000, 3))
+        leg(tr, "C5_2^20_outside_in", scenes.outside_in_rays(1 << 20, 4), 512, 5)
+        del tr
+        torch.cuda.empty_cache()
+    if "c4" in legs:
+        tr = tracer(*cached_mesh(scenes, 45000, 2))
+        leg(tr, "C4_frame_800x800", bench.frame_rays(scenes, 0, 800, 800), 512, 10)
+        leg(tr, "C4_batch_4096_outside_in", scenes.outside_in_rays(4096, 1), 512, 40)
+        leg(tr, "C4_batch_4096_inside_out", scenes.inside_out_rays(4096, 2), 512, 40)
+        del tr
+        torch.cuda.empty_cache()
+    if "c2" in legs:
+        tr = tracer(*cached_mesh(scenes, 15000, 0))
+        leg(tr, "C2_frame_800x800", bench.frame_rays(scenes, 0, 800, 800), 512, 10)
+        del tr
+    return out
+
+
+def summarise(path):
+    rows = [json.loads(l) for l in Path(path).read_text().splitlines() if l.strip()]
+    labels = sorted({r["label"] for r in rows}, key=lambda l: (l != "parent", l))
+    legs = [k for k in rows[0] if isinstance(rows[0][k], dict) and "ms" in rows[0][k]]
+    print(f"{len(rows)} samples, one fresh process each, in file order: " + " ".join(r["label"] for r in rows))
+    for name in legs:
+        print(f"\n{name}")
+        stat = {}
+        for lab in labels:
+            ms = [r[name]["ms"] for r in rows if r["label"] == lab and name in r]
+            lit = [r[name]["timing"]["literal_pairing"] for r in rows if r["label"] == lab and name in r and r[name]["timing"]]
+            stat[lab] = (ms, lit)
+            line = f"  {lab:7s} ms/call: " + " ".join(f"{x:.4f}" for x in ms) + f" | min {min(ms):.4f} mean {sum(ms) / len(ms):.4f} max {max(ms):.4f} (max/min {max(ms) / min(ms):.3f})"
+            if lit:
+                line += f" | literal_pairing serialised: mean {sum(lit) / len(lit):.4f} (" + " ".join(f"{x:.3f}" for x in lit) + ")"
+            print(line)
+        if "parent" in stat and len(labels) > 1:
+            for lab in labels:
+                if lab == "parent":
+                    continue
+                (pm, pl), (bm, bl) = stat["parent"], stat[lab]
+                mean = lambda v: sum(v) / len(v)
+                print(f"  {lab} / parent: mean ms {mean(bm) / mean(pm):.3f}; ranges " +
+                      ("DISJOINT, every sample below the parent's" if max(bm) < min(pm) else
+                       "disjoint, every sample ABOVE the parent's" if min(bm) > max(pm) else "overlap") +
+                      (f"; literal_pairing serialised {mean(bl) / mean(pl):.3f} of the parent's" if pl and bl else ""))
+
+
+def main():
+    ap = argparse.ArgumentParser()
+    ap.add_argument("--tree", default=str(Path(__file__).resolve().parents[1]))
+    ap.add_argument("--label", default="build")
+    ap.add_argument("--legs", default="c6,c5,c4,c2")
+    ap.add_argument("--reps-scale", type=int, default=1)
+    ap.add_argument("--out", default=None, help="append the sample as one JSON line")
+    ap.add_argument("--summarise", metavar="JSONL", default=None)
+    a = ap.parse_args()
+    if a.summarise:
+        return summarise(a.summarise)
+    res = sample(Path(a.tree).resolve(), a.legs.split(","), a.reps_scale)
+    res["label"] = a.label
+    line = json.dumps(res)
+    if a.out:
+        with open(a.out, "a") as f:
+            f.write(line + "\n")
+    else:
+        print(line)
+
+
+if __name__ == "__main__":
+    main()
diff --git a/profiles/literal_pairing_time.py b/profiles/literal_pairing_time.py
--- /dev/null
+++ b/profiles/literal_pairing_time.py
@@ -0,0 +1,48 @@
+import ctypes as C
+import importlib
+import sys
+from pathlib import Path
+
+import torch
+
+sys.path.insert(0, str(Path(__file__).resolve().parents[1]))
+sys.path.insert(0, str(Path(__file__).resolve().parent))
+from literal_pairing_bench import cached_mesh
+import bench
+
+tn = importlib.import_module("tetra-nerf_amd")
+scenes = importlib.import_module("tetra-nerf_amd.scenes")
+lib = importlib.import_module("tetra-nerf_amd._lib").load()
+dev = torch.device("cuda:0")
+PHASES = ("log read", "face ids -> LDS", "sort", "face_tets + faces gather", "chain test + phases 1/2", "emission", "tail")
+print(lib.tn_version().decode())
+for name, npts, seed, M, rays in (("C6 frame 512x400", 1_000_000, 7, 1024, lambda: bench.frame_rays(scenes, 0, 512, 400)),
+                                  ("C5 2^20 outside-in", 150000, 3, 512, lambda: scenes.outside_in_rays(1 << 20, 4)),
+                                  ("C2 frame 800x800", 15000, 0, 512, lambda: bench.frame_rays(scenes, 0, 800, 800))):
+    pts, cells = cached_mesh(scenes, npts, seed)
+    tr = tn.TetrahedraTracer(dev)
+    tr.load_tetrahedra(torch.from_numpy(pts).to(dev), torch.from_numpy(cells).to(dev))
+    o, d = rays()
+    o, d = torch.from_numpy(o).to(dev), torch.from_numpy(d).to(dev)
+    arr = (C.c_ulonglong * 14)()
+    for timing in (0, 1):
+        tr.set_option("timing", timing)
+        for _ in range(2):
+            tr.trace_rays(o, d, M)
+        torch.cuda.synchronize()
+        lib.tn_debug_literal_time(arr, 1)
+        e0, e1 = torch.cuda.Event(enable_timing=True), torch.cuda.Event(enable_timing=True)
+        e0.record(); tr.trace_rays(o, d, M); e1.record()
+        torch.cuda.synchronize()
+        lib.tn_debug_literal_time(arr, 1)
+        n = max(arr[0], 1)
+        hits = tr.literal_hits()
+        total = sum(arr[1:8]) / n / 100
+        kern = f", kernel {tr.trace_timings()['literal_pairing']:.3f} ms" if timing else ""
+        print(f"{name} ({len(cells)} tets, M = {M}), {'serialised' if timing else 'overlapped'}: call {e0.elapsed_time(e1):.3f} ms{kern} | "
+              f"{arr[0]} literal rays, {hits.mean():.0f} hits on average (max {hits.max()}) | {total:.1f} us per ray: " +
+              ", ".join(f"{p} {arr[i + 1] / n / 100:.1f}" for i, p in enumerate(PHASES)) +
+              f" | pairing in parts: chain test {arr[8] / n / 100:.1f}, phase 1 {arr[9] / n / 100:.1f}, phase 2 plain steps {arr[10] / n / 100:.1f}, "
+              f"lane 0's literal steps + id refresh {arr[11] / n / 100:.1f} ({arr[12] / n:.1f} literal steps, {arr[13] / n:.1f} look-ahead iterations per ray)", flush=True)
+    del tr
+    torch.cuda.empty_cache()
diff --git a/tetra-nerf_amd/_lib.py b/tetra-nerf_amd/_lib.py
--- a/tetra-nerf_amd/_lib.py
+++ b/tetra-nerf_amd/_lib.py
@@ -19,7 +19,7 @@
     "tn_mlp_forward", "tn_mlp_forward_gather", "tn_composite", "tn_gather_uint32", "tn_scatter_ema_uint32",
     "tn_mlp_forward_gather_train", "tn_mlp_forward_gather_train_ex", "tn_mlp_backward", "tn_mlp_backward_ex", "tn_mlp_ray_head_grad", "tn_mlp_param_grads", "tn_mlp_param_grads_ex", "tn_composite_backward", "tn_sample_coarse", "tn_sample_pdf",
     "tn_trace_timings", "tn_trace_cross_check", "tn_fill_rows", "tn_compact_hits", "tn_render_rays", "tn_render_rays_ex",
-    "tn_trace_ray_order",
+    "tn_trace_ray_order", "tn_trace_literal_hits",
     "tn_interpolate_values_backward_bary_vm", "tn_sample_positions_backward",
     "tn_occupancy_update", "tn_cull_samples", "tn_mlp_forward_gather_indexed",
     "tn_mlp_forward_gather_train_indexed", "tn_mlp_param_grads_indexed", "tn_mlp_ray_head_grad_indexed", "tn_compact_rows",
@@ -115,6 +115,7 @@
     lib.tn_trace_timings.argtypes = [vp, C.POINTER(C.c_float * 8)]
     lib.tn_trace_cross_check.argtypes = [vp, C.POINTER(C.c_uint64 * 8)]
     lib.tn_trace_ray_order.argtypes = [vp, vp, C.POINTER(sz)]
+    lib.tn_trace_literal_hits.argtypes = [vp, vp, C.POINTER(sz)]
     lib.tn_fill_rows.argtypes = [sz, u32, u32, vp, vp, vp, vp, vp]
     lib.tn_mlp_create.argtypes = [i32, C.POINTER(vp)]
     lib.tn_mlp_destroy.argtypes = [vp]
diff --git a/tetra-nerf_amd/csrc/tn_api_tracer.hip b/tetra-nerf_amd/csrc/tn_api_tracer.hip
--- a/tetra-nerf_amd/csrc/tn_api_tracer.hip
+++ b/tetra-nerf_amd/csrc/tn_api_tracer.hip
@@ -62,6 +62,7 @@
         bool verify_risk = true;
         unsigned risk_band = 2;
         bool verify_inject = false;
+        unsigned literal_lds_cap = 0;
         unsigned literal_sort_passes = 8;
         int cert_ends = 2;
         bool bin_rays = false;
@@ -264,10 +265,15 @@
         f.k_split = k_hi;
         tn::launch_fill(rows.at(base), n, s().walk_n.p + base, f, stream);
     }
+    uint32_t literal_lds_cap() const {
+        if (o().literal_lds_cap) return o().literal_lds_cap;
+        const uint32_t expect = (uint32_t)(3.6 * std::cbrt((double)std::max<uint32_t>(mesh().T, 1u)));
+        return std::min<uint32_t>((expect + 64u) & ~63u, 512u);
+    }
     void pair_literal(size_t base, size_t n, hipStream_t st) const {
         if (!o().literal) return;
         tn::launch_postprocess_log(trace_params(base, n), mesh().fidt, s().hit_log.p, s().literal_list.p, s().literal_count(), n, st,
-                                   binned ? s().order.p : nullptr);
+                                   binned ? s().order.p : nullptr, literal_lds_cap());
     }
     void trace_listed(const uint32_t *list, const uint32_t *count, size_t max_items, hipStream_t st) const {
         tn::TraceParams q = trace_params(0, max_items);
@@ -1089,6 +1095,24 @@
     });
 }
 
+int tn_trace_literal_hits(tn_tracer_t tracer, uint32_t *hits_host, size_t *n) {
+    return guarded([&] {
+        tn_tracer *t = checked(tracer);
+        std::lock_guard<std::mutex> lock(t->mu);
+        if (!n) throw tn::Error("n is null");
+        tn_tracer::Scratch &s = t->scratch;
+        DeviceGuard g(t->device);
+        TN_HIP(hipStreamSynchronize(s.last_stream));
+        uint32_t count = 0;
+        if (s.literal_list.n) TN_HIP(hipMemcpy(&count, s.literal_count(), sizeof count, hipMemcpyDeviceToHost));
+        *n = std::min<size_t>(count, s.literal_list.n);
+        if (!hits_host || !*n) return;
+        std::vector<uint2> ent(*n);
+        TN_HIP(hipMemcpy(ent.data(), s.literal_list.p, *n * sizeof(uint2), hipMemcpyDeviceToHost));
+        for (size_t i = 0; i < *n; ++i) hits_host[i] = ent[i].y;
+    });
+}
+
 int tn_trace_timings(tn_tracer_t tracer, float ms[8]) {
     return guarded([&] {
         tn_tracer *t = checked(tracer);
@@ -1149,6 +1173,10 @@
             if (value < 0 || (value & (value - 1)) != 0 || (value && value < 8)) throw tn::Error("lds_cap must be 0 or a power of two >= 8");
             o.lds_cap = (unsigned)value;
         }
+        else if (k == "literal_lds_cap") {
+            if (value < 0 || (value && value < 8)) throw tn::Error("literal_lds_cap must be 0 or >= 8");
+            o.literal_lds_cap = (unsigned)value;
+        }
         else if (k == "writer_table") o.writer_table = value;
         else if (k == "refit_tables") o.refit_tables = value != 0;
         else if (k == "cert_ends") { if (value < 0 || value > 3) throw tn::Error("cert_ends must be 0 .. 3"); o.cert_ends = value; }
diff --git a/tetra-nerf_amd/csrc/tn_kernels.h b/tetra-nerf_amd/csrc/tn_kernels.h
--- a/tetra-nerf_amd/csrc/tn_kernels.h
+++ b/tetra-nerf_amd/csrc/tn_kernels.h
@@ -78,7 +78,8 @@
 };
 void launch_trace_walk(const WalkParams &p, hipStream_t stream, size_t lds_reserve = 0);
 void launch_postprocess_log(const TraceParams &p, const WalkFid *fidt, const uint4 *hit_log, const uint2 *literal_list,
-                            const uint32_t *literal_count, size_t max_items, hipStream_t stream, const uint32_t *order = nullptr);
+                            const uint32_t *literal_count, size_t max_items, hipStream_t stream, const uint32_t *order = nullptr,
+                            uint32_t lds_cap = 0);
 
 void launch_verify_counts(const TraceParams &p, uint32_t stride, uint32_t *walk_n, uint32_t *fallback_list, uint32_t *fallback_count,
                           size_t ray_base, hipStream_t stream, bool late = false, bool inject = false, const uint32_t *ray_list = nullptr,
diff --git a/tetra-nerf_amd/csrc/tn_trace_general.hip b/tetra-nerf_amd/csrc/tn_trace_general.hip
--- a/tetra-nerf_amd/csrc/tn_trace_general.hip
+++ b/tetra-nerf_amd/csrc/tn_trace_general.hip
@@ -46,12 +46,42 @@
     wave_sync();
 }
 
+#ifndef TN_WALK_DIAG
+#define TN_WALK_DIAG 0
+#endif
+struct PairTicks { unsigned long long gathered, tested, phase1, plain, paired, emitted, steps, looks; };
+
+template <int FQ>
 __device__ void postprocess_and_write(const WaveSmem &s, uint32_t nh, uint32_t M, const uint32_t *__restrict__ faces,
                                       const uint32_t *__restrict__ face_tets, uint32_t *__restrict__ out_num,
                                       uint32_t *__restrict__ out_cells, float *__restrict__ out_bary,
                                       float *__restrict__ out_dist, uint32_t *__restrict__ out_verts,
-                                      unsigned long long *stats, int lane, bool compact = false) {
-    for (uint32_t base = 0; base < nh; base += 512) {
+                                      uint32_t &serial_rays, int lane, bool compact = false, PairTicks *ticks = nullptr) {
+    uint32_t idf[FQ ? FQ : 1], idv[FQ ? FQ : 1][3];
+    if (FQ) {
+        uint2 ft[FQ ? FQ : 1];
+#pragma unroll
+        for (int q = 0; q < FQ; ++q) {
+            const uint32_t j = 64 * q + lane;
+            idf[q] = j < nh ? (uint32_t)s.key[j] : TN_EMPTY;
+            idv[q][0] = idv[q][1] = idv[q][2] = 0u;
+            ft[q] = make_uint2(0u, 0u);
+        }
+#pragma unroll
+        for (int q = 0; q < FQ; ++q) {
+            if (64u * q < nh && idf[q] != TN_EMPTY) {
+                ft[q] = *reinterpret_cast<const uint2 *>(face_tets + 2 * (size_t)idf[q]);
+#pragma unroll
+                for (int k = 0; k < 3; ++k) idv[q][k] = faces[3 * (size_t)idf[q] + k];
+            }
+        }
+#pragma unroll
+        for (int q = 0; q < FQ; ++q) {
+            const uint32_t j = 64 * q + lane;
+            if (j < nh) { s.hft[j] = ft[q]; s.mark[j] = 0; }
+        }
+    }
+    for (uint32_t base = 64 * FQ; base < nh; base += 512) {
         uint2 ft[8];
 #pragma unroll
         for (int q = 0; q < 8; ++q) {
@@ -65,6 +95,9 @@
         }
     }
     wave_sync();
+#if TN_WALK_DIAG
+    if (ticks) ticks->gathered = wall_clock64();
+#endif
 
     bool bad = false;
     for (uint32_t j = lane; j + 1 < nh; j += 64) {
@@ -78,6 +111,9 @@
         }
     }
     const bool clean = (__ballot(bad) == 0ull);
+#if TN_WALK_DIAG
+    if (ticks) ticks->tested = ticks->phase1 = ticks->plain = wall_clock64();
+#endif
 
     if (clean) {
         for (uint32_t j = lane; j < nh; j += 64) {
@@ -90,7 +126,7 @@
             s.emitf[j] = em ? 1 : 0;
         }
     } else {
-        if (stats && lane == 0) atomicAdd(&stats[STAT_LITERAL_BRANCH], 1ull);
+        serial_rays++;
         auto Tk = [](uint64_t k) { return __uint_as_float((uint32_t)(k >> 32)); };
         auto T = [&](uint32_t j) { return Tk(s.key[j]); };
         auto ID = [&](uint32_t j) { return (uint32_t)s.key[j]; };
@@ -138,6 +174,9 @@
             for (uint32_t j = 0; j + 1 < nh; ++j) phase1_at(j);
         }
         wave_sync();
+#if TN_WALK_DIAG
+        if (ticks) ticks->phase1 = ticks->plain = wall_clock64();
+#endif
         unsigned long long *amask = reinterpret_cast<unsigned long long *>(s.stack);
         for (uint32_t base = 0; base < nh; base += 64) {
             const uint32_t j = base + lane;
@@ -154,6 +193,9 @@
             if (lane == 0) amask[base >> 6] = m;
         }
         wave_sync();
+#if TN_WALK_DIAG
+        if (ticks) ticks->plain = wall_clock64();
+#endif
         if (lane == 0) {
             const uint32_t nwords = (nh + 63) >> 6;
             auto next_anomaly = [&](uint32_t from) -> uint32_t {
@@ -167,6 +209,9 @@
             uint32_t touched = 0;
             uint32_t j = next_anomaly(0);
             while (j < nh) {
+#if TN_WALK_DIAG
+                if (ticks) ticks->steps++;
+#endif
                 s.emitf[j] = 0;
                 if (ID(j) != TN_EMPTY) {
                     uint32_t cell;
@@ -177,6 +222,9 @@
                         float dn = T(j);
                         uint32_t real_off = 1;
                         for (uint32_t off = 1; j + off < nh && (real_off < 3 || ID(j + off) == TN_EMPTY || fabsf(T(j + off) - dn) < TN_EPS); ++off) {
+#if TN_WALK_DIAG
+                            if (ticks) ticks->looks++;
+#endif
                             if (ID(j + off) == TN_EMPTY) continue;
                             if (common_tet(orig, s.hft[j + off], cell)) {
                                 if (fabsf(T(j) - T(j + off)) >= TN_EPS) s.emitf[j] = 1;
@@ -201,8 +249,60 @@
         }
     }
     wave_sync();
+    if (!clean) {
+#pragma unroll
+        for (int q = 0; q < FQ; ++q) {
+            const uint32_t j = 64 * q + lane;
+            const uint32_t f = j < nh ? (uint32_t)s.key[j] : TN_EMPTY;
+            if (f != idf[q] && f != TN_EMPTY) {
+                idf[q] = f;
+#pragma unroll
+                for (int k = 0; k < 3; ++k) idv[q][k] = faces[3 * (size_t)f + k];
+            }
+        }
+    }
+#if TN_WALK_DIAG
+    if (ticks) ticks->paired = wall_clock64();
+#endif
 
     uint32_t nseg = 0;
+    auto emit_row = [&](uint32_t j, uint32_t slot, const uint32_t (&id1)[3], const uint32_t (&id2)[3]) {
+        const float t0 = __uint_as_float((uint32_t)(s.key[j] >> 32));
+        const float t1 = __uint_as_float((uint32_t)(s.key[j + 1] >> 32));
+        uint32_t cell = TN_EMPTY;
+        common_tet(s.hft[j], s.hft[j + 1], cell);
+        uint32_t vi[4];
+        float b1[3], b2[3];
+        combine_indices(id1, id2, s.hu[j], s.hv[j], s.hu[j + 1], s.hv[j + 1], vi, b1, b2);
+        out_cells[slot] = cell;
+        *reinterpret_cast<float2 *>(out_dist + 2 * (size_t)slot) = make_float2(t0, t1);
+        float2 *bp = reinterpret_cast<float2 *>(out_bary + 6 * (size_t)slot);
+        bp[0] = make_float2(b1[0], b1[1]);
+        bp[1] = make_float2(b1[2], b2[0]);
+        bp[2] = make_float2(b2[1], b2[2]);
+        if (out_verts) *reinterpret_cast<uint4 *>(out_verts + 4 * (size_t)slot) = make_uint4(vi[0], vi[1], vi[2], vi[3]);
+    };
+#pragma unroll
+    for (int q = 0; q < FQ; ++q) {
+        if (64u * q + 1 < nh) {
+            const uint32_t j = 64 * q + lane;
+            const bool emit = j + 1 < nh && s.emitf[j] != 0;
+            uint32_t id2[3];
+#pragma unroll
+            for (int k = 0; k < 3; ++k) {
+                const uint32_t give = (q + 1 < FQ && lane == 0) ? idv[q + 1 < FQ ? q + 1 : q][k] : idv[q][k];
+                id2[k] = __shfl(give, (lane + 1) & 63);
+            }
+            if (q + 1 == FQ && lane == 63 && emit) {
+                const uint32_t f1 = (uint32_t)s.key[j + 1];
+#pragma unroll
+                for (int k = 0; k < 3; ++k) id2[k] = faces[3 * (size_t)f1 + k];
+            }
+            const uint64_t m = __ballot(emit);
+            if (emit) emit_row(j, nseg + __popcll(m & lanemask_lt()), idv[q], id2);
+            nseg += __popcll(m);
+        }
+    }
     struct FaceIds { uint32_t a[3], b[3]; bool emit; };
     auto face_ids = [&](uint32_t base) {
         FaceIds r;
@@ -217,34 +317,20 @@
         }
         return r;
     };
-    FaceIds nxt = face_ids(0);
-    for (uint32_t base = 0; base + 1 < nh; base += 64) {
-        const uint32_t j = base + lane;
-        const FaceIds cur = nxt;
-        if (base + 65 < nh) nxt = face_ids(base + 64);
-        const bool emit = cur.emit;
-        const uint64_t m = __ballot(emit);
-        if (emit) {
-            const uint32_t slot = nseg + __popcll(m & lanemask_lt());
-            const float t0 = __uint_as_float((uint32_t)(s.key[j] >> 32));
-            const float t1 = __uint_as_float((uint32_t)(s.key[j + 1] >> 32));
-            uint32_t cell = TN_EMPTY;
-            common_tet(s.hft[j], s.hft[j + 1], cell);
-            const uint32_t id1[3] = {cur.a[0], cur.a[1], cur.a[2]};
-            const uint32_t id2[3] = {cur.b[0], cur.b[1], cur.b[2]};
-            uint32_t vi[4];
-            float b1[3], b2[3];
-            combine_indices(id1, id2, s.hu[j], s.hv[j], s.hu[j + 1], s.hv[j + 1], vi, b1, b2);
-            out_cells[slot] = cell;
-            *reinterpret_cast<float2 *>(out_dist + 2 * (size_t)slot) = make_float2(t0, t1);
-            float2 *bp = reinterpret_cast<float2 *>(out_bary + 6 * (size_t)slot);
-            bp[0] = make_float2(b1[0], b1[1]);
-            bp[1] = make_float2(b1[2], b2[0]);
-            bp[2] = make_float2(b2[1], b2[2]);
-            if (out_verts) *reinterpret_cast<uint4 *>(out_verts + 4 * (size_t)slot) = make_uint4(vi[0], vi[1], vi[2], vi[3]);
-        }
-        nseg += __popcll(m);
-    }
+    if (64u * FQ + 1 < nh) {
+        FaceIds nxt = face_ids(64 * FQ);
+        for (uint32_t base = 64 * FQ; base + 1 < nh; base += 64) {
+            const uint32_t j = base + lane;
+            const FaceIds cur = nxt;
+            if (base + 65 < nh) nxt = face_ids(base + 64);
+            const uint64_t m = __ballot(cur.emit);
+            if (cur.emit) emit_row(j, nseg + __popcll(m & lanemask_lt()), cur.a, cur.b);
+            nseg += __popcll(m);
+        }
+    }
+#if TN_WALK_DIAG
+    if (ticks) ticks->emitted = wall_clock64();
+#endif
 
     for (uint32_t j = nseg + lane; j < (compact ? nseg : M); j += 64) {
         out_cells[j] = TN_EMPTY;
@@ -280,6 +366,27 @@
 }
 
 __device__ void sort_logged_hits(const WaveSmem &s, uint32_t nh, int lane, uint32_t max_passes) {
+    auto network = [&]() {
+        uint32_t Np = 1;
+        while (Np < nh) Np <<= 1;
+        for (uint32_t k = 2; k <= Np; k <<= 1) {
+            for (uint32_t j = k >> 1; j > 0; j >>= 1) {
+                for (uint32_t tix = lane; tix < (Np >> 1); tix += 64) {
+                    const uint32_t i = ((tix & ~(j - 1)) << 1) | (tix & (j - 1));
+                    const uint32_t ij = j == (k >> 1) ? i ^ (k - 1) : i | j;
+                    if (ij < nh) {
+                        const uint64_t a = s.key[i], b = s.key[ij];
+                        if (a > b) {
+                            s.key[i] = b; s.key[ij] = a;
+                            const float ua = s.hu[i], ub = s.hu[ij]; s.hu[i] = ub; s.hu[ij] = ua;
+                            const float va = s.hv[i], vb = s.hv[ij]; s.hv[i] = vb; s.hv[ij] = va;
+                        }
+                    }
+                }
+                wave_sync();
+            }
+        }
+    };
     for (uint32_t pass = 0; pass < max_passes; ++pass) {
         bool swapped = false;
 #pragma unroll
@@ -297,7 +404,7 @@
         }
         if (__ballot(swapped) == 0ull) return;
     }
-    sort_hits(s, nh, lane);
+    network();
 }
 
 }
@@ -452,6 +559,7 @@
     const uint32_t cap = C - 1;
 
     const size_t n_items = p.item_count ? (size_t)*p.item_count : p.num_items;
+    uint32_t n_serial = 0;
     for (size_t it = blockIdx.x; it < n_items; it += gridDim.x) {
         const size_t ray = p.ray_list ? (size_t)p.ray_list[it] : it;
         bool overflow = false;
@@ -475,9 +583,9 @@
 #if TN_WALK_DIAG
         const unsigned long long tk2 = wall_clock64();
 #endif
-        postprocess_and_write(s, nh, M, p.faces, p.face_tets, p.out_num + ray, p.out_cells + ray * M,
+        postprocess_and_write<0>(s, nh, M, p.faces, p.face_tets, p.out_num + ray, p.out_cells + ray * M,
                               p.out_bary + ray * M * 6, p.out_dist + ray * M * 2,
-                              p.out_verts ? p.out_verts + ray * M * 4 : nullptr, p.stats, lane, p.compact_rows != 0);
+                              p.out_verts ? p.out_verts + ray * M * 4 : nullptr, n_serial, lane, p.compact_rows != 0);
         wave_sync();
 #if TN_WALK_DIAG
         if (lane == 0) {
@@ -487,6 +595,7 @@
         }
 #endif
     }
+    if (lane == 0 && p.stats && n_serial) atomicAdd(&p.stats[STAT_LITERAL_BRANCH], (unsigned long long)n_serial);
 }
 
 __global__ __launch_bounds__(64) void k_postprocess_hits(TraceParams p, const uint32_t *hit_count,
@@ -496,6 +605,7 @@
     WaveSmem s = carve(smem, p.M);
     const int lane = threadIdx.x;
     const uint32_t M = p.M;
+    uint32_t n_serial = 0;
     for (size_t ray = blockIdx.x; ray < p.num_items; ray += gridDim.x) {
         const uint32_t nh = hit_count[ray] < M ? hit_count[ray] : M;
         for (uint32_t j = lane; j < nh; j += 64) {
@@ -504,41 +614,84 @@
             s.hv[j] = hit_uv[2 * (ray * M + j) + 1];
         }
         wave_sync();
-        postprocess_and_write(s, nh, M, p.faces, p.face_tets, p.out_num + ray, p.out_cells + ray * M,
+        postprocess_and_write<8>(s, nh, M, p.faces, p.face_tets, p.out_num + ray, p.out_cells + ray * M,
                               p.out_bary + ray * M * 6, p.out_dist + ray * M * 2,
-                              p.out_verts ? p.out_verts + ray * M * 4 : nullptr, p.stats, lane);
-        wave_sync();
-    }
-}
-
-template <bool BINNED>
-__global__ __launch_bounds__(64) void k_postprocess_log(TraceParams p, const WalkFid *__restrict__ fidt,
+                              p.out_verts ? p.out_verts + ray * M * 4 : nullptr, n_serial, lane);
+        wave_sync();
+    }
+    if (lane == 0 && p.stats && n_serial) atomicAdd(&p.stats[STAT_LITERAL_BRANCH], (unsigned long long)n_serial);
+}
+
+#if TN_WALK_DIAG
+__device__ unsigned long long g_lit_time[14];
+extern "C" int tn_debug_literal_time(unsigned long long out[14], int reset) {
+    if (hipMemcpyFromSymbol(out, HIP_SYMBOL(g_lit_time), sizeof(unsigned long long) * 14) != hipSuccess) return 1;
+    if (reset) { unsigned long long z[14] = {}; if (hipMemcpyToSymbol(HIP_SYMBOL(g_lit_time), z, sizeof z) != hipSuccess) return 1; }
+    return 0;
+}
+#endif
+template <bool BINNED, int FQ>
+__global__ __launch_bounds__(64) __attribute__((amdgpu_waves_per_eu(FQ <= 8 ? 3 : 2))) void k_postprocess_log(TraceParams p, const WalkFid *__restrict__ fidt,
                                                         const uint4 *__restrict__ hit_log,
                                                         const uint2 *__restrict__ literal_list,
                                                         const uint32_t *__restrict__ literal_count,
-                                                        const uint32_t *__restrict__ order) {
+                                                        const uint32_t *__restrict__ order, uint32_t C, uint32_t split, uint32_t take) {
     extern __shared__ __attribute__((aligned(16))) char smem[];
-    WaveSmem s = carve(smem, p.M);
+    WaveSmem s = carve(smem, C);
     const int lane = threadIdx.x;
     const uint32_t M = p.M;
     const size_t n_items = *literal_count;
-    for (size_t it = blockIdx.x; it < n_items; it += gridDim.x) {
-        const uint2 ent = literal_list[it];
+    auto next_own = [&](size_t from, uint2 &ent) -> size_t {
+        for (size_t it = from; it < n_items; it += gridDim.x) {
+            ent = literal_list[it];
+            if (take == 0u || (ent.y < split) == (take == 1u)) return it;
+        }
+        return n_items;
+    };
+    auto hits_of = [&](const uint2 &ent) { return ent.y < M ? ent.y : M - 1; };
+    auto log_of = [&](const uint2 &ent) { return hit_log + ((size_t)ent.x >> 6) * (size_t)M * 64 + (ent.x & 63u); };
+    uint4 e[8];
+    auto request_log = [&](const uint2 &ent) {
+        const uint32_t n = hits_of(ent);
+        const uint4 *lg = log_of(ent);
+#pragma unroll
+        for (int q = 0; q < 8; ++q) {
+            const uint32_t j = 64 * q + lane;
+            e[q] = make_uint4(0u, 0u, 0u, 0u);
+            if (j < n) e[q] = lg[(size_t)j * 64];
+        }
+    };
+    uint32_t n_serial = 0, n_paired = 0;
+    uint2 ent = make_uint2(0u, 0u);
+    size_t it = next_own(blockIdx.x, ent);
+    if (it < n_items) request_log(ent);
+    while (it < n_items) {
+#if TN_WALK_DIAG
+        const unsigned long long tk0 = wall_clock64();
+#endif
         const size_t item = ent.x;
         const size_t ray = BINNED ? (size_t)order[item] : item;
-        const uint32_t nh = ent.y < M ? ent.y : M - 1;
-        const uint4 *lg = hit_log + (item >> 6) * (size_t)M * 64 + (item & 63);
+        const uint32_t nh = hits_of(ent);
+        const uint4 *lg = log_of(ent);
+        uint2 ent_n = make_uint2(0u, 0u);
+        const size_t it_n = next_own(it + gridDim.x, ent_n);
+#if TN_WALK_DIAG
+        { uint32_t w = 0; for (int q = 0; q < 8; ++q) w |= e[q].w; asm volatile("" ::"v"(w)); }
+        const unsigned long long tk1 = wall_clock64();
+#endif
         for (uint32_t base = 0; base < nh; base += 512) {
-            uint4 e[8];
             uint32_t fid[8];
+            if (base) {
+#pragma unroll
+                for (int q = 0; q < 8; ++q) {
+                    const uint32_t j = base + 64 * q + lane;
+                    if (j < nh) e[q] = lg[(size_t)j * 64];
+                }
+            }
 #pragma unroll
             for (int q = 0; q < 8; ++q) {
                 const uint32_t j = base + 64 * q + lane;
-                if (j < nh) e[q] = lg[(size_t)j * 64];
-            }
-#pragma unroll
-            for (int q = 0; q < 8; ++q) {
-                const uint32_t j = base + 64 * q + lane;
+                fid[q] = TN_EMPTY;
                 if (j < nh) {
                     const uint32_t x = e[q].w >> 30, lo = e[q].w & 0x3FFFFFFFu;
                     fid[q] = x == 3u ? lo : fidt[lo].fid[x];
@@ -555,12 +708,38 @@
             }
         }
         wave_sync();
+#if TN_WALK_DIAG
+        const unsigned long long tk2 = wall_clock64();
+#endif
+        if (it_n < n_items) request_log(ent_n);
         sort_logged_hits(s, nh, lane, p.sort_passes);
-        postprocess_and_write(s, nh, M, p.faces, p.face_tets, p.out_num + ray, p.out_cells + ray * M,
-                              p.out_bary + ray * M * 6, p.out_dist + ray * M * 2,
-                              p.out_verts ? p.out_verts + ray * M * 4 : nullptr, p.stats, lane, p.compact_rows != 0);
-        if (lane == 0 && p.stats) atomicAdd(&p.stats[STAT_REASON + REASON_LITERAL_PAIRED], 1ull);
-        wave_sync();
+        PairTicks tk{};
+#if TN_WALK_DIAG
+        const unsigned long long tk3 = wall_clock64();
+#endif
+        postprocess_and_write<FQ>(s, nh, M, p.faces, p.face_tets, p.out_num + ray, p.out_cells + ray * M,
+                                  p.out_bary + ray * M * 6, p.out_dist + ray * M * 2,
+                                  p.out_verts ? p.out_verts + ray * M * 4 : nullptr, n_serial, lane, p.compact_rows != 0, &tk);
+        n_paired++;
+        wave_sync();
+#if TN_WALK_DIAG
+        if (lane == 0) {
+            const unsigned long long tk4 = wall_clock64();
+            atomicAdd(&g_lit_time[0], 1ull); atomicAdd(&g_lit_time[1], tk1 - tk0); atomicAdd(&g_lit_time[2], tk2 - tk1);
+            atomicAdd(&g_lit_time[3], tk3 - tk2); atomicAdd(&g_lit_time[4], tk.gathered - tk3);
+            atomicAdd(&g_lit_time[5], tk.paired - tk.gathered); atomicAdd(&g_lit_time[6], tk.emitted - tk.paired);
+            atomicAdd(&g_lit_time[7], tk4 - tk.emitted);
+            atomicAdd(&g_lit_time[8], tk.tested - tk.gathered); atomicAdd(&g_lit_time[9], tk.phase1 - tk.tested);
+            atomicAdd(&g_lit_time[10], tk.plain - tk.phase1); atomicAdd(&g_lit_time[11], tk.paired - tk.plain);
+            atomicAdd(&g_lit_time[12], tk.steps); atomicAdd(&g_lit_time[13], tk.looks);
+        }
+#endif
+        it = it_n;
+        ent = ent_n;
+    }
+    if (lane == 0 && p.stats) {
+        if (n_serial) atomicAdd(&p.stats[STAT_LITERAL_BRANCH], (unsigned long long)n_serial);
+        if (n_paired) atomicAdd(&p.stats[STAT_REASON + REASON_LITERAL_PAIRED], (unsigned long long)n_paired);
     }
 }
 
@@ -724,16 +903,25 @@
 }
 
 void launch_postprocess_log(const TraceParams &p, const WalkFid *fidt, const uint4 *hit_log, const uint2 *literal_list,
-                            const uint32_t *literal_count, size_t max_items, hipStream_t stream, const uint32_t *order) {
+                            const uint32_t *literal_count, size_t max_items, hipStream_t stream, const uint32_t *order,
+                            uint32_t lds_cap) {
     if (max_items == 0) return;
     const size_t max_blocks = 256 * 16;
     const unsigned grid = (unsigned)(max_items < max_blocks ? max_items : max_blocks);
-    if (order)
-        hipLaunchKernelGGL(k_postprocess_log<true>, dim3(grid), dim3(64), wave_smem(k_postprocess_log<true>, p.M), stream, p, fidt,
-                           hit_log, literal_list, literal_count, order);
-    else
-        hipLaunchKernelGGL(k_postprocess_log<false>, dim3(grid), dim3(64), wave_smem(k_postprocess_log<false>, p.M), stream, p, fidt,
-                           hit_log, literal_list, literal_count, order);
+    auto launch = [&](uint32_t C, uint32_t take) {
+        auto go = [&](auto kernel) {
+            hipLaunchKernelGGL(kernel, dim3(grid), dim3(64), wave_smem(kernel, C), stream, p, fidt, hit_log, literal_list,
+                               literal_count, order, C, lds_cap, take);
+        };
+        if (C <= 512) { if (order) go(k_postprocess_log<true, 8>); else go(k_postprocess_log<false, 8>); }
+        else          { if (order) go(k_postprocess_log<true, 16>); else go(k_postprocess_log<false, 16>); }
+    };
+    if (lds_cap && lds_cap < p.M) {
+        launch(lds_cap, 1u);
+        launch(p.M, 2u);
+    } else {
+        launch(p.M, 0u);
+    }
 }
 
 void launch_postprocess_hits(const TraceParams &p, const uint32_t *hit_count, const uint32_t *hit_ids,
diff --git a/tetra-nerf_amd/tetranerf_cpp_extension.py b/tetra-nerf_amd/tetranerf_cpp_extension.py
--- a/tetra-nerf_amd/tetranerf_cpp_extension.py
+++ b/tetra-nerf_amd/tetranerf_cpp_extension.py
@@ -466,6 +466,16 @@
         if n.value:
             _lib.check(self._lib.tn_trace_ray_order(self._h, out.ctypes.data_as(C.c_void_p), C.byref(n)))
         return out.astype(np.int64)
+
+    def literal_hits(self):
+        import numpy as np
+
+        n = C.c_size_t(0)
+        _lib.check(self._lib.tn_trace_literal_hits(self._h, None, C.byref(n)))
+        out = np.empty(n.value, np.uint32)
+        if n.value:
+            _lib.check(self._lib.tn_trace_literal_hits(self._h, out.ctypes.data_as(C.c_void_p), C.byref(n)))
+        return out[:n.value].astype(np.int64)
 
     TIMING_KEYS = ("speculative_fill", "walk", "bvh_fallback", "cross_check", "segment_writer", "literal_pairing", "tail_fill",
                    "cross_check_retrace")
```

Result: no change. 7.580 billion (median of 2 runs) (-0.3%).
